# WPCLab/OpenSeg3D

Measured on AMD Instinct MI355X. Metric: points/sec fwd+bwd, Waymo 1-sweep ~180k pts @0.1m voxel; logit parity, higher is better.
Workload: dtype f32 storage/accumulate, bf16x3 products; 1 GPU; waymo_one_sweep (BASELINE configs[1]): synthetic scene, 174633 pts/step/GPU, voxel [0.1, 0.1, 0.1], grid [1440, 1440, 64], fwd (attention dropout p=0.1, DropPath) + criterion (ohem_ce+lovasz on 3 heads) + bwd + SGD step; mode=fwdbwd, segmentor=segformer, voxels=108690, parallelism=dp1

## Files before the change

include/seg3d_hip.h:

```cpp
#ifndef SEG3D_HIP_H
#define SEG3D_HIP_H

#include <stddef.h>
#include <stdint.h>

#ifdef __cplusplus
extern "C" {
#endif

#define SEG3D_OK 0
#define SEG3D_EINVAL (-1)
#define SEG3D_EWORKSPACE (-2)
#define SEG3D_ELAUNCH (-3)

#define SEG3D_REDUCE_SUM 0
#define SEG3D_REDUCE_MEAN 1
#define SEG3D_REDUCE_MAX 2

int seg3d_abi_version(void);

const char* seg3d_last_error(void);

int seg3d_grid_size(const float* voxel_size, const float* range, int32_t* grid_xyz);

size_t seg3d_voxelize_workspace_bytes(int64_t n_points);
int seg3d_voxelize_f32(const float* points, int64_t n_points, int32_t row_stride, int32_t xyz_col,
                       int32_t batch_col, const float* voxel_size, const float* range,
                       int32_t* voxel_coords, int32_t* point_voxel_ids, int32_t* n_voxels,
                       void* workspace, size_t workspace_bytes, void* stream);
int seg3d_voxelize_f64(const double* points, int64_t n_points, int32_t row_stride, int32_t xyz_col,
                       int32_t batch_col, const float* voxel_size, const float* range,
                       int32_t* voxel_coords, int32_t* point_voxel_ids, int32_t* n_voxels,
                       void* workspace, size_t workspace_bytes, void* stream);

size_t seg3d_voxelize_host_workspace_bytes(int64_t n_points);
int seg3d_voxelize_host_f32(const float* points, int64_t n_points, int32_t row_stride, int32_t xyz_col,
                            int32_t batch_col, const float* voxel_size, const float* range,
                            int32_t* voxel_coords, int32_t* point_voxel_ids, int32_t* n_voxels,
                            void* workspace, size_t workspace_bytes);
int seg3d_voxelize_host_f64(const double* points, int64_t n_points, int32_t row_stride, int32_t xyz_col,
                            int32_t batch_col, const float* voxel_size, const float* range,
                            int32_t* voxel_coords, int32_t* point_voxel_ids, int32_t* n_voxels,
                            void* workspace, size_t workspace_bytes);

int seg3d_cart2polar_f32(const float* points, int64_t n_points, int32_t row_stride, int32_t xyz_col,
                         float* out , void* stream);
int seg3d_cart2polar_f64(const double* points, int64_t n_points, int32_t row_stride, int32_t xyz_col,
                         double* out , void* stream);

size_t seg3d_group_index_workspace_bytes(int64_t n, int64_t n_groups);
int seg3d_group_index(const int32_t* group_ids, int64_t n, int64_t n_groups, int32_t* rank,
                      int32_t* order, int32_t* offsets, void* workspace, size_t workspace_bytes,
                      void* stream);

size_t seg3d_coord_hash_bytes(int64_t m);
int seg3d_coord_hash_build(const int32_t* coords, int64_t m, const int32_t* shape_zyx ,
                           void* table, size_t table_bytes, void* stream);
int seg3d_rulebook_subm(const int32_t* coords, int64_t m, const int32_t* shape_zyx ,
                        const void* table, size_t table_bytes, int32_t* nbr, void* stream);
size_t seg3d_downsample_workspace_bytes(int32_t batch_size, const int32_t* shape_in_zyx );
int seg3d_downsample_coords(const int32_t* coords_in, int64_t m_in,
                            const int32_t* m_in_dev ,
                            int32_t batch_size, const int32_t* shape_in_zyx , int32_t* coords_out,
                            int64_t cap_out, int32_t* m_out , void* workspace, size_t workspace_bytes,
                            void* stream);
int seg3d_rulebook_strided(const int32_t* coords_out, int64_t m_out, int64_t m_in,
                           const int32_t* shape_in_zyx , const void* table_in,
                           size_t table_bytes, int32_t* nbr_fwd, int32_t* nbr_inv, void* stream);

size_t seg3d_spconv_packed_bytes(int32_t cin, int32_t cout, int32_t flags);
int seg3d_spconv_pack_weight(const float* weight, int32_t cin, int32_t cout, int32_t flags,
                             void* w_packed, void* stream);
int seg3d_spconv_fwd(const float* x, const int32_t* nbr, int64_t m_out, int64_t m_in,
                     const void* w_packed, int32_t pack_flags, const float* bias ,
                     int32_t cin, int32_t cout, float* y,
                     const int32_t* row_order ,
                     void* stream);
int seg3d_spconv_fwd_act(const float* x, const int32_t* nbr, int64_t m_out, int64_t m_in, const void* w_packed,
                         int32_t pack_flags, const float* bias , const float* addend ,
                         int32_t relu, int32_t cin, int32_t cout, float* y, const int32_t* row_order ,
                         void* stream);
int seg3d_spconv_fwd_act_bf16(const void* x, int32_t x_bf16, const int32_t* nbr, int64_t m_out, int64_t m_in,
                              const void* w_packed, int32_t pack_flags, const float* bias,
                              const void* addend_bf16, int32_t relu, int32_t cin, int32_t cout, void* y_bf16,
                              const int32_t* row_order, void* stream);
size_t seg3d_spconv_presplit_bytes(int64_t m_in, int32_t cin);
int seg3d_spconv_presplit(const float* x, int64_t m_in, int32_t cin, void* xs, void* stream);
int seg3d_spconv_fwd_presplit(const void* xs, const int32_t* nbr, int64_t m_out, int64_t m_in, const void* w_packed,
                              int32_t pack_flags, const float* bias , const float* addend ,
                              int32_t relu, int32_t cin, int32_t cout, float* y,
                              const int32_t* row_order , void* stream);
size_t seg3d_conv_plan_bytes(int64_t m_out);
size_t seg3d_conv_plan_workspace_bytes(int64_t m_out);
int seg3d_conv_plan_build(const int32_t* coords, const int32_t* nbr, int64_t m_out, void* plan, void* workspace,
                          size_t workspace_bytes, void* stream);
int32_t seg3d_spconv_tiled_supported(int32_t cin, int32_t cout);
int seg3d_spconv_fwd_tiled(const float* x, const int32_t* nbr, const void* plan, int64_t m_out, int64_t m_in,
                           const void* w_packed, int32_t pack_flags, const float* bias ,
                           const float* addend , int32_t relu, int32_t cin, int32_t cout, float* y, void* stream);
int seg3d_spconv_fwd_tiled_bf16(const void* x, int32_t x_bf16, const int32_t* nbr, const void* plan, int64_t m_out,
                                int64_t m_in, const void* w_packed, int32_t pack_flags, const float* bias ,
                                const void* addend_bf16 , int32_t relu, int32_t cin, int32_t cout, void* y_bf16,
                                void* stream);
int seg3d_debug_set_conv_nbt(int32_t nbt);
int seg3d_debug_set_linear_stream(int32_t on);
size_t seg3d_spconv_wgrad_workspace_bytes(int64_t m_out, int32_t cin, int32_t cout);
int seg3d_spconv_wgrad(const float* x, const float* dy, const int32_t* nbr, int64_t m_out,
                       int64_t m_in, int32_t cin, int32_t cout, int32_t flags ,
                       float* dw, void* workspace, size_t workspace_bytes, void* stream);

int seg3d_spconv_wgrad_partials(const float* x, const float* dy, const int32_t* nbr, int64_t m_out, int64_t m_in,
                                int32_t cin, int32_t cout, void* workspace, size_t workspace_bytes, int32_t* chunks,
                                void* stream);
int seg3d_spconv_wgrad_partials_xbf16(const uint16_t* x_bf16, const float* dy, const int32_t* nbr, int64_t m_out,
                                      int64_t m_in, int32_t cin, int32_t cout, void* workspace, size_t workspace_bytes,
                                      int32_t* chunks, void* stream);

size_t seg3d_linear_wgrad_workspace_bytes(int64_t m, int32_t cin, int32_t cout);
int seg3d_linear_wgrad(const float* x, const float* dy, int64_t m, int32_t cin, int32_t cout, float* dw,
                       float* db , void* workspace, size_t workspace_bytes, void* stream);
int seg3d_linear_wgrad_partials(const float* x, const float* dy, int64_t m, int32_t cin, int32_t cout, int32_t with_bias,
                                void* workspace, size_t workspace_bytes, int32_t* chunks, void* stream);
int seg3d_linear_wgrad_partials_xbf16(const uint16_t* x_bf16, const float* dy, int64_t m, int32_t cin, int32_t cout,
                                      int32_t with_bias, void* workspace, size_t workspace_bytes, int32_t* chunks,
                                      void* stream);
int seg3d_debug_set_wgrad_lds(int32_t on);
int seg3d_reduce_partials(const float* part, int32_t chunks, int64_t n, int64_t nw, float* dw, float* db, void* stream);
int seg3d_reduce_partials_batched(const void* jobs, int32_t n_jobs, int64_t total_blocks, void* stream);
size_t seg3d_linear_packed_bytes_f32(int32_t cin, int32_t cout);
int seg3d_linear_pack_weight_f32(const float* weight, int32_t cin, int32_t cout, int32_t transpose,
                                 void* w_packed, void* stream);
int seg3d_linear_fwd_f32(const float* x, int64_t m, const void* w_packed, const float* bias ,
                         int32_t cin, int32_t cout, float* y, void* stream);
size_t seg3d_linear_packed_bytes_x6(int32_t cin, int32_t cout);
int seg3d_linear_pack_weight_x6(const float* weight, int32_t cin, int32_t cout, int32_t transpose, void* w_packed,
                                void* stream);
int seg3d_linear_fwd_x6(const float* x, int64_t m, const void* w_packed, const float* bias ,
                        const float* scale , const float* shift , int32_t relu, int32_t cin,
                        int32_t cout, float* y, void* stream);

typedef struct {
  const float* src;
  void* dst;
  int32_t cin, cout;
  int32_t kk, transpose, flip, reserved;
  int64_t first_block;
} seg3d_pack_job;
int seg3d_pack_weights_batched(const void* jobs, int32_t n_jobs, int64_t total_blocks, void* stream);

size_t seg3d_linear_packed_bytes(int32_t cin, int32_t cout, int32_t transpose);
int seg3d_linear_pack_weight(const float* weight, int32_t cin, int32_t cout, int32_t transpose,
                             void* w_packed, void* stream);
int seg3d_linear_fwd(const float* x, int64_t m, const void* w_packed, const float* bias ,
                     const float* addend , int32_t cin, int32_t cout,
                     float* y, void* stream);
int seg3d_linear_fwd_sum(const float* x, const float* x_add, int64_t m, const void* w_packed, const float* bias,
                         int32_t cin, int32_t cout, float* y, void* stream);
int seg3d_linear_layernorm_fwd(const float* x, int64_t m, const void* w_packed, const float* bias, const float* res,
                               const float* gamma, const float* beta, float eps, int32_t cin, int32_t cout, float* y,
                               void* stream);
int seg3d_linear_fwd_mul(const float* x, int64_t m, const void* w_packed, const float* factor, int32_t cin, int32_t cout,
                         float* y, void* stream);

size_t seg3d_window_partition_workspace_bytes(int64_t m, int32_t batch_size, const int32_t* nwin_xyz);
int seg3d_window_partition(const int32_t* coords, int64_t m, int32_t batch_size,
                           const int32_t* win_xyz, const int32_t* nwin_xyz, const int32_t* shift_xyz,
                           int32_t n_levels, const int32_t* level_lo, const int32_t* level_hi,
                           const int32_t* level_cap, int32_t* win_id, int32_t* in_win, int32_t* rank,
                           int32_t* level, int32_t* slot, int32_t* tok, int32_t* win_start,
                           int32_t* win_count, int32_t* win_tile0, int32_t* tile_item,
                           int32_t* qg_item, int32_t* counts, void* workspace,
                           size_t workspace_bytes, void* stream);

int seg3d_pos_embed(const int32_t* in_win, int64_t m, const int32_t* win_xyz ,
                    const float* inv_freq, int32_t c, float* pos, void* stream);

int seg3d_window_attn_supported(int32_t heads, int32_t dh);
size_t seg3d_window_attn_workspace_bytes(int64_t m, int32_t n_tiles, int32_t heads, int32_t dh);
int seg3d_window_attn_schedule(int32_t n_tiles, int32_t n_chunks, int32_t heads, int32_t dh, float dropout_p, int32_t* out);
int seg3d_window_attn_fwd(const float* q, const float* k, const float* v, int32_t ldq, int32_t ldk,
                          int32_t ldv, const int32_t* tok, const int32_t* win_start,
                          const int32_t* win_count, const int32_t* win_tile0,
                          const int32_t* tile_item, int32_t n_tiles, const int32_t* qg_item,
                          int32_t n_qgroups, int64_t m, int32_t n_windows, int32_t heads, int32_t dh,
                          const float* tau, float tau_min, float dropout_p, uint64_t dropout_seed, float* out,
                          float* lse, void* workspace, size_t workspace_bytes, void* stream);
int seg3d_window_attn_bwd(const float* q, const float* k, const float* v, int32_t ldq, int32_t ldk,
                          int32_t ldv, const float* out, const float* dout, const float* lse,
                          const int32_t* tok, const int32_t* win_start, const int32_t* win_count,
                          const int32_t* win_tile0, const int32_t* tile_item, int32_t n_tiles,
                          const int32_t* qg_item, int32_t n_qgroups, int64_t m, int32_t n_windows,
                          int32_t heads, int32_t dh, const float* tau,
                          float tau_min, float dropout_p, uint64_t dropout_seed, float* dq, float* dk,
                          float* dv, int32_t lddq, int32_t lddk,
                          int32_t lddv, float* dtau, void* workspace, size_t workspace_bytes,
                          void* stream);

int seg3d_layernorm_fwd(const float* x, const float* res, const float* gamma, const float* beta,
                        const float* rowscale, float eps, int64_t m, int32_t c, float* y, float* mean,
                        float* rstd, void* stream);
size_t seg3d_layernorm_bwd_workspace_bytes(int64_t m, int32_t c);
int seg3d_layernorm_bwd(const float* dy, const float* x, const float* mean, const float* rstd,
                        const float* gamma, const float* rowscale, int64_t m, int32_t c, float* dx,
                        float* dgamma, float* dbeta, void* workspace, size_t workspace_bytes, void* stream);
int seg3d_layernorm_bwd_partials(const float* dy, const float* x, const float* mean, const float* rstd,
                                 const float* gamma, const float* rowscale, int64_t m, int32_t c, float* dx,
                                 void* workspace, size_t workspace_bytes, int32_t* nblocks, void* stream);
size_t seg3d_batchnorm_workspace_bytes(int64_t m, int32_t c);
int seg3d_colstats(const float* x, int64_t m, int32_t c, float* sums, void* workspace, size_t workspace_bytes,
                   void* stream);
int seg3d_batchnorm_stats(const float* x, int64_t m, int32_t c, float eps, const float* gamma, const float* beta,
                          float momentum, float* running_mean, float* running_var, float* stats, void* workspace,
                          size_t workspace_bytes, void* stream);
int seg3d_gelu_fwd(const float* h, int64_t n, float* g, float* gp, void* stream);
int seg3d_affine_act(const float* x, const float* res, const float* scale, const float* shift, int32_t relu,
                     int64_t m, int32_t c, float* y, void* stream);
int seg3d_batchnorm_bwd(const float* dy, const float* y, const float* x, const float* mean, const float* rstd,
                        const float* gamma, int32_t relu, int64_t m, int32_t c, float* dx, float* dres,
                        float* sums, void* workspace, size_t workspace_bytes, void* stream);
int seg3d_batchnorm_bwd_reduce(const float* dy, const float* y, const float* x, const float* mean,
                               const float* rstd, int32_t relu, int64_t m, int32_t c, float* sums,
                               void* workspace, size_t workspace_bytes, void* stream);
int seg3d_batchnorm_bwd_apply(const float* dy, const float* y, const float* x, const float* mean,
                              const float* rstd, const float* gamma, const float* sums, const float* inv_count,
                              int32_t relu, int64_t m, int32_t c, float* dx, float* dres, void* stream);

int seg3d_segment_reduce_fwd(const float* x, int32_t c, const int32_t* order, const int32_t* offsets,
                             int64_t n_seg, int32_t mode, float* out, int32_t* argmax, void* stream);
int seg3d_segment_reduce_bwd(const float* dout, int32_t c, const int32_t* seg_of_row, int64_t n,
                             const int32_t* offsets, const int32_t* argmax, int64_t n_seg,
                             int32_t mode, float* dx, void* stream);

int seg3d_knn_attention_fwd(const float* q, const float* k, const float* v, const int32_t* idx,
                            const uint8_t* invalid, const float* keep, int64_t n, int64_t n_src,
                            int32_t n_neighbors, int32_t d, float scale, float* out, float* prob, void* stream);
int seg3d_knn_attention_bwd(const float* q, const float* k, const float* v, const int32_t* idx, const float* keep,
                            const float* prob, const float* dout, const int32_t* pair_order,
                            const int32_t* pair_offsets, int64_t n, int64_t n_src, int32_t n_neighbors, int32_t d,
                            float scale, float* dq, float* dk, float* dv, float* scratch, void* stream);

int seg3d_class_context_fwd(const float* feats, const float* probs, const int32_t* offsets, const int32_t* chunks,
                            const int32_t* chunk_offsets, int32_t n_chunks, int32_t batch, int64_t m,
                            int32_t classes, int32_t c, float scale, float* weights, float* partials, float* stats,
                            float* context, void* stream);
int seg3d_class_context_bwd(const float* feats, const float* weights, const float* dcontext,
                            const int32_t* offsets, const int32_t* chunks, const int32_t* chunk_offsets,
                            int32_t n_chunks, int32_t batch, int64_t m, int32_t classes, int32_t c, float scale,
                            float* dfeats, float* dprobs, float* scratch, void* stream);

int seg3d_gather_rows(const float* feats, const int32_t* ids, int64_t n, int32_t c, float* out,
                      void* stream);

int seg3d_knn_query(const float* xyz, int64_t n, const float* new_xyz, int64_t m, const int32_t* offset,
                    const int32_t* new_offset, int32_t batch_size, int32_t k, int32_t* idx, float* dist2,
                    void* stream);

size_t seg3d_knn_level_workspace_bytes(int64_t n);
int seg3d_knn_level_build(const float* xyz, int64_t n, const int32_t* offset, int32_t batch_size, float cell,
                          float* sorted_xyz, int32_t* src_index, int32_t* cell_end, void* table_keys, int32_t* table_vals,
                          int64_t capacity, void* workspace, size_t workspace_bytes, void* stream);
int seg3d_knn_query_order(const float* new_xyz, int64_t m, const int32_t* new_offset, int32_t batch_size, float cell,
                          int32_t* order, void* workspace, size_t workspace_bytes, void* stream);
int seg3d_parity_order(const int32_t* coords, int64_t m, int32_t* order, void* workspace, size_t workspace_bytes,
                       void* stream);
typedef struct {
  const float* sorted_xyz;
  const int32_t* src_index;
  const int32_t* cell_end;
  const void* table_keys;
  const int32_t* table_vals;
  int64_t capacity;
  float cell;
  int32_t max_ring;
} seg3d_knn_level;
int seg3d_knn_grid_query(const seg3d_knn_level* levels, int32_t n_levels, const float* new_xyz,
                         const int32_t* query_order , int64_t m,
                         const int32_t* offset, const int32_t* new_offset, int32_t batch_size, int32_t k,
                         int32_t* idx, float* dist2, void* stream);

size_t seg3d_furthest_sampling_workspace_bytes(int64_t n);
int seg3d_furthest_sampling(const float* xyz, int64_t n, const int32_t* order, const int32_t* offset,
                            const int32_t* new_offset, int32_t n_segments, int32_t* idx, void* workspace,
                            size_t workspace_bytes, void* stream);
int seg3d_furthest_sampling_host(const float* xyz, int64_t n, const int32_t* order, const int32_t* offset,
                                 const int32_t* new_offset, int32_t n_segments, int32_t* idx);
int seg3d_sector_angles(const float* xyz, int64_t n, const int32_t* offset, int32_t batch_size, float* angle,
                        float* minmax, void* stream);
int seg3d_sector_angles_host(const float* xyz, int64_t n, const int32_t* offset, int32_t batch_size, float* angle,
                             float* minmax);
int seg3d_sector_assign(const float* angle, int64_t n, const int32_t* offset, int32_t batch_size, const float* edges,
                        const int32_t* sector_offset, int32_t* sector_id, void* stream);
int seg3d_sector_assign_host(const float* angle, int64_t n, const int32_t* offset, int32_t batch_size,
                             const float* edges, const int32_t* sector_offset, int32_t* sector_id);

#define SEG3D_POINTOPS_CHUNK 512
size_t seg3d_pointops_scratch_bytes(int64_t m, int32_t k, int32_t width);
int seg3d_group_points_fwd(const float* xyz, const float* new_xyz, const float* feat, const int32_t* idx, int64_t n,
                           int64_t m, int32_t k, int32_t c, float* out, void* stream);
int seg3d_group_points_fwd_host(const float* xyz, const float* new_xyz, const float* feat, const int32_t* idx, int64_t n,
                                int64_t m, int32_t k, int32_t c, float* out);
int seg3d_group_points_bwd(const float* dout, const int32_t* idx, const int32_t* pair_order, const int32_t* pair_offsets,
                           int64_t n, int64_t m, int32_t k, int32_t c, int32_t with_xyz, float* dxyz, float* dnew_xyz,
                           float* dfeat, void* scratch, size_t scratch_bytes, void* stream);
int seg3d_group_points_bwd_host(const float* dout, const int32_t* idx, const int32_t* pair_order,
                                const int32_t* pair_offsets, int64_t n, int64_t m, int32_t k, int32_t c,
                                int32_t with_xyz, float* dxyz, float* dnew_xyz, float* dfeat);
int seg3d_knn_interpolate_fwd(const float* feat, const int32_t* idx, const float* dist, int64_t n, int64_t m, int32_t k,
                              int32_t c, float* out, float* weight, void* stream);
int seg3d_knn_interpolate_fwd_host(const float* feat, const int32_t* idx, const float* dist, int64_t n, int64_t m,
                                   int32_t k, int32_t c, float* out, float* weight);
int seg3d_knn_interpolate_bwd(const float* dout, const float* weight, const int32_t* idx, const int32_t* pair_order,
                              const int32_t* pair_offsets, int64_t n, int64_t m, int32_t k, int32_t c, float* dfeat,
                              void* scratch, size_t scratch_bytes, void* stream);
int seg3d_knn_interpolate_bwd_host(const float* dout, const float* weight, const int32_t* idx, const int32_t* pair_order,
                                   const int32_t* pair_offsets, int64_t n, int64_t m, int32_t k, int32_t c,
                                   float* dfeat);

#define SEG3D_SUBM_DOT_ROWS 128
size_t seg3d_subm_dot_scratch_bytes(int64_t M, int32_t C);
int seg3d_subm_dot_fwd(const float* x, const int32_t* nbr, const float* w, const float* bias, int64_t M, int32_t C,
                       float* s_out, float* y_out, void* stream);
int seg3d_subm_dot_fwd_host(const float* x, const int32_t* nbr, const float* w, const float* bias, int64_t M, int32_t C,
                            float* s_out, float* y_out);
int seg3d_subm_dot_bwd_ds(const float* dy, const float* x, const float* s, int64_t M, int32_t C, float* ds_out,
                          void* stream);
int seg3d_subm_dot_bwd_ds_host(const float* dy, const float* x, const float* s, int64_t M, int32_t C, float* ds_out);
int seg3d_subm_dot_bwd(const float* dy, const float* x, const float* s, const float* ds, const int32_t* nbr,
                       const float* w, int64_t M, int32_t C, float* dx, float* dw, float* dbias, void* scratch,
                       size_t scratch_bytes, void* stream);
int seg3d_subm_dot_bwd_host(const float* dy, const float* x, const float* s, const float* ds, const int32_t* nbr,
                            const float* w, int64_t M, int32_t C, float* dx, float* dw, float* dbias);

int seg3d_voxel_majority_labels(const uint8_t* point_labels, const int32_t* order, const int32_t* offsets,
                                int64_t n_voxels, int32_t ignore_index, uint8_t* voxel_labels, void* stream);

size_t seg3d_cross_entropy_workspace_bytes(int64_t n);
int seg3d_cross_entropy_fwd(const float* logits, const int64_t* labels, int64_t n, int32_t c, int64_t ignore_index,
                            float keep_thresh, float* lse, float* stats, void* workspace, size_t workspace_bytes,
                            void* stream);
int seg3d_cross_entropy_bwd(const float* logits, const int64_t* labels, const float* lse, const float* stats,
                            const float* grad_out, int64_t n, int32_t c, float* dlogits, void* stream);

size_t seg3d_lovasz_workspace_bytes(int64_t n, int32_t c);
int seg3d_lovasz_softmax_fwd(const float* logits, const int64_t* labels, int64_t n, int32_t c, int64_t ignore_index,
                             int32_t classes_mode, const int32_t* include, const float* class_weight, float* coef,
                             float* stats, void* workspace, size_t workspace_bytes, void* stream);
int seg3d_lovasz_softmax_bwd(const float* logits, const float* coef, const float* stats, const float* grad_out,
                             int64_t n, int32_t c, float* dlogits, void* stream);

#define SEG3D_CRITERION_MAX_HEADS 4
#define SEG3D_CRITERION_CE 1
#define SEG3D_CRITERION_LOVASZ 2
#define SEG3D_CRITERION_STATS_STRIDE 68
typedef struct {
    const float* logits;
    const int64_t* labels;
    int64_t n;
    float weight;
} seg3d_criterion_head;
typedef struct {
    int32_t n_heads;
    seg3d_criterion_head heads[SEG3D_CRITERION_MAX_HEADS];
} seg3d_criterion_table;
size_t seg3d_criterion_workspace_bytes(const seg3d_criterion_table* heads, int32_t c, int32_t terms);
int seg3d_criterion_fwd(const seg3d_criterion_table* heads, int32_t c, int32_t terms, int64_t ignore_index,
                        float keep_thresh, float w_ce, float w_lovasz, float* lse, float* coef, float* stats, float* loss,
                        void* workspace, size_t workspace_bytes, void* stream);
int seg3d_criterion_bwd(const seg3d_criterion_table* heads, int32_t c, int32_t terms, float w_ce, float w_lovasz,
                        const float* lse, const float* coef, const float* stats, const float* grad_out,
                        float* const* dlogits, void* stream);

size_t seg3d_pointwise_loss_workspace_bytes(int64_t n);
// ... 209 lines not shown
```

openseg3d_amd/_lib.py:

```python
import ctypes
import os
import re

_HERE = os.path.dirname(os.path.abspath(__file__))
LIB_PATH = os.path.join(_HERE, "csrc", "libseg3d_hip.so")
HEADER_PATH = os.path.join(os.path.dirname(_HERE), "include", "seg3d_hip.h")

OK, EINVAL, EWORKSPACE, ELAUNCH = 0, -1, -2, -3
REDUCE_SUM, REDUCE_MEAN, REDUCE_MAX = 0, 1, 2
ABI_VERSION = 53

_p, _i32, _i64, _sz, _f = ctypes.c_void_p, ctypes.c_int32, ctypes.c_int64, ctypes.c_size_t, ctypes.c_float
_u64 = ctypes.c_uint64
_d = ctypes.c_double

SIGNATURES = {
    "seg3d_abi_version": (ctypes.c_int, []),
    "seg3d_last_error": (ctypes.c_char_p, []),
    "seg3d_grid_size": (ctypes.c_int, [_p, _p, _p]),
    "seg3d_voxelize_workspace_bytes": (_sz, [_i64]),
    "seg3d_voxelize_f32": (ctypes.c_int, [_p, _i64, _i32, _i32, _i32, _p, _p, _p, _p, _p, _p, _sz, _p]),
    "seg3d_voxelize_f64": (ctypes.c_int, [_p, _i64, _i32, _i32, _i32, _p, _p, _p, _p, _p, _p, _sz, _p]),
    "seg3d_voxelize_host_workspace_bytes": (_sz, [_i64]),
    "seg3d_voxelize_host_f32": (ctypes.c_int, [_p, _i64, _i32, _i32, _i32, _p, _p, _p, _p, _p, _p, _sz]),
    "seg3d_voxelize_host_f64": (ctypes.c_int, [_p, _i64, _i32, _i32, _i32, _p, _p, _p, _p, _p, _p, _sz]),
    "seg3d_cart2polar_f32": (ctypes.c_int, [_p, _i64, _i32, _i32, _p, _p]),
    "seg3d_cart2polar_f64": (ctypes.c_int, [_p, _i64, _i32, _i32, _p, _p]),
    "seg3d_group_index_workspace_bytes": (_sz, [_i64, _i64]),
    "seg3d_group_index": (ctypes.c_int, [_p, _i64, _i64, _p, _p, _p, _p, _sz, _p]),
    "seg3d_coord_hash_bytes": (_sz, [_i64]),
    "seg3d_coord_hash_build": (ctypes.c_int, [_p, _i64, _p, _p, _sz, _p]),
    "seg3d_rulebook_subm": (ctypes.c_int, [_p, _i64, _p, _p, _sz, _p, _p]),
    "seg3d_downsample_workspace_bytes": (_sz, [_i32, _p]),
    "seg3d_downsample_coords": (ctypes.c_int, [_p, _i64, _p, _i32, _p, _p, _i64, _p, _p, _sz, _p]),
    "seg3d_rulebook_strided": (ctypes.c_int, [_p, _i64, _i64, _p, _p, _sz, _p, _p, _p]),
    "seg3d_spconv_packed_bytes": (_sz, [_i32, _i32, _i32]),
    "seg3d_spconv_pack_weight": (ctypes.c_int, [_p, _i32, _i32, _i32, _p, _p]),
    "seg3d_spconv_fwd": (ctypes.c_int, [_p, _p, _i64, _i64, _p, _i32, _p, _i32, _i32, _p, _p, _p]),
    "seg3d_spconv_fwd_act": (ctypes.c_int, [_p, _p, _i64, _i64, _p, _i32, _p, _p, _i32, _i32, _i32, _p, _p, _p]),
    "seg3d_spconv_fwd_act_bf16": (ctypes.c_int, [_p, _i32, _p, _i64, _i64, _p, _i32, _p, _p, _i32, _i32, _i32, _p, _p, _p]),
    "seg3d_spconv_presplit_bytes": (_sz, [_i64, _i32]),
    "seg3d_spconv_presplit": (ctypes.c_int, [_p, _i64, _i32, _p, _p]),
    "seg3d_spconv_fwd_presplit": (ctypes.c_int, [_p, _p, _i64, _i64, _p, _i32, _p, _p, _i32, _i32, _i32, _p, _p, _p]),
    "seg3d_conv_plan_bytes": (_sz, [_i64]),
    "seg3d_conv_plan_workspace_bytes": (_sz, [_i64]),
    "seg3d_conv_plan_build": (ctypes.c_int, [_p, _p, _i64, _p, _p, _sz, _p]),
    "seg3d_spconv_tiled_supported": (_i32, [_i32, _i32]),
    "seg3d_spconv_fwd_tiled": (ctypes.c_int, [_p, _p, _p, _i64, _i64, _p, _i32, _p, _p, _i32, _i32, _i32, _p, _p]),
    "seg3d_spconv_fwd_tiled_bf16": (ctypes.c_int, [_p, _i32, _p, _p, _i64, _i64, _p, _i32, _p, _p, _i32, _i32, _i32, _p, _p]),
    "seg3d_debug_set_conv_nbt": (ctypes.c_int, [_i32]),
    "seg3d_debug_set_linear_stream": (ctypes.c_int, [_i32]),
    "seg3d_spconv_wgrad_workspace_bytes": (_sz, [_i64, _i32, _i32]),
    "seg3d_spconv_wgrad": (ctypes.c_int, [_p, _p, _p, _i64, _i64, _i32, _i32, _i32, _p, _p, _sz, _p]),
    "seg3d_spconv_wgrad_partials": (ctypes.c_int, [_p, _p, _p, _i64, _i64, _i32, _i32, _p, _sz, _p, _p]),
    "seg3d_spconv_wgrad_partials_xbf16": (ctypes.c_int, [_p, _p, _p, _i64, _i64, _i32, _i32, _p, _sz, _p, _p]),
    "seg3d_linear_wgrad_partials_xbf16": (ctypes.c_int, [_p, _p, _i64, _i32, _i32, _i32, _p, ctypes.c_size_t, _p, _p]),
    "seg3d_linear_packed_bytes_f32": (ctypes.c_size_t, [_i32, _i32]),
    "seg3d_linear_pack_weight_f32": (ctypes.c_int, [_p, _i32, _i32, _i32, _p, _p]),
    "seg3d_linear_fwd_f32": (ctypes.c_int, [_p, _i64, _p, _p, _i32, _i32, _p, _p]),
    "seg3d_debug_set_wgrad_lds": (ctypes.c_int, [_i32]),
    "seg3d_linear_packed_bytes_x6": (ctypes.c_size_t, [_i32, _i32]),
    "seg3d_linear_pack_weight_x6": (ctypes.c_int, [_p, _i32, _i32, _i32, _p, _p]),
    "seg3d_linear_fwd_x6": (ctypes.c_int, [_p, _i64, _p, _p, _p, _p, _i32, _i32, _i32, _p, _p]),
    "seg3d_pack_weights_batched": (ctypes.c_int, [_p, _i32, _i64, _p]),
    "seg3d_linear_wgrad_workspace_bytes": (ctypes.c_size_t, [_i64, _i32, _i32]),
    "seg3d_linear_wgrad": (ctypes.c_int, [_p, _p, _i64, _i32, _i32, _p, _p, _p, ctypes.c_size_t, _p]),
    "seg3d_linear_wgrad_partials": (ctypes.c_int, [_p, _p, _i64, _i32, _i32, _i32, _p, ctypes.c_size_t, _p, _p]),
    "seg3d_reduce_partials": (ctypes.c_int, [_p, _i32, _i64, _i64, _p, _p, _p]),
    "seg3d_reduce_partials_batched": (ctypes.c_int, [_p, _i32, _i64, _p]),
    "seg3d_linear_packed_bytes": (_sz, [_i32, _i32, _i32]),
    "seg3d_linear_pack_weight": (ctypes.c_int, [_p, _i32, _i32, _i32, _p, _p]),
    "seg3d_linear_fwd": (ctypes.c_int, [_p, _i64, _p, _p, _p, _i32, _i32, _p, _p]),
    "seg3d_linear_fwd_sum": (ctypes.c_int, [_p, _p, _i64, _p, _p, _i32, _i32, _p, _p]),
    "seg3d_linear_fwd_mul": (ctypes.c_int, [_p, _i64, _p, _p, _i32, _i32, _p, _p]),
    "seg3d_linear_layernorm_fwd": (ctypes.c_int, [_p, _i64, _p, _p, _p, _p, _p, ctypes.c_float, _i32, _i32, _p, _p]),
    "seg3d_window_partition_workspace_bytes": (_sz, [_i64, _i32, _p]),
    "seg3d_window_partition": (ctypes.c_int, [_p, _i64, _i32, _p, _p, _p, _i32, _p, _p, _p,
                                              _p, _p, _p, _p, _p, _p, _p, _p, _p, _p, _p, _p, _p, _sz, _p]),
    "seg3d_pos_embed": (ctypes.c_int, [_p, _i64, _p, _p, _i32, _p, _p]),
    "seg3d_window_attn_supported": (ctypes.c_int, [_i32, _i32]),
    "seg3d_window_attn_workspace_bytes": (_sz, [_i64, _i32, _i32, _i32]),
    "seg3d_window_attn_schedule": (ctypes.c_int, [_i32, _i32, _i32, _i32, _f, _p]),
    "seg3d_window_attn_fwd": (ctypes.c_int, [_p, _p, _p, _i32, _i32, _i32, _p, _p, _p, _p, _p, _i32, _p, _i32,
                                             _i64, _i32, _i32, _i32, _p, _f, _f, _u64, _p, _p, _p, _sz, _p]),
    "seg3d_window_attn_bwd": (ctypes.c_int, [_p, _p, _p, _i32, _i32, _i32, _p, _p, _p, _p, _p, _p, _p, _p, _i32, _p,
                                             _i32, _i64, _i32, _i32, _i32, _p, _f, _f, _u64, _p, _p, _p, _i32, _i32, _i32,
                                             _p, _p, _sz, _p]),
    "seg3d_layernorm_fwd": (ctypes.c_int, [_p, _p, _p, _p, _p, _f, _i64, _i32, _p, _p, _p, _p]),
    "seg3d_layernorm_bwd_workspace_bytes": (ctypes.c_size_t, [_i64, _i32]),
    "seg3d_layernorm_bwd": (ctypes.c_int, [_p, _p, _p, _p, _p, _p, _i64, _i32, _p, _p, _p, _p, ctypes.c_size_t, _p]),
    "seg3d_layernorm_bwd_partials": (ctypes.c_int, [_p, _p, _p, _p, _p, _p, _i64, _i32, _p, _p, ctypes.c_size_t, _p, _p]),
    "seg3d_batchnorm_workspace_bytes": (ctypes.c_size_t, [_i64, _i32]),
    "seg3d_colstats": (ctypes.c_int, [_p, _i64, _i32, _p, _p, ctypes.c_size_t, _p]),
    "seg3d_batchnorm_stats": (ctypes.c_int, [_p, _i64, _i32, _f, _p, _p, _f, _p, _p, _p, _p, ctypes.c_size_t, _p]),
    "seg3d_affine_act": (ctypes.c_int, [_p, _p, _p, _p, _i32, _i64, _i32, _p, _p]),
    "seg3d_gelu_fwd": (ctypes.c_int, [_p, _i64, _p, _p, _p]),
    "seg3d_batchnorm_bwd": (ctypes.c_int, [_p, _p, _p, _p, _p, _p, _i32, _i64, _i32, _p, _p, _p, _p, ctypes.c_size_t, _p]),
    "seg3d_batchnorm_bwd_reduce": (ctypes.c_int, [_p, _p, _p, _p, _p, _i32, _i64, _i32, _p, _p, ctypes.c_size_t, _p]),
    "seg3d_batchnorm_bwd_apply": (ctypes.c_int, [_p, _p, _p, _p, _p, _p, _p, _p, _i32, _i64, _i32, _p, _p, _p]),
    "seg3d_segment_reduce_fwd": (ctypes.c_int, [_p, _i32, _p, _p, _i64, _i32, _p, _p, _p]),
    "seg3d_segment_reduce_bwd": (ctypes.c_int, [_p, _i32, _p, _i64, _p, _p, _i64, _i32, _p, _p]),
    "seg3d_voxel_majority_labels": (ctypes.c_int, [_p, _p, _p, _i64, _i32, _p, _p]),
    "seg3d_cross_entropy_workspace_bytes": (ctypes.c_size_t, [_i64]),
    "seg3d_cross_entropy_fwd": (ctypes.c_int, [_p, _p, _i64, _i32, _i64, _f, _p, _p, _p, ctypes.c_size_t, _p]),
    "seg3d_cross_entropy_bwd": (ctypes.c_int, [_p, _p, _p, _p, _p, _i64, _i32, _p, _p]),
    "seg3d_lovasz_workspace_bytes": (ctypes.c_size_t, [_i64, _i32]),
    "seg3d_lovasz_softmax_fwd": (ctypes.c_int, [_p, _p, _i64, _i32, _i64, _i32, _p, _p, _p, _p, _p, ctypes.c_size_t, _p]),
    "seg3d_lovasz_softmax_bwd": (ctypes.c_int, [_p, _p, _p, _p, _i64, _i32, _p, _p]),
    "seg3d_criterion_workspace_bytes": (ctypes.c_size_t, [_p, _i32, _i32]),
    "seg3d_criterion_fwd": (ctypes.c_int, [_p, _i32, _i32, _i64, _f, _f, _f, _p, _p, _p, _p, _p, ctypes.c_size_t, _p]),
    "seg3d_criterion_bwd": (ctypes.c_int, [_p, _i32, _i32, _f, _f, _p, _p, _p, _p, _p, _p]),
    "seg3d_pointwise_loss_workspace_bytes": (ctypes.c_size_t, [_i64]),
    "seg3d_focal_loss_fwd": (ctypes.c_int, [_p, _p, _i64, _i32, _i64, _f, _f, _p, _i32, _p, _p, ctypes.c_size_t, _p]),
    "seg3d_focal_loss_bwd": (ctypes.c_int, [_p, _p, _p, _p, _i64, _i32, _i64, _f, _f, _p, _i32, _p, _p]),
    "seg3d_dice_loss_fwd": (ctypes.c_int, [_p, _p, _i64, _i32, _i64, _f, _f, _p, _f, _f, _p, _p, ctypes.c_size_t, _p]),
    "seg3d_dice_loss_bwd": (ctypes.c_int, [_p, _p, _p, _i64, _i32, _i64, _f, _f, _p, _f, _f, _p, _p]),
    "seg3d_ce_select_workspace_bytes": (ctypes.c_size_t, [_i64]),
    "seg3d_ce_select_fwd": (ctypes.c_int, [_p, _p, _i64, _i32, _i64, _p, _i32, _f, ctypes.c_double, _p, _p, _p,
                                           ctypes.c_size_t, _p]),
    "seg3d_ce_select_bwd": (ctypes.c_int, [_p, _p, _p, _p, _p, _p, _i64, _i32, _i32, _p, _p]),
    "seg3d_knn_level_workspace_bytes": (ctypes.c_size_t, [_i64]),
    "seg3d_knn_level_build": (ctypes.c_int, [_p, _i64, _p, _i32, _f, _p, _p, _p, _p, _p, _i64, _p, ctypes.c_size_t, _p]),
    "seg3d_parity_order": (ctypes.c_int, [_p, _i64, _p, _p, ctypes.c_size_t, _p]),
    "seg3d_knn_query_order": (ctypes.c_int, [_p, _i64, _p, _i32, _f, _p, _p, ctypes.c_size_t, _p]),
    "seg3d_knn_grid_query": (ctypes.c_int, [_p, _i32, _p, _p, _i64, _p, _p, _i32, _i32, _p, _p, _p]),
    "seg3d_knn_query": (ctypes.c_int, [_p, _i64, _p, _i64, _p, _p, _i32, _i32, _p, _p, _p]),
    "seg3d_furthest_sampling_workspace_bytes": (_sz, [_i64]),
    "seg3d_furthest_sampling": (ctypes.c_int, [_p, _i64, _p, _p, _p, _i32, _p, _p, _sz, _p]),
    "seg3d_furthest_sampling_host": (ctypes.c_int, [_p, _i64, _p, _p, _p, _i32, _p]),
    "seg3d_sector_angles": (ctypes.c_int, [_p, _i64, _p, _i32, _p, _p, _p]),
    "seg3d_sector_angles_host": (ctypes.c_int, [_p, _i64, _p, _i32, _p, _p]),
    "seg3d_sector_assign": (ctypes.c_int, [_p, _i64, _p, _i32, _p, _p, _p, _p]),
    "seg3d_sector_assign_host": (ctypes.c_int, [_p, _i64, _p, _i32, _p, _p, _p]),
    "seg3d_pointops_scratch_bytes": (_sz, [_i64, _i32, _i32]),
    "seg3d_group_points_fwd": (ctypes.c_int, [_p, _p, _p, _p, _i64, _i64, _i32, _i32, _p, _p]),
    "seg3d_group_points_fwd_host": (ctypes.c_int, [_p, _p, _p, _p, _i64, _i64, _i32, _i32, _p]),
    "seg3d_group_points_bwd": (ctypes.c_int, [_p, _p, _p, _p, _i64, _i64, _i32, _i32, _i32, _p, _p, _p, _p, _sz, _p]),
    "seg3d_group_points_bwd_host": (ctypes.c_int, [_p, _p, _p, _p, _i64, _i64, _i32, _i32, _i32, _p, _p, _p]),
    "seg3d_knn_interpolate_fwd": (ctypes.c_int, [_p, _p, _p, _i64, _i64, _i32, _i32, _p, _p, _p]),
    "seg3d_knn_interpolate_fwd_host": (ctypes.c_int, [_p, _p, _p, _i64, _i64, _i32, _i32, _p, _p]),
    "seg3d_knn_interpolate_bwd": (ctypes.c_int, [_p, _p, _p, _p, _p, _i64, _i64, _i32, _i32, _p, _p, _sz, _p]),
    "seg3d_knn_interpolate_bwd_host": (ctypes.c_int, [_p, _p, _p, _p, _p, _i64, _i64, _i32, _i32, _p]),
    "seg3d_subm_dot_scratch_bytes": (_sz, [_i64, _i32]),
    "seg3d_subm_dot_fwd": (ctypes.c_int, [_p, _p, _p, _p, _i64, _i32, _p, _p, _p]),
    "seg3d_subm_dot_fwd_host": (ctypes.c_int, [_p, _p, _p, _p, _i64, _i32, _p, _p]),
    "seg3d_subm_dot_bwd_ds": (ctypes.c_int, [_p, _p, _p, _i64, _i32, _p, _p]),
    "seg3d_subm_dot_bwd_ds_host": (ctypes.c_int, [_p, _p, _p, _i64, _i32, _p]),
    "seg3d_subm_dot_bwd": (ctypes.c_int, [_p, _p, _p, _p, _p, _p, _i64, _i32, _p, _p, _p, _p, _sz, _p]),
    "seg3d_subm_dot_bwd_host": (ctypes.c_int, [_p, _p, _p, _p, _p, _p, _i64, _i32, _p, _p, _p]),
    "seg3d_gather_rows":(ctypes.c_int, [_p, _p, _i64, _i32, _p, _p]),
    "seg3d_class_context_fwd": (ctypes.c_int, [_p, _p, _p, _p, _p, _i32, _i32, _i64, _i32, _i32, _f, _p, _p, _p, _p, _p]),
    "seg3d_class_context_bwd": (ctypes.c_int, [_p, _p, _p, _p, _p, _p, _i32, _i32, _i64, _i32, _i32, _f, _p, _p, _p, _p]),
    "seg3d_knn_attention_fwd": (ctypes.c_int, [_p, _p, _p, _p, _p, _p, _i64, _i64, _i32, _i32, _f, _p, _p, _p]),
    "seg3d_knn_attention_bwd": (ctypes.c_int, [_p, _p, _p, _p, _p, _p, _p, _p, _p, _i64, _i64, _i32, _i32, _f, _p, _p, _p, _p, _p]),
    "seg3d_tta_views_f32": (ctypes.c_int, [_p, _i64, _i32, _p, _p, _p]),
    "seg3d_tta_views_host_f32": (ctypes.c_int, [_p, _i64, _i32, _p, _p]),
    "seg3d_softmax_accumulate_f32": (ctypes.c_int, [_p, _i64, _i32, _i32, _i32, _p, _p]),
    "seg3d_argmax_confusion": (ctypes.c_int, [_p, _p, _i64, _i32, _i32, _p, _i32, _p, _p, _p]),
    "seg3d_aug_polarmix_workspace_bytes": (_sz, [_i64, _i64]),
    "seg3d_aug_polarmix_map": (ctypes.c_int, [_p, _i64, _p, _i64, _i32, _i32, _p, _i32, _i32, _d, _d, _p, _i32, _i32, _i64,
                                              _p, _p, _p, _p, _sz, _p]),
    "seg3d_aug_polarmix_map_host": (ctypes.c_int, [_p, _i64, _p, _i64, _i32, _i32, _p, _i32, _i32, _d, _d, _p, _i32, _i32,
                                                   _i64, _p, _p, _p]),
    "seg3d_aug_far_near_workspace_bytes": (_sz, [_i64]),
    "seg3d_aug_far_near": (ctypes.c_int, [_p, _i64, _p, _i64, _i32, _i32, _p, _p, _i64, _p, _i64, _p, _f, _p, _p, _p, _p,
                                          _p, _sz, _p]),
    "seg3d_aug_far_near_host": (ctypes.c_int, [_p, _i64, _p, _i64, _i32, _i32, _p, _p, _i64, _p, _i64, _p, _f, _p, _p, _p,
                                               _p]),
    "seg3d_aug_sample_workspace_bytes": (_sz, [_i64]),
    "seg3d_aug_sample_device": (ctypes.c_int, [_p, _i64, _i64, _u64, _p, _p, _sz, _p]),
    "seg3d_aug_sample_host": (ctypes.c_int, [_p, _i64, _i64, _u64, _p]),
    "seg3d_aug_cur_map_workspace_bytes": (_sz, [_i64, _i64]),
    "seg3d_aug_cur_map": (ctypes.c_int, [_p, _i64, _p, _i64, _i64, _p, _p, _p, _p, _sz, _p]),
    "seg3d_aug_cur_map_host": (ctypes.c_int, [_p, _i64, _p, _i64, _i64, _p, _p, _p]),
    "seg3d_aug_apply_f32": (ctypes.c_int, [_p, _i64, _p, _i64, _i32, _p, _p, _i64, _p, _p, _p]),
    "seg3d_aug_apply_f64in": (ctypes.c_int, [_p, _i64, _p, _i64, _i32, _p, _p, _i64, _p, _p, _p]),
    "seg3d_aug_apply_host_f32": (ctypes.c_int, [_p, _i64, _p, _i64, _i32, _p, _p, _i64, _p, _p]),
    "seg3d_aug_apply_host_f64in": (ctypes.c_int, [_p, _i64, _p, _i64, _i32, _p, _p, _i64, _p, _p]),
    "seg3d_aug_gather": (ctypes.c_int, [_p, _i64, _p, _i64, _i64, _p, _i64, _p, _p]),
    "seg3d_aug_gather_host": (ctypes.c_int, [_p, _i64, _p, _i64, _i64, _p, _i64, _p]),
    "seg3d_aug_instance_workspace_bytes": (_sz, [_i64, _i64, _i32]),
    "seg3d_aug_instance_paste": (ctypes.c_int, [_p, _i64, _i32, _i32, _p, _i32, _p, _i32, _p, _i64, _p, _i32, _i64, _p, _p,
                                                _p, _p, _p, _sz, _p]),
    "seg3d_aug_instance_paste_host": (ctypes.c_int, [_p, _i64, _i32, _i32, _p, _i32, _p, _i32, _p, _i64, _p, _i32, _i64, _p,
                                                     _p, _p, _p]),
    "seg3d_instance_extract_workspace_bytes": (_sz, [_i64, _i32]),
    "seg3d_instance_extract": (ctypes.c_int, [_p, _i64, _i32, _i32, _p, _i32, _p, _p, _i32, _p, _i32, _d, _i32, _p, _p, _p, _p,
                                              _p, _sz, _p]),
    "seg3d_instance_extract_host": (ctypes.c_int, [_p, _i64, _i32, _i32, _p, _i32, _p, _p, _i32, _p, _i32, _d, _i32, _p, _p, _p,
                                                   _p]),
    "seg3d_frame_assemble": (ctypes.c_int, [_p, _i32, _i32, _p, _p, _p, _f, _p]),
    "seg3d_frame_assemble_host": (ctypes.c_int, [_p, _i32, _i32, _p, _p, _p, _f]),
    "seg3d_range_image_workspace_bytes": (_sz, [_i32, _i32]),
    "seg3d_range_image_labels": (ctypes.c_int, [_p, _i32, _p, _i64, _i32, _i32, _i32, _p, _p, _p, _p, _sz, _p]),
    "seg3d_range_image_labels_host": (ctypes.c_int, [_p, _i32, _p, _i64, _i32, _i32, _i32, _p, _p, _p]),
    "seg3d_point_image_features": (ctypes.c_int, [_p, _p, _i32, _i64, _i32, _i32, _p, _p, _p, _p]),
    "seg3d_point_image_features_host": (ctypes.c_int, [_p, _p, _i32, _i64, _i32, _i32, _p, _p, _p]),
}

_ERR = {EINVAL: "SEG3D_EINVAL (bad argument)", EWORKSPACE: "SEG3D_EWORKSPACE (workspace too small)",
        ELAUNCH: "SEG3D_ELAUNCH (HIP launch/runtime error)"}

_lib = None


class Seg3dError(RuntimeError):
    pass


def header_symbols():
    with open(HEADER_PATH) as f:
        text = f.read()
    text = re.sub(r"/\*.*?\*/", "", text, flags=re.S)
    return sorted(set(re.findall(r"\b(seg3d_[a-z0-9_]+)\s*\(", text)))


def load():
    global _lib
    if _lib is not None:
        return _lib
    if not os.path.exists(LIB_PATH):
        raise Seg3dError(
            f"{LIB_PATH} not found: the HIP library is required (no CPU fallback). "
            "Build it with `python __graft_entry__.py`.")
    import torch
    lib = ctypes.CDLL(LIB_PATH)
    for name, (res, args) in SIGNATURES.items():
        fn = getattr(lib, name)
        fn.restype = res
        fn.argtypes = args
    if lib.seg3d_abi_version() != ABI_VERSION:
        raise Seg3dError(f"libseg3d_hip.so ABI {lib.seg3d_abi_version()} != binding {ABI_VERSION}")
    _lib = lib
    return lib


def call(name, *args):
    lib = load()
    rc = getattr(lib, name)(*args)
    if rc != OK:
        detail = ""
        if rc == ELAUNCH:
            text = lib.seg3d_last_error()
            detail = f": {text.decode(errors='replace')}" if text else ""
        raise Seg3dError(f"{name} failed: {_ERR.get(rc, rc)}{detail}")


def query(name, *args):
    return int(getattr(load(), name)(*args))
```

openseg3d_amd/csrc/linear_x6.hip:

```cpp
#include <cstdlib>
#include <type_traits>

#include "split_bf16.hpp"

namespace {

using namespace sbf;

constexpr int kThreads = 256;
constexpr int kSlab = 4 * 3 * 64;

__global__ __launch_bounds__(256) void pack_x6_kernel(const float* __restrict__ w, int cin, int cout, int transpose,
                                                      uint4* __restrict__ wp) {
    const int ncg = cout >> 6;
    const int64_t total = (int64_t)(cin >> 5) * ncg * 4 * 64;
    const int64_t t = (int64_t)blockIdx.x * 256 + threadIdx.x;
    if (t >= total) return;
    const int lane = (int)(t & 63), j = (int)((t >> 6) & 3);
    const int64_t r = t >> 8;
    const int cg = (int)(r % ncg), kb = (int)(r / ncg);
    const int mi = lane & 15, g = lane >> 4;
    const int co = cg * 64 + 16 * j + mi;
    const int ci0 = kb * 32 + 4 * g;
    float v[8];
#pragma unroll
    for (int e = 0; e < 8; ++e) {
        const int ci = ci0 + (e < 4 ? e : 12 + e);
        v[e] = transpose ? w[(int64_t)ci * cout + co] : w[(int64_t)co * cin + ci];
    }
    bf16x8 h, m, l;
    split3(v, &h, &m, &l);
    uint4* dst = wp + ((((int64_t)kb * ncg + cg) * 4 + j) * 3) * 64 + lane;
    dst[0] = __builtin_bit_cast(uint4, h);
    dst[64] = __builtin_bit_cast(uint4, m);
    dst[128] = __builtin_bit_cast(uint4, l);
}

template <int RT, int WPS>
__global__ __launch_bounds__(kThreads, WPS) void linear_x6_kernel(const float* __restrict__ x, int64_t m_rows,
                                                                  const uint4* __restrict__ wp, const float* __restrict__ bias,
                                                                  const float* __restrict__ scale, const float* __restrict__ shift,
                                                                  int relu, int cin, int cout, float* __restrict__ y, int ncg,
                                                                  int64_t nrb) {
    constexpr int DEPTH = 2;
    __shared__ __attribute__((aligned(16))) uint4 wl[2][kSlab];
    const int tid = threadIdx.x, lane = tid & 63, wave = tid >> 6;
    const int g = lane >> 4, c16 = lane & 15;
    const int64_t id = blockIdx.x;
    const int64_t k = id >> 3;
    const int64_t rb = (k / ncg) * 8 + (id & 7);
    const int cg = (int)(k % ncg);
    if (rb >= nrb) return;
    const int64_t row0 = rb * (64 * RT) + wave * (16 * RT);
    const float* xp[RT];
#pragma unroll
    for (int i = 0; i < RT; ++i) {
        int64_t r = row0 + 16 * i + c16;
        r = r < m_rows ? r : m_rows - 1;
        xp[i] = x + r * cin + 4 * g;
    }
    const int nkb = cin >> 5;
    const uint4* wsrc = wp + (int64_t)cg * kSlab + tid;
    f32x4 raw[DEPTH][RT][2];
    auto issue_rows = [&](int kb, auto slot_tag) {
        constexpr int slot = decltype(slot_tag)::value;
        kb = kb < nkb ? kb : nkb - 1;
#pragma unroll
        for (int i = 0; i < RT; ++i) {
            const f32x4* p = reinterpret_cast<const f32x4*>(xp[i] + kb * 32);
            raw[slot][i][0] = p[0];
            raw[slot][i][1] = p[4];
        }
    };
    issue_rows(0, std::integral_constant<int, 0>{});
    issue_rows(1, std::integral_constant<int, 1>{});
    u32x4 wreg[2][3];
    auto issue_w = [&](int kb, auto slot_tag) {
        constexpr int slot = decltype(slot_tag)::value;
        kb = kb < nkb ? kb : nkb - 1;
        const u32x4* s = reinterpret_cast<const u32x4*>(wsrc + (int64_t)kb * ncg * kSlab);
        wreg[slot][0] = s[0];
        wreg[slot][1] = s[256];
        wreg[slot][2] = s[512];
    };
    {
        const uint4* s = wsrc;
        wl[0][tid] = s[0];
        wl[0][tid + 256] = s[256];
        wl[0][tid + 512] = s[512];
    }
    issue_w(1, std::integral_constant<int, 1>{});
    f32x4 acc[RT][4];
#pragma unroll
    for (int i = 0; i < RT; ++i)
#pragma unroll
        for (int j = 0; j < 4; ++j) acc[i][j] = (f32x4){0.f, 0.f, 0.f, 0.f};
    __syncthreads();

    auto step = [&](int kb, auto slot_tag) {
        constexpr int SLOT = decltype(slot_tag)::value;
        const int cur = kb & 1;
        const bool more = kb + 1 < nkb;
        bf16x8 xh[RT], xm[RT], xl[RT];
#pragma unroll
        for (int i = 0; i < RT; ++i) {
            const float v[8] = {raw[SLOT][i][0][0], raw[SLOT][i][0][1], raw[SLOT][i][0][2], raw[SLOT][i][0][3],
                                raw[SLOT][i][1][0], raw[SLOT][i][1][1], raw[SLOT][i][1][2], raw[SLOT][i][1][3]};
            split3(v, &xh[i], &xm[i], &xl[i]);
        }
        if (kb + 2 < nkb) {
            issue_rows(kb + DEPTH, slot_tag);
            issue_w(kb + 2, slot_tag);
        }
        __builtin_amdgcn_sched_barrier(0);
#pragma unroll
        for (int j = 0; j < 4; ++j) {
            const bf16x8 wh = __builtin_bit_cast(bf16x8, wl[cur][(j * 3 + 0) * 64 + lane]);
            const bf16x8 wm = __builtin_bit_cast(bf16x8, wl[cur][(j * 3 + 1) * 64 + lane]);
            const bf16x8 wlo = __builtin_bit_cast(bf16x8, wl[cur][(j * 3 + 2) * 64 + lane]);
#pragma unroll
            for (int i = 0; i < RT; ++i) {
                f32x4 a = acc[i][j];
                a = __builtin_amdgcn_mfma_f32_16x16x32_bf16(wlo, xh[i], a, 0, 0, 0);
                a = __builtin_amdgcn_mfma_f32_16x16x32_bf16(wh, xl[i], a, 0, 0, 0);
                a = __builtin_amdgcn_mfma_f32_16x16x32_bf16(wm, xm[i], a, 0, 0, 0);
                a = __builtin_amdgcn_mfma_f32_16x16x32_bf16(wm, xh[i], a, 0, 0, 0);
                a = __builtin_amdgcn_mfma_f32_16x16x32_bf16(wh, xm[i], a, 0, 0, 0);
                a = __builtin_amdgcn_mfma_f32_16x16x32_bf16(wh, xh[i], a, 0, 0, 0);
                acc[i][j] = a;
            }
        }
        if (more) {
            u32x4* dst = reinterpret_cast<u32x4*>(&wl[cur ^ 1][tid]);
            dst[0] = wreg[SLOT ^ 1][0];
            dst[256] = wreg[SLOT ^ 1][1];
            dst[512] = wreg[SLOT ^ 1][2];
        }
        __syncthreads();
    };
    if constexpr (DEPTH == 2) {
        int kb = 0;
        for (; kb + 1 < nkb; kb += 2) {
            step(kb, std::integral_constant<int, 0>{});
            step(kb + 1, std::integral_constant<int, 1>{});
        }
        if (kb < nkb) step(kb, std::integral_constant<int, 0>{});
    } else {
        for (int kb = 0; kb < nkb; ++kb) step(kb, std::integral_constant<int, 0>{});
    }

    const int col0 = cg * 64 + 4 * g;
    f32x4 b4[4], s4[4], t4[4];
#pragma unroll
    for (int j = 0; j < 4; ++j) {
        b4[j] = bias ? *reinterpret_cast<const f32x4*>(bias + col0 + 16 * j) : (f32x4){0.f, 0.f, 0.f, 0.f};
        if (scale) {
            s4[j] = *reinterpret_cast<const f32x4*>(scale + col0 + 16 * j);
            t4[j] = *reinterpret_cast<const f32x4*>(shift + col0 + 16 * j);
        }
    }
#pragma unroll
    for (int i = 0; i < RT; ++i) {
        const int64_t r = row0 + 16 * i + c16;
        if (r >= m_rows) continue;
        float* yr = y + r * cout + col0;
#pragma unroll
        for (int j = 0; j < 4; ++j) {
            f32x4 v = acc[i][j];
            if (bias) v = v + b4[j];
            if (scale) v = v * s4[j] + t4[j];
            if (relu) {
#pragma unroll
                for (int e = 0; e < 4; ++e) v[e] = fmaxf(v[e], 0.f);
            }
            *reinterpret_cast<f32x4*>(yr + 16 * j) = v;
        }
    }
}

static const int g_x6_rt = [] {
    const char* e = getenv("SEG3D_X6_RT");
    const int v = e ? atoi(e) : 2;
    return v == 4 ? 4 : 2;
}();
static const int g_x6_wps = [] {
    const char* e = getenv("SEG3D_X6_WPS");
    const int v = e ? atoi(e) : 3;
    return v == 4 ? 4 : 3;
}();

}

extern "C" {

size_t seg3d_linear_packed_bytes_x6(int32_t cin, int32_t cout) {
    if (cin <= 0 || cout <= 0 || (cin & 31) || (cout & 63)) return 0;
    return (size_t)(cin >> 5) * (size_t)(cout >> 6) * kSlab * sizeof(uint4);
}

int seg3d_linear_pack_weight_x6(const float* weight, int32_t cin, int32_t cout, int32_t transpose, void* w_packed, void* stream) {
    if (!weight || !w_packed || seg3d_linear_packed_bytes_x6(cin, cout) == 0) return SEG3D_EINVAL;
    const int64_t total = (int64_t)(cin >> 5) * (cout >> 6) * 256;
    hipLaunchKernelGGL(pack_x6_kernel, dim3((unsigned)((total + 255) / 256)), dim3(256), 0, as_stream(stream), weight, cin, cout,
                       transpose ? 1 : 0, static_cast<uint4*>(w_packed));
    SEG3D_CHECK_LAUNCH();
    return SEG3D_OK;
}

int seg3d_linear_fwd_x6(const float* x, int64_t m, const void* w_packed, const float* bias, const float* scale,
                        const float* shift, int32_t relu, int32_t cin, int32_t cout, float* y, void* stream) {
    if (m < 0 || seg3d_linear_packed_bytes_x6(cin, cout) == 0 || (scale == nullptr) != (shift == nullptr)) return SEG3D_EINVAL;
    if (m == 0) return SEG3D_OK;
    if (!x || !w_packed || !y) return SEG3D_EINVAL;
    const int ncg = cout >> 6;
    const int rows = 64 * g_x6_rt;
    const int64_t nrb = (m + rows - 1) / rows;
    const int64_t blocks = (nrb + 7) / 8 * 8 * ncg;
    if (blocks > 0x7FFFFFFFll) return SEG3D_EINVAL;
    if (g_x6_rt == 4)
        hipLaunchKernelGGL((linear_x6_kernel<4, 2>), dim3((unsigned)blocks), dim3(kThreads), 0, as_stream(stream), x, m,
                           static_cast<const uint4*>(w_packed), bias, scale, shift, relu ? 1 : 0, cin, cout, y, ncg, nrb);
    else if (g_x6_wps == 4)
        hipLaunchKernelGGL((linear_x6_kernel<2, 4>), dim3((unsigned)blocks), dim3(kThreads), 0, as_stream(stream), x, m,
                           static_cast<const uint4*>(w_packed), bias, scale, shift, relu ? 1 : 0, cin, cout, y, ncg, nrb);
    else
        hipLaunchKernelGGL((linear_x6_kernel<2, 3>), dim3((unsigned)blocks), dim3(kThreads), 0, as_stream(stream), x, m,
                           static_cast<const uint4*>(w_packed), bias, scale, shift, relu ? 1 : 0, cin, cout, y, ncg, nrb);
    SEG3D_CHECK_LAUNCH();
    return SEG3D_OK;
}

}
```

openseg3d_amd/csrc/rownorm.hip:

```cpp
#include "common.hpp"

namespace {

constexpr int kThreads = 256;
constexpr int kMaxBlocks = 2048;
constexpr int kLnBwdMaxBlocks = 1024;

struct RowMap {
    int quads;
    int p;
    int items;
};

inline RowMap row_map(int c) {
    RowMap m;
    m.quads = c / 4;
    m.items = (m.quads + 63) / 64;
    int need = (m.quads + m.items - 1) / m.items;
    m.p = 8;
    while (m.p < need) m.p <<= 1;
    return m;
}

__device__ __forceinline__ float group_sum(float v, int p) {
// ... 146 lines not shown
            s0 += part[(int64_t)b * 2 * c + i];
            s1 += part[(int64_t)(b + 32) * 2 * c + i];
            s2 += part[(int64_t)(b + 64) * 2 * c + i];
            s3 += part[(int64_t)(b + 96) * 2 * c + i];
        }
        for (; b < nblocks; b += 32) s0 += part[(int64_t)b * 2 * c + i];
        s = (s0 + s1) + (s2 + s3);
    }
    red[q][col] = s;
    __syncthreads();
    if (q == 0 && i < 2 * c) {
        float t = red[0][col];
#pragma unroll
        for (int k = 1; k < 32; ++k) t += red[k][col];
        if (i < c) dgamma[i] = t;
        else dbeta[i - c] = t;
    }
}

template <int MODE>
__global__ __launch_bounds__(kThreads) void col_reduce_kernel(const float* __restrict__ x, const float* __restrict__ dy,
                                                              const float* __restrict__ y, const float* __restrict__ mean,
                                                              const float* __restrict__ rstd, int relu, int64_t m, int c,
                                                              float* __restrict__ part ) {
    extern __shared__ float red[];
    const int quads = c / 4;
    const int lanes = kThreads / quads;
    const int q = threadIdx.x % quads, rl = threadIdx.x / quads;
    if (rl < lanes) {
        float4 a = make_float4(0.f, 0.f, 0.f, 0.f), b = a;
        float4 p0 = a, p1 = a;
        if (MODE == 0) p0 = *reinterpret_cast<const float4*>(x + 4 * q);
        if (MODE == 1) {
            p0 = *reinterpret_cast<const float4*>(mean + 4 * q);
            p1 = *reinterpret_cast<const float4*>(rstd + 4 * q);
        }
        for (int64_t row = (int64_t)blockIdx.x * lanes + rl; row < m; row += (int64_t)gridDim.x * lanes) {
            const float4 xv = *reinterpret_cast<const float4*>(x + row * c + 4 * q);
            if (MODE == 0) {
                const float dx_ = xv.x - p0.x, dy_ = xv.y - p0.y, dz_ = xv.z - p0.z, dw_ = xv.w - p0.w;
                a.x += dx_; a.y += dy_; a.z += dz_; a.w += dw_;
                b.x += dx_ * dx_; b.y += dy_ * dy_; b.z += dz_ * dz_; b.w += dw_ * dw_;
            } else {
                float4 g = *reinterpret_cast<const float4*>(dy + row * c + 4 * q);
                if (relu) {
                    const float4 yv = *reinterpret_cast<const float4*>(y + row * c + 4 * q);
                    g.x = yv.x > 0.f ? g.x : 0.f; g.y = yv.y > 0.f ? g.y : 0.f;
                    g.z = yv.z > 0.f ? g.z : 0.f; g.w = yv.w > 0.f ? g.w : 0.f;
                }
                a.x += g.x; a.y += g.y; a.z += g.z; a.w += g.w;
                b.x += g.x * (xv.x - p0.x) * p1.x; b.y += g.y * (xv.y - p0.y) * p1.y;
                b.z += g.z * (xv.z - p0.z) * p1.z; b.w += g.w * (xv.w - p0.w) * p1.w;
            }
        }
        *reinterpret_cast<float4*>(red + (size_t)rl * 2 * c + 4 * q) = a;
        *reinterpret_cast<float4*>(red + (size_t)rl * 2 * c + c + 4 * q) = b;
    }
    __syncthreads();
    for (int i = threadIdx.x; i < 2 * c; i += kThreads) {
        float t = red[i];
        for (int l = 1; l < lanes; ++l) t += red[(size_t)l * 2 * c + i];
        part[(size_t)blockIdx.x * 2 * c + i] = t;
    }
}

__device__ __forceinline__ float col_partial_sum(const float* __restrict__ part, int nblocks, int c2, int i, float (*red)[33]) {
    const int col = threadIdx.x & 31, q = threadIdx.x >> 5;
    float s = 0.f;
    if (i < c2) {
        float s0 = 0.f, s1 = 0.f, s2 = 0.f, s3 = 0.f;
        int b = q;
        for (; b + 96 < nblocks; b += 128) {
            s0 += part[(int64_t)b * c2 + i];
            s1 += part[(int64_t)(b + 32) * c2 + i];
            s2 += part[(int64_t)(b + 64) * c2 + i];
            s3 += part[(int64_t)(b + 96) * c2 + i];
        }
        for (; b < nblocks; b += 32) s0 += part[(int64_t)b * c2 + i];
        s = (s0 + s1) + (s2 + s3);
    }
    red[q][col] = s;
    __syncthreads();
    float t = red[0][col];
#pragma unroll
    for (int k = 1; k < 32; ++k) t += red[k][col];
    __syncthreads();
    return t;
}

__global__ __launch_bounds__(1024) void col_sums_finish(const float* __restrict__ part, int nblocks, int c,
                                                        float* __restrict__ sums ) {
    __shared__ float red[32][33];
    const int i = blockIdx.x * 32 + (threadIdx.x & 31);
    const float t = col_partial_sum(part, nblocks, 2 * c, i, red);
    if ((threadIdx.x >> 5) == 0 && i < 2 * c) sums[i] = t;
}

__global__ __launch_bounds__(kThreads) void gelu_fwd_kernel(const float* __restrict__ h, int64_t quads, float* __restrict__ g,
                                                            float* __restrict__ gp) {
    for (int64_t t = (int64_t)blockIdx.x * kThreads + threadIdx.x; t < quads; t += (int64_t)gridDim.x * kThreads) {
        const float4 v = reinterpret_cast<const float4*>(h)[t];
        const float in[4] = {v.x, v.y, v.z, v.w};
        float o[4], d[4];
#pragma unroll
        for (int i = 0; i < 4; ++i) {
            const float cdf = 0.5f * (1.0f + erff(in[i] * 0.70710678118654752440f));
            o[i] = in[i] * cdf;
            d[i] = cdf + in[i] * (0.39894228040143267794f * __expf(-0.5f * in[i] * in[i]));
        }
        reinterpret_cast<float4*>(g)[t] = make_float4(o[0], o[1], o[2], o[3]);
        if (gp) reinterpret_cast<float4*>(gp)[t] = make_float4(d[0], d[1], d[2], d[3]);
    }
}

__global__ __launch_bounds__(kThreads) void affine_act_kernel(const float* __restrict__ x, const float* __restrict__ res,
                                                              const float* __restrict__ scale, const float* __restrict__ shift,
                                                              int relu, int64_t total_quads, int quads, float* __restrict__ y) {
    for (int64_t t = (int64_t)blockIdx.x * kThreads + threadIdx.x; t < total_quads; t += (int64_t)gridDim.x * kThreads) {
        const int q = (int)(t % quads);
        const float4 xv = reinterpret_cast<const float4*>(x)[t];
        const float4 s = *reinterpret_cast<const float4*>(scale + 4 * q);
        const float4 b = *reinterpret_cast<const float4*>(shift + 4 * q);
        float4 o = make_float4(xv.x * s.x + b.x, xv.y * s.y + b.y, xv.z * s.z + b.z, xv.w * s.w + b.w);
        if (res) {
            const float4 r = reinterpret_cast<const float4*>(res)[t];
            o.x += r.x; o.y += r.y; o.z += r.z; o.w += r.w;
        }
        if (relu) {
            o.x = fmaxf(o.x, 0.f); o.y = fmaxf(o.y, 0.f); o.z = fmaxf(o.z, 0.f); o.w = fmaxf(o.w, 0.f);
        }
        reinterpret_cast<float4*>(y)[t] = o;
    }
}

__global__ __launch_bounds__(kThreads) void bn_bwd_apply_kernel(const float* __restrict__ dy, const float* __restrict__ y,
                                                                const float* __restrict__ x, const float* __restrict__ mean,
                                                                const float* __restrict__ rstd, const float* __restrict__ gamma,
                                                                const float* __restrict__ sums , int relu,
                                                                float inv_m, const float* __restrict__ inv_m_dev,
                                                                int64_t total_quads, int quads,
                                                                float* __restrict__ dx, float* __restrict__ dres) {
    const int c = quads * 4;
    if (inv_m_dev) inv_m = inv_m_dev[0];
    for (int64_t t = (int64_t)blockIdx.x * kThreads + threadIdx.x; t < total_quads; t += (int64_t)gridDim.x * kThreads) {
        const int q = (int)(t % quads);
        float4 g = reinterpret_cast<const float4*>(dy)[t];
        if (relu) {
            const float4 yv = reinterpret_cast<const float4*>(y)[t];
            g.x = yv.x > 0.f ? g.x : 0.f; g.y = yv.y > 0.f ? g.y : 0.f;
            g.z = yv.z > 0.f ? g.z : 0.f; g.w = yv.w > 0.f ? g.w : 0.f;
        }
        if (dres) reinterpret_cast<float4*>(dres)[t] = g;
        const float4 xv = reinterpret_cast<const float4*>(x)[t];
        const float4 mu = *reinterpret_cast<const float4*>(mean + 4 * q);
        const float4 rs = *reinterpret_cast<const float4*>(rstd + 4 * q);
        const float4 ga = *reinterpret_cast<const float4*>(gamma + 4 * q);
        const float4 s1 = *reinterpret_cast<const float4*>(sums + 4 * q);
        const float4 s2 = *reinterpret_cast<const float4*>(sums + c + 4 * q);
        float4 o;
        o.x = ga.x * rs.x * (g.x - s1.x * inv_m - (xv.x - mu.x) * rs.x * s2.x * inv_m);
        o.y = ga.y * rs.y * (g.y - s1.y * inv_m - (xv.y - mu.y) * rs.y * s2.y * inv_m);
        o.z = ga.z * rs.z * (g.z - s1.z * inv_m - (xv.z - mu.z) * rs.z * s2.z * inv_m);
        o.w = ga.w * rs.w * (g.w - s1.w * inv_m - (xv.w - mu.w) * rs.w * s2.w * inv_m);
        reinterpret_cast<float4*>(dx)[t] = o;
    }
}

__global__ __launch_bounds__(1024) void bn_finalize_kernel(const float* __restrict__ x, const float* __restrict__ part,
                                                           int nblocks, int64_t m, int c, float eps,
                                                           const float* __restrict__ gamma, const float* __restrict__ beta,
                                                           float momentum, float* __restrict__ running_mean,
                                                           float* __restrict__ running_var, float* __restrict__ stats) {
    __shared__ float red[32][33];
    const int i = blockIdx.x * 32 + (threadIdx.x & 31);
    const float s1 = col_partial_sum(part, nblocks, 2 * c, i < c ? i : 2 * c, red);
    const float s2 = col_partial_sum(part, nblocks, 2 * c, i < c ? c + i : 2 * c, red);
    if ((threadIdx.x >> 5) != 0 || i >= c) return;
    stats[i] = s1;
    stats[c + i] = s2;
    const float inv_m = 1.0f / (float)m;
    const float d = s1 * inv_m;
    const float mean = x[i] + d;
    const float var = fmaxf(s2 * inv_m - d * d, 0.0f);
    const float rstd = 1.0f / sqrtf(var + eps);
    const float scale = gamma[i] * rstd;
    stats[2 * c + i] = mean;
    stats[3 * c + i] = rstd;
    stats[4 * c + i] = scale;
    stats[5 * c + i] = beta[i] - mean * scale;
    if (running_mean) {
        running_mean[i] = running_mean[i] * (1.0f - momentum) + mean * momentum;
        const float unbiased = m > 1 ? var * ((float)m / (float)(m - 1)) : var;
        running_var[i] = running_var[i] * (1.0f - momentum) + unbiased * momentum;
    }
}

constexpr int kColMaxBlocks = 1024;
constexpr size_t kColSmem = 8192;

inline unsigned blocks_for(int64_t work_items, int per_block) {
    int64_t b = ceil_div64(work_items, per_block);
    if (b > kMaxBlocks) b = kMaxBlocks;
    if (b < 1) b = 1;
    return (unsigned)b;
}

inline bool bad_c(int c) { return c <= 0 || (c & 3) || c > 1024; }

}

extern "C" {

int seg3d_layernorm_fwd(const float* x, const float* res, const float* gamma, const float* beta, const float* rowscale,
                        float eps, int64_t m, int32_t c, float* y, float* mean, float* rstd, void* stream) {
    if (m < 0 || bad_c(c) || c > 512) return SEG3D_EINVAL;
    if (m == 0) return SEG3D_OK;
    if (!x || !gamma || !beta || !y) return SEG3D_EINVAL;
    const RowMap rm = row_map(c);
    const unsigned nb = blocks_for(m, 4 * (64 / rm.p));
    if (rm.items == 1)
        hipLaunchKernelGGL(ln_fwd_kernel<1>, dim3(nb), dim3(kThreads), 0, as_stream(stream), x, res, gamma, beta, rowscale,
                           eps, m, c, rm, y, mean, rstd);
    else
        hipLaunchKernelGGL(ln_fwd_kernel<2>, dim3(nb), dim3(kThreads), 0, as_stream(stream), x, res, gamma, beta, rowscale,
                           eps, m, c, rm, y, mean, rstd);
    SEG3D_CHECK_LAUNCH();
    return SEG3D_OK;
}

size_t seg3d_layernorm_bwd_workspace_bytes(int64_t m, int32_t c) {
    if (m < 0 || bad_c(c)) return 0;
    return (size_t)kLnBwdMaxBlocks * 2 * c * sizeof(float);
}

int seg3d_layernorm_bwd_partials(const float* dy, const float* x, const float* mean, const float* rstd, const float* gamma,
                                 const float* rowscale, int64_t m, int32_t c, float* dx, void* workspace,
                                 size_t workspace_bytes, int32_t* nblocks, void* stream) {
    if (m < 0 || bad_c(c) || c > 512 || !nblocks) return SEG3D_EINVAL;
    if (workspace_bytes < seg3d_layernorm_bwd_workspace_bytes(m, c) || !workspace) return SEG3D_EWORKSPACE;
    *nblocks = 0;
    if (m == 0) return SEG3D_OK;
    if (!dy || !x || !mean || !rstd || !gamma || !dx) return SEG3D_EINVAL;
    hipStream_t st = as_stream(stream);
    float* part = static_cast<float*>(workspace);
    const RowMap rm = row_map(c);
    unsigned nb = blocks_for(m, 4 * (64 / rm.p) * 4);
    if (nb > (unsigned)kLnBwdMaxBlocks) nb = kLnBwdMaxBlocks;
    const size_t smem = (size_t)4 * (64 / rm.p) * 2 * c * sizeof(float);
    if (rm.items == 1)
        hipLaunchKernelGGL(ln_bwd_kernel<1>, dim3(nb), dim3(kThreads), smem, st, dy, x, mean, rstd, gamma, rowscale, m, c, rm,
                           dx, part);
    else
        hipLaunchKernelGGL(ln_bwd_kernel<2>, dim3(nb), dim3(kThreads), smem, st, dy, x, mean, rstd, gamma, rowscale, m, c, rm,
                           dx, part);
    SEG3D_CHECK_LAUNCH();
    *nblocks = (int32_t)nb;
    return SEG3D_OK;
}

int seg3d_layernorm_bwd(const float* dy, const float* x, const float* mean, const float* rstd, const float* gamma,
                        const float* rowscale, int64_t m, int32_t c, float* dx, float* dgamma, float* dbeta,
                        void* workspace, size_t workspace_bytes, void* stream) {
    if (m < 0 || bad_c(c) || c > 512 || !dgamma || !dbeta) return SEG3D_EINVAL;
    if (workspace_bytes < seg3d_layernorm_bwd_workspace_bytes(m, c) || !workspace) return SEG3D_EWORKSPACE;
    hipStream_t st = as_stream(stream);
    float* part = static_cast<float*>(workspace);
    unsigned nb = 0;
    if (m > 0) {
        if (!dy || !x || !mean || !rstd || !gamma || !dx) return SEG3D_EINVAL;
        const RowMap rm = row_map(c);
        nb = blocks_for(m, 4 * (64 / rm.p) * 4);
        if (nb > (unsigned)kLnBwdMaxBlocks) nb = kLnBwdMaxBlocks;
        const size_t smem = (size_t)4 * (64 / rm.p) * 2 * c * sizeof(float);
        if (rm.items == 1)
            hipLaunchKernelGGL(ln_bwd_kernel<1>, dim3(nb), dim3(kThreads), smem, st, dy, x, mean, rstd, gamma, rowscale, m, c,
                               rm, dx, part);
        else
            hipLaunchKernelGGL(ln_bwd_kernel<2>, dim3(nb), dim3(kThreads), smem, st, dy, x, mean, rstd, gamma, rowscale, m, c,
                               rm, dx, part);
        SEG3D_CHECK_LAUNCH();
    }
    hipLaunchKernelGGL(ln_bwd_reduce, dim3((unsigned)((2 * c + 31) / 32)), dim3(1024), 0, st, part, (int)nb, c, dgamma,
                       dbeta);
    SEG3D_CHECK_LAUNCH();
    return SEG3D_OK;
}

size_t seg3d_batchnorm_workspace_bytes(int64_t m, int32_t c) {
    if (m < 0 || bad_c(c)) return 0;
    return (size_t)kColMaxBlocks * 2 * c * sizeof(float);
}

static unsigned col_blocks(int64_t m, int c) {
    const int lanes = kThreads / (c / 4);
    unsigned nb = blocks_for(m, lanes * 16);
    return nb > (unsigned)kColMaxBlocks ? (unsigned)kColMaxBlocks : nb;
}

int seg3d_colstats(const float* x, int64_t m, int32_t c, float* sums ,
                   void* workspace, size_t workspace_bytes, void* stream) {
    if (m <= 0 || bad_c(c) || !sums || !x) return SEG3D_EINVAL;
    if (!workspace || workspace_bytes < seg3d_batchnorm_workspace_bytes(m, c)) return SEG3D_EWORKSPACE;
    hipStream_t st = as_stream(stream);
    float* part = static_cast<float*>(workspace);
    const unsigned nb = col_blocks(m, c);
    hipLaunchKernelGGL(col_reduce_kernel<0>, dim3(nb), dim3(kThreads), kColSmem, st, x, nullptr, nullptr, nullptr, nullptr, 0, m,
                       c, part);
    SEG3D_CHECK_LAUNCH();
    hipLaunchKernelGGL(col_sums_finish, dim3((unsigned)((2 * c + 31) / 32)), dim3(1024), 0, st, part, (int)nb, c, sums);
    SEG3D_CHECK_LAUNCH();
    return SEG3D_OK;
}

int seg3d_batchnorm_stats(const float* x, int64_t m, int32_t c, float eps, const float* gamma, const float* beta,
                          float momentum, float* running_mean, float* running_var, float* stats ,
                          void* workspace, size_t workspace_bytes, void* stream) {
    if (m <= 0 || bad_c(c) || !x || !gamma || !beta || !stats || (running_mean && !running_var)) return SEG3D_EINVAL;
    if (!workspace || workspace_bytes < seg3d_batchnorm_workspace_bytes(m, c)) return SEG3D_EWORKSPACE;
    hipStream_t st = as_stream(stream);
    float* part = static_cast<float*>(workspace);
    const unsigned nb = col_blocks(m, c);
    hipLaunchKernelGGL(col_reduce_kernel<0>, dim3(nb), dim3(kThreads), kColSmem, st, x, nullptr, nullptr, nullptr, nullptr, 0, m,
                       c, part);
    SEG3D_CHECK_LAUNCH();
    hipLaunchKernelGGL(bn_finalize_kernel, dim3((unsigned)((c + 31) / 32)), dim3(1024), 0, st, x, part, (int)nb, m, c, eps, gamma,
                       beta, momentum, running_mean, running_var, stats);
    SEG3D_CHECK_LAUNCH();
    return SEG3D_OK;
}

int seg3d_gelu_fwd(const float* h, int64_t n, float* g, float* gp, void* stream) {
    if (n < 0 || (n & 3)) return SEG3D_EINVAL;
    if (n == 0) return SEG3D_OK;
    if (!h || !g) return SEG3D_EINVAL;
    hipLaunchKernelGGL(gelu_fwd_kernel, dim3(blocks_for(n / 4, kThreads * 4)), dim3(kThreads), 0, as_stream(stream), h, n / 4, g,
                       gp);
    SEG3D_CHECK_LAUNCH();
    return SEG3D_OK;
}

int seg3d_affine_act(const float* x, const float* res, const float* scale, const float* shift, int32_t relu, int64_t m,
                     int32_t c, float* y, void* stream) {
    if (m < 0 || bad_c(c)) return SEG3D_EINVAL;
    if (m == 0) return SEG3D_OK;
    if (!x || !scale || !shift || !y) return SEG3D_EINVAL;
    const int64_t tq = m * (c / 4);
    hipLaunchKernelGGL(affine_act_kernel, dim3(blocks_for(tq, kThreads * 4)), dim3(kThreads), 0, as_stream(stream), x, res,
                       scale, shift, relu, tq, c / 4, y);
    SEG3D_CHECK_LAUNCH();
    return SEG3D_OK;
}

int seg3d_batchnorm_bwd(const float* dy, const float* y, const float* x, const float* mean, const float* rstd,
                        const float* gamma, int32_t relu, int64_t m, int32_t c, float* dx, float* dres,
                        float* sums , void* workspace, size_t workspace_bytes, void* stream) {
    if (m <= 0 || bad_c(c) || !sums) return SEG3D_EINVAL;
    if (!workspace || workspace_bytes < seg3d_batchnorm_workspace_bytes(m, c)) return SEG3D_EWORKSPACE;
    if (!dy || !x || !mean || !rstd || !gamma || !dx || (relu && !y)) return SEG3D_EINVAL;
    hipStream_t st = as_stream(stream);
    float* part = static_cast<float*>(workspace);
    const unsigned nb = col_blocks(m, c);
    hipLaunchKernelGGL(col_reduce_kernel<1>, dim3(nb), dim3(kThreads), kColSmem, st, x, dy, y, mean, rstd, relu, m, c, part);
    SEG3D_CHECK_LAUNCH();
    hipLaunchKernelGGL(col_sums_finish, dim3((unsigned)((2 * c + 31) / 32)), dim3(1024), 0, st, part, (int)nb, c, sums);
    SEG3D_CHECK_LAUNCH();
    const int64_t tq = m * (c / 4);
    hipLaunchKernelGGL(bn_bwd_apply_kernel, dim3(blocks_for(tq, kThreads * 4)), dim3(kThreads), 0, st, dy, y, x, mean, rstd,
                       gamma, sums, relu, 1.0f / (float)m, nullptr, tq, c / 4, dx, dres);
    SEG3D_CHECK_LAUNCH();
    return SEG3D_OK;
}

int seg3d_batchnorm_bwd_reduce(const float* dy, const float* y, const float* x, const float* mean, const float* rstd,
                               int32_t relu, int64_t m, int32_t c, float* sums, void* workspace, size_t workspace_bytes,
                               void* stream) {
    if (m <= 0 || bad_c(c) || !sums) return SEG3D_EINVAL;
    if (!workspace || workspace_bytes < seg3d_batchnorm_workspace_bytes(m, c)) return SEG3D_EWORKSPACE;
    if (!dy || !x || !mean || !rstd || (relu && !y)) return SEG3D_EINVAL;
    hipStream_t st = as_stream(stream);
    float* part = static_cast<float*>(workspace);
    const unsigned nb = col_blocks(m, c);
    hipLaunchKernelGGL(col_reduce_kernel<1>, dim3(nb), dim3(kThreads), kColSmem, st, x, dy, y, mean, rstd, relu, m, c, part);
    SEG3D_CHECK_LAUNCH();
    hipLaunchKernelGGL(col_sums_finish, dim3((unsigned)((2 * c + 31) / 32)), dim3(1024), 0, st, part, (int)nb, c, sums);
    SEG3D_CHECK_LAUNCH();
    return SEG3D_OK;
}

int seg3d_batchnorm_bwd_apply(const float* dy, const float* y, const float* x, const float* mean, const float* rstd,
                              const float* gamma, const float* sums, const float* inv_count, int32_t relu, int64_t m,
                              int32_t c, float* dx, float* dres, void* stream) {
    if (m <= 0 || bad_c(c) || !sums || !inv_count) return SEG3D_EINVAL;
    if (!dy || !x || !mean || !rstd || !gamma || !dx || (relu && !y)) return SEG3D_EINVAL;
    const int64_t tq = m * (c / 4);
    hipLaunchKernelGGL(bn_bwd_apply_kernel, dim3(blocks_for(tq, kThreads * 4)), dim3(kThreads), 0, as_stream(stream), dy, y, x,
                       mean, rstd, gamma, sums, relu, 0.0f, inv_count, tq, c / 4, dx, dres);
    SEG3D_CHECK_LAUNCH();
    return SEG3D_OK;
}

}
```

openseg3d_amd/csrc/voxelize.hip:

```cpp
#include <cstdio>

#include "common.hpp"

namespace {

constexpr int kThreads = 256;

struct VoxParams {
    int32_t grid[3];
    int32_t row_stride, xyz_col, batch_col;
};

template <typename T>
struct VoxConst {
    T lo[3];
    T vs[3];
};

__device__ __forceinline__ float floor_t(float v) { return floorf(v); }
__device__ __forceinline__ double floor_t(double v) { return floor(v); }

template <typename T>
__global__ __launch_bounds__(kThreads) void vox_insert(const T* __restrict__ pts, int64_t n, VoxParams p,
                                                       VoxConst<T> c, HashView h, uint32_t* __restrict__ slot_of) {
// ... 97 lines not shown
                  int32_t* n_voxels, void* workspace, size_t workspace_bytes, void* stream) {
    if (n < 0 || n >= (int64_t)0x7F000000 || !voxel_size || !range || !voxel_coords || !n_voxels || !workspace ||
        row_stride < 3 || xyz_col < 0 || xyz_col + 3 > row_stride || batch_col >= row_stride)
        return SEG3D_EINVAL;
    if (n > 0 && (!points || !point_voxel_ids)) return SEG3D_EINVAL;
    if (workspace_bytes < ws_bytes(n)) return SEG3D_EWORKSPACE;
    hipStream_t st = as_stream(stream);
    VoxParams p;
    if (seg3d_grid_size(voxel_size, range, p.grid) != SEG3D_OK) return SEG3D_EINVAL;
    p.row_stride = row_stride;
    p.xyz_col = xyz_col;
    p.batch_col = batch_col;
    VoxConst<T> c;
    for (int j = 0; j < 3; ++j) {
        c.lo[j] = (T)range[j];
        c.vs[j] = (T)voxel_size[j];
    }
    VoxWs w = carve(workspace, n);
    HashView h = hash_view(w.table, w.cap);
    SEG3D_CHECK_HIP(hipMemsetAsync(h.keys, 0xFF, w.cap * 8, st));
    SEG3D_CHECK_HIP(hipMemsetAsync(h.vals, 0x7F, w.cap * 4, st));
    if (n == 0) {
        SEG3D_CHECK_HIP(hipMemsetAsync(n_voxels, 0, 4, st));
        return SEG3D_OK;
    }
    const unsigned nb = (unsigned)ceil_div64(n, kThreads);
    hipLaunchKernelGGL(vox_insert<T>, dim3(nb), dim3(kThreads), 0, st, points, n, p, c, h, w.slot_of);
    SEG3D_CHECK_LAUNCH();
    hipLaunchKernelGGL(vox_flag, dim3(nb), dim3(kThreads), 0, st, w.slot_of, n, h, w.flag);
    SEG3D_CHECK_LAUNCH();
    int rc = scan_exclusive_u32(w.flag, w.rank, n, reinterpret_cast<uint32_t*>(n_voxels), w.tmp, st);
    if (rc != SEG3D_OK) return rc;
    hipLaunchKernelGGL(vox_emit, dim3(nb), dim3(kThreads), 0, st, w.slot_of, w.rank, n, h, p, voxel_coords,
                       point_voxel_ids);
    SEG3D_CHECK_LAUNCH();
    return SEG3D_OK;
}

__device__ __forceinline__ float atan2_t(float y, float x) { return (float)atan2((double)y, (double)x); }
__device__ __forceinline__ double atan2_t(double y, double x) { return atan2(y, x); }
__device__ __forceinline__ float sqrt_t(float v) { return sqrtf(v); }
__device__ __forceinline__ double sqrt_t(double v) { return sqrt(v); }

template <typename T>
__global__ __launch_bounds__(kThreads) void cart2polar_rows(const T* __restrict__ pts, int64_t n, int row_stride, int xyz_col,
                                                            T* __restrict__ out) {
    const int64_t i = (int64_t)blockIdx.x * kThreads + threadIdx.x;
    if (i >= n) return;
    const T* row = pts + i * row_stride;
    T* o = out + i * (row_stride + 2);
    for (int j = 0; j < xyz_col; ++j) o[j] = row[j];
    const T x = row[xyz_col], y = row[xyz_col + 1], z = row[xyz_col + 2];
    o[xyz_col] = sqrt_t(x * x + y * y);
    o[xyz_col + 1] = atan2_t(y, x);
    o[xyz_col + 2] = z;
    o[xyz_col + 3] = x;
    o[xyz_col + 4] = y;
    for (int j = xyz_col + 3; j < row_stride; ++j) o[j + 2] = row[j];
}

template <typename T>
int cart2polar_impl(const T* points, int64_t n, int32_t row_stride, int32_t xyz_col, T* out, void* stream) {
    if (n < 0 || row_stride < 3 || xyz_col < 0 || xyz_col + 3 > row_stride) return SEG3D_EINVAL;
    if (n == 0) return SEG3D_OK;
    if (!points || !out) return SEG3D_EINVAL;
    hipLaunchKernelGGL(cart2polar_rows<T>, dim3((unsigned)ceil_div64(n, kThreads)), dim3(kThreads), 0, as_stream(stream), points, n,
                       row_stride, xyz_col, out);
    SEG3D_CHECK_LAUNCH();
    return SEG3D_OK;
}


inline float floor_h(float v) { return __builtin_floorf(v); }
inline double floor_h(double v) { return __builtin_floor(v); }

inline uint64_t host_capacity(int64_t n) {
    uint64_t cap = 64;
    while (cap < (uint64_t)(2 * n + 2)) cap <<= 1;
    return cap;
}

template <typename T>
int voxelize_host_impl(const T* points, int64_t n, int32_t row_stride, int32_t xyz_col, int32_t batch_col,
                       const float* voxel_size, const float* range, int32_t* voxel_coords, int32_t* point_voxel_ids,
                       int32_t* n_voxels, void* workspace, size_t workspace_bytes) {
    if (n < 0 || n >= (int64_t)0x7F000000 || !voxel_size || !range || !n_voxels || row_stride < 3 || xyz_col < 0 ||
        xyz_col + 3 > row_stride || batch_col >= row_stride)
        return SEG3D_EINVAL;
    if (n > 0 && (!points || !point_voxel_ids || !voxel_coords || !workspace)) return SEG3D_EINVAL;
    const uint64_t cap = host_capacity(n);
    if (n > 0 && workspace_bytes < cap * 12) return SEG3D_EWORKSPACE;
    int32_t grid[3];
    if (seg3d_grid_size(voxel_size, range, grid) != SEG3D_OK) return SEG3D_EINVAL;
    *n_voxels = 0;
    if (n == 0) return SEG3D_OK;
    uint64_t* keys = static_cast<uint64_t*>(workspace);
    int32_t* vals = reinterpret_cast<int32_t*>(keys + cap);
    for (uint64_t s = 0; s < cap; ++s) keys[s] = ~0ull;
    T lo[3], vs[3];
    for (int j = 0; j < 3; ++j) {
        lo[j] = (T)range[j];
        vs[j] = (T)voxel_size[j];
    }
    int32_t count = 0;
    for (int64_t i = 0; i < n; ++i) {
        const T* row = points + i * row_stride;
        int32_t cc[3];
        bool ok = true;
        for (int j = 0; j < 3 && ok; ++j) {
            volatile T d = row[xyz_col + j] - lo[j];
            volatile T q = d / vs[j];
            const T v = floor_h((T)q);
            if (!(v >= (T)0) || v >= (T)grid[j]) ok = false;
            else cc[j] = (int32_t)v;
        }
        if (!ok) {
            point_voxel_ids[i] = -1;
            continue;
        }
        const int64_t b = batch_col >= 0 ? (int64_t)row[batch_col] : 0;
        const uint64_t key = (uint64_t)(((b * grid[2] + cc[2]) * grid[1] + cc[1]) * (int64_t)grid[0] + cc[0]);
        uint64_t h = key * 0x9E3779B97F4A7C15ull;
        uint64_t s = (h ^ (h >> 29)) & (cap - 1);
        while (keys[s] != key && keys[s] != ~0ull) s = (s + 1) & (cap - 1);
        if (keys[s] == ~0ull) {
            keys[s] = key;
            vals[s] = count;
            int32_t* o = voxel_coords + 4 * (int64_t)count;
            o[0] = (int32_t)b;
            o[1] = cc[2];
            o[2] = cc[1];
            o[3] = cc[0];
            ++count;
        }
        point_voxel_ids[i] = vals[s];
    }
    *n_voxels = count;
    return SEG3D_OK;
}

}

extern "C" {

int seg3d_cart2polar_f32(const float* points, int64_t n_points, int32_t row_stride, int32_t xyz_col, float* out, void* stream) {
    return cart2polar_impl<float>(points, n_points, row_stride, xyz_col, out, stream);
}

int seg3d_cart2polar_f64(const double* points, int64_t n_points, int32_t row_stride, int32_t xyz_col, double* out,
                         void* stream) {
    return cart2polar_impl<double>(points, n_points, row_stride, xyz_col, out, stream);
}

int seg3d_abi_version(void) { return 53; }

namespace {
thread_local char g_last_error[320] = "";
}

const char* seg3d_last_error(void) { return g_last_error; }

int seg3d_grid_size(const float* voxel_size, const float* range, int32_t* grid_xyz) {
    if (!voxel_size || !range || !grid_xyz) return SEG3D_EINVAL;
    for (int j = 0; j < 3; ++j) {
        volatile float span = range[3 + j] - range[j];
        volatile float g = span / voxel_size[j];
        grid_xyz[j] = (int32_t)__builtin_rintf(g);
        if (grid_xyz[j] <= 0) return SEG3D_EINVAL;
    }
    return SEG3D_OK;
}

size_t seg3d_voxelize_workspace_bytes(int64_t n_points) { return ws_bytes(n_points < 0 ? 0 : n_points); }

int seg3d_voxelize_f32(const float* points, int64_t n_points, int32_t row_stride, int32_t xyz_col, int32_t batch_col,
                       const float* voxel_size, const float* range, int32_t* voxel_coords, int32_t* point_voxel_ids,
                       int32_t* n_voxels, void* workspace, size_t workspace_bytes, void* stream) {
    return voxelize_impl<float>(points, n_points, row_stride, xyz_col, batch_col, voxel_size, range, voxel_coords,
                                point_voxel_ids, n_voxels, workspace, workspace_bytes, stream);
}

int seg3d_voxelize_f64(const double* points, int64_t n_points, int32_t row_stride, int32_t xyz_col, int32_t batch_col,
                       const float* voxel_size, const float* range, int32_t* voxel_coords, int32_t* point_voxel_ids,
                       int32_t* n_voxels, void* workspace, size_t workspace_bytes, void* stream) {
    return voxelize_impl<double>(points, n_points, row_stride, xyz_col, batch_col, voxel_size, range, voxel_coords,
                                 point_voxel_ids, n_voxels, workspace, workspace_bytes, stream);
}

size_t seg3d_voxelize_host_workspace_bytes(int64_t n_points) { return (size_t)host_capacity(n_points < 0 ? 0 : n_points) * 12; }

int seg3d_voxelize_host_f32(const float* points, int64_t n_points, int32_t row_stride, int32_t xyz_col, int32_t batch_col,
                            const float* voxel_size, const float* range, int32_t* voxel_coords, int32_t* point_voxel_ids,
                            int32_t* n_voxels, void* workspace, size_t workspace_bytes) {
    return voxelize_host_impl<float>(points, n_points, row_stride, xyz_col, batch_col, voxel_size, range, voxel_coords,
                                     point_voxel_ids, n_voxels, workspace, workspace_bytes);
}

int seg3d_voxelize_host_f64(const double* points, int64_t n_points, int32_t row_stride, int32_t xyz_col, int32_t batch_col,
                            const float* voxel_size, const float* range, int32_t* voxel_coords, int32_t* point_voxel_ids,
                            int32_t* n_voxels, void* workspace, size_t workspace_bytes) {
    return voxelize_host_impl<double>(points, n_points, row_stride, xyz_col, batch_col, voxel_size, range, voxel_coords,
                                      point_voxel_ids, n_voxels, workspace, workspace_bytes);
}

}

void seg3d_note_hip_error(int code, const char* file, int line) {
    const char* base = file;
    for (const char* p = file; *p; ++p)
        if (*p == '/') base = p + 1;
    snprintf(g_last_error, sizeof(g_last_error), "%s (%s) at %s:%d", hipGetErrorString((hipError_t)code),
             hipGetErrorName((hipError_t)code), base, line);
}
```

openseg3d_amd/csrc/wgrad_dense.hip:

```cpp
#include <cstdlib>
#include <type_traits>

#include "split_bf16.hpp"

int wgrad_dense_lds_plan(int64_t m, int cin, int cout, int* chunks, int64_t* rows);
int wgrad_dense_lds_launch(const float* x, const float* dy, int64_t m, int cin, int cout, int chunks, int64_t rows, float* part,
                           int want_bias, hipStream_t st);

namespace {

using namespace sbf;

constexpr int kWaves = 4;
constexpr int kThreads = 64 * kWaves;

struct Plan {
    int nbo, nbi;
    int chunks;
    int64_t rows;
    int group;
    int lds;
};

static const bool g_wgrad_group = [] {
    const char* e = getenv("SEG3D_WGRAD_GROUP");
    return e && atoi(e) == 1;
}();

Plan plan(int64_t m, int cin, int cout, bool allow_lds = false) {
    Plan p{(cout + 63) / 64, (cin + 63) / 64, 0, 32, 0, 0};
    if (m <= 0) return p;
    if (allow_lds) {
        int c = 0;
        int64_t r = 0;
        if (wgrad_dense_lds_plan(m, cin, cout, &c, &r)) {
            p.chunks = c;
            p.rows = r;
            p.lds = 1;
            return p;
        }
    }
    if (g_wgrad_group && p.nbo * p.nbi >= 4 && m >= 8192) {
        int best_b = 0, best_c = 0;
        float best = 1e9f;
        for (int qb = 1; qb <= 4; ++qb)
            for (int qc = 1; qb * qc <= 4; ++qc) {
                if (p.nbo % qb || p.nbi % qc || qb * qc < 3) continue;
                const float slabs = (float)(qb + qc) / (float)(qb * qc) - 0.01f * (float)(qb * qc);
                if (slabs < best) best = slabs, best_b = qb, best_c = qc;
            }
        if (best_b) {
            p.group = best_b << 4 | best_c;
            const int groups = (p.nbo / best_b) * (p.nbi / best_c);
            int64_t chunks = 512 / groups / 8 * 8;
            if (chunks < 8) chunks = 8;
            int64_t rows = (m + chunks - 1) / chunks;
            if (rows < 32 * 8) rows = 32 * 8;
            rows = (rows + 31) / 32 * 32;
            p.rows = rows;
            p.chunks = (int)((m + rows - 1) / rows);
            return p;
        }
    }
    const int tiles = p.nbo * p.nbi;
    int target = tiles >= 16 ? 1024 : 512;
    if (const char* e = getenv("SEG3D_WGRAD_TARGET")) target = atoi(e);
    int64_t chunks = target / tiles / 8 * 8;
    if (chunks < 8) chunks = 8;
    int64_t rows = (m + chunks - 1) / chunks;
    if (rows < 32 * kWaves * 4) rows = 32 * kWaves * 4;
    rows = (rows + 31) / 32 * 32;
    p.rows = rows;
    p.chunks = (int)((m + rows - 1) / rows);
    return p;
}

template <bool XB, bool GROUP, int DEPTH = 1>
__global__ __launch_bounds__(kThreads, (DEPTH > 1 ? 1 : 2)) void wgrad_dense_kernel(const void* __restrict__ x_v, const float* __restrict__ dy,
                                                               int64_t m_rows, int cin, int cout, int rows_per_chunk,
                                                               int nbi, int tiles, float* __restrict__ part,
                                                               int want_bias, int group) {
    const float* x = static_cast<const float*>(x_v);
    __shared__ __attribute__((aligned(16))) float red[GROUP ? 4 : 64 * 64];
    __shared__ float red_b[GROUP ? 1 : kWaves][64];
    const int lane = threadIdx.x & 63, wave = threadIdx.x >> 6;
    const int cq = lane & 15, rg = lane >> 4;
    const int xcd = blockIdx.x & 7, k = blockIdx.x >> 3;
    const int chunk = (k / tiles) * 8 + xcd, tile = k % tiles;
    int bi = tile % nbi, bo = tile / nbi;
    if constexpr (GROUP) {
        const int qb = group >> 4, qc = group & 15;
        if (wave >= qb * qc) return;
        bo = bo * qb + wave / qc;
        bi = bi * qc + wave % qc;
    }
    const int ci0 = bi * 64, co0 = bo * 64;
    const int64_t r_begin = (int64_t)chunk * rows_per_chunk;
    if (r_begin >= m_rows) return;
    const int64_t r_end = r_begin + rows_per_chunk < m_rows ? r_begin + rows_per_chunk : m_rows;
    const bool a_ok = co0 + 4 * cq < cout, b_ok = ci0 + 4 * cq < cin;
    const uint32_t yoff = (uint32_t)((8 * rg * cout + (a_ok ? co0 + 4 * cq : 0)) * 4);
    const uint32_t xoff = (uint32_t)((8 * rg * cin + (b_ok ? ci0 + 4 * cq : 0)) * (XB ? 2 : 4));
    const bool want_db = want_bias && bi == 0;

    f32x4 acc[4][4];
#pragma unroll
    for (int a = 0; a < 4; ++a)
#pragma unroll
        for (int b = 0; b < 4; ++b) acc[a][b] = (f32x4){0.f, 0.f, 0.f, 0.f};
    f32x4 db_acc = {0.f, 0.f, 0.f, 0.f};

    f32x4 xr[XB ? 1 : 8], yr[8];
    f32x4 xd[DEPTH > 1 ? DEPTH : 1][8], yd[DEPTH > 1 ? DEPTH : 1][8];
    uint2 xq[XB ? 8 : 1];
    bf16x8 b_hi[4], b_lo[XB ? 1 : 4];
    auto load_rows = [&](const float* src, int ld, uint32_t off, int step, f32x4(&dst)[8]) {
        const char* base = reinterpret_cast<const char*>(src + (r_begin + 32 * (int64_t)step) * ld);
#pragma unroll
        for (int i = 0; i < 8; ++i) dst[i] = *reinterpret_cast<const f32x4*>(base + (size_t)i * ld * 4 + off);
    };
    auto load_x = [&](int step, auto& xs) {
        if constexpr (XB) {
            const char* base = static_cast<const char*>(x_v) + (r_begin + 32 * (int64_t)step) * cin * 2;
#pragma unroll
            for (int i = 0; i < 8; ++i) xq[i] = *reinterpret_cast<const uint2*>(base + (size_t)i * cin * 2 + xoff);
        } else {
            const char* base = reinterpret_cast<const char*>(x + (r_begin + 32 * (int64_t)step) * cin);
#pragma unroll
            for (int i = 0; i < 8; ++i) xs[i] = *reinterpret_cast<const f32x4*>(base + (size_t)i * cin * 4 + xoff);
        }
    };
    auto make_b = [&](auto& xs) {
#pragma unroll
        for (int b = 0; b < 4; ++b) {
            if constexpr (XB) {
                b_hi[b] = frag_from_bf16_rows(xq, b);
            } else {
                float v[8];
#pragma unroll
                for (int i = 0; i < 8; ++i) v[i] = xs[i][b];
                split_frag(v, &b_hi[b], &b_lo[b]);
            }
        }
    };
    auto multiply = [&](auto& ys) {
        if (want_db) {
#pragma unroll
            for (int i = 0; i < 8; ++i) db_acc += ys[i];
        }
#pragma unroll
        for (int a = 0; a < 4; ++a) {
            float v[8];
#pragma unroll
            for (int i = 0; i < 8; ++i) v[i] = ys[i][a];
            bf16x8 a_hi, a_lo;
            split_frag(v, &a_hi, &a_lo);
#pragma unroll
            for (int b = 0; b < 4; ++b) {
                if constexpr (XB) acc[a][b] = mfma2(a_hi, a_lo, b_hi[b], acc[a][b]);
                else acc[a][b] = mfma3(a_hi, a_lo, b_hi[b], b_lo[b], acc[a][b]);
            }
        }
    };
    const int n_full = (int)((r_end - r_begin) / 32);
    constexpr int kStride = GROUP ? 1 : kWaves;
    int s = GROUP ? 0 : wave;
    if constexpr (DEPTH > 1) {
        static_assert(!XB && !GROUP, "the deep form is the fp32 split-K form's");
#pragma unroll
        for (int d = 0; d < DEPTH; ++d)
            if (s + d * kStride < n_full) {
                load_x(s + d * kStride, xd[d]);
                load_rows(dy, cout, yoff, s + d * kStride, yd[d]);
            }
        for (; s < n_full; s += DEPTH * kStride) {
#pragma unroll
            for (int d = 0; d < DEPTH; ++d) {
                const int cur = s + d * kStride;
                if (cur < n_full) {
                    const bool more = cur + DEPTH * kStride < n_full;
                    make_b(xd[d]);
                    if (more) load_x(cur + DEPTH * kStride, xd[d]);
                    multiply(yd[d]);
                    if (more) load_rows(dy, cout, yoff, cur + DEPTH * kStride, yd[d]);
                }
            }
        }
    } else {
        if (s < n_full) {
            load_x(s, xr);
            load_rows(dy, cout, yoff, s, yr);
        }
        for (; s < n_full; s += kStride) {
            const bool more = s + kStride < n_full;
            make_b(xr);
            if (more) load_x(s + kStride, xr);
            multiply(yr);
            if (more) load_rows(dy, cout, yoff, s + kStride, yr);
        }
    }
    if ((r_end - r_begin) % 32 != 0 && (GROUP || n_full % kWaves == wave)) {
        const int64_t r0 = r_begin + 32 * (int64_t)n_full + 8 * rg;
        const f32x4 z = {0.f, 0.f, 0.f, 0.f};
#pragma unroll
        for (int i = 0; i < 8; ++i) {
            const bool ok = r0 + i < r_end;
            const int64_t r = ok ? r0 + i : r_end - 1;
            const f32x4 vy = *reinterpret_cast<const f32x4*>(dy + r * cout + (a_ok ? co0 + 4 * cq : 0));
            if constexpr (XB) {
                const uint2 vx = *reinterpret_cast<const uint2*>(static_cast<const char*>(x_v) + (r * cin + (b_ok ? ci0 + 4 * cq : 0)) * 2);
                xq[i] = ok ? vx : make_uint2(0u, 0u);
            } else {
                const f32x4 vx = *reinterpret_cast<const f32x4*>(x + r * cin + (b_ok ? ci0 + 4 * cq : 0));
                xr[i] = ok ? vx : z;
            }
            yr[i] = ok ? vy : z;
        }
        make_b(xr);
        multiply(yr);
    }

    float* pw = part + (int64_t)chunk * ((int64_t)cout * cin + cout);
    if constexpr (GROUP) {
#pragma unroll
        for (int a = 0; a < 4; ++a)
#pragma unroll
            for (int r = 0; r < 4; ++r) {
                const int co = co0 + 4 * (4 * rg + r) + a, ci = ci0 + 4 * cq;
                if (co < cout && ci < cin)
                    *reinterpret_cast<f32x4*>(pw + (int64_t)co * cin + ci) = (f32x4){acc[a][0][r], acc[a][1][r], acc[a][2][r], acc[a][3][r]};
            }
        if (want_db) {
#pragma unroll
            for (int j = 0; j < 4; ++j) {
                float v = db_acc[j];
                v += __shfl_xor(v, 16, SEG3D_WAVE);
                v += __shfl_xor(v, 32, SEG3D_WAVE);
                if (rg == 0 && co0 + 4 * cq + j < cout) pw[(int64_t)cout * cin + co0 + 4 * cq + j] = v;
            }
        }
        return;
    }
    for (int w = 0; w < kWaves; ++w) {
        if (wave == w) {
#pragma unroll
            for (int a = 0; a < 4; ++a)
#pragma unroll
                for (int r = 0; r < 4; ++r) {
                    f32x4* slot = reinterpret_cast<f32x4*>(&red[(4 * (4 * rg + r) + a) * 64 + 4 * cq]);
                    f32x4 v = {acc[a][0][r], acc[a][1][r], acc[a][2][r], acc[a][3][r]};
                    if (w > 0) v += *slot;
                    *slot = v;
                }
        }
        __syncthreads();
    }
    for (int e = threadIdx.x; e < 64 * 16; e += kThreads) {
        const int row = e >> 4, q = e & 15;
        const int co = co0 + row, ci = ci0 + 4 * q;
        if (co < cout && ci < cin)
            *reinterpret_cast<f32x4*>(pw + (int64_t)co * cin + ci) = *reinterpret_cast<const f32x4*>(&red[row * 64 + 4 * q]);
    }
    if (want_db) {
#pragma unroll
        for (int j = 0; j < 4; ++j) {
            float v = db_acc[j];
            v += __shfl_xor(v, 16, SEG3D_WAVE);
            v += __shfl_xor(v, 32, SEG3D_WAVE);
            if (rg == 0) red_b[wave][4 * cq + j] = v;
        }
        __syncthreads();
        if (threadIdx.x < 64 && co0 + threadIdx.x < cout) {
            float t = red_b[0][threadIdx.x];
#pragma unroll
            for (int w = 1; w < kWaves; ++w) t += red_b[w][threadIdx.x];
            pw[(int64_t)cout * cin + co0 + threadIdx.x] = t;
        }
    }
}

__device__ __forceinline__ void reduce_block(const float* __restrict__ part, int chunks, int64_t n, int64_t nw,
                                             float* __restrict__ dw, float* __restrict__ db, int64_t block) {
    __shared__ float4 red[4][64];
    const int cq = threadIdx.x & 63, q = threadIdx.x >> 6;
    const int64_t i = (block * 64 + cq) * 4;
    float4 acc[4];
#pragma unroll
    for (int u = 0; u < 4; ++u) acc[u] = make_float4(0.f, 0.f, 0.f, 0.f);
    if (i < n) {
        int c = q;
        for (; c + 12 < chunks; c += 16) {
#pragma unroll
            for (int u = 0; u < 4; ++u) {
                const float4 v = *reinterpret_cast<const float4*>(part + (int64_t)(c + 4 * u) * n + i);
                acc[u].x += v.x; acc[u].y += v.y; acc[u].z += v.z; acc[u].w += v.w;
            }
        }
        for (; c < chunks; c += 4) {
            const float4 v = *reinterpret_cast<const float4*>(part + (int64_t)c * n + i);
            acc[0].x += v.x; acc[0].y += v.y; acc[0].z += v.z; acc[0].w += v.w;
        }
    }
    float4 s;
    s.x = (acc[0].x + acc[1].x) + (acc[2].x + acc[3].x);
    s.y = (acc[0].y + acc[1].y) + (acc[2].y + acc[3].y);
    s.z = (acc[0].z + acc[1].z) + (acc[2].z + acc[3].z);
    s.w = (acc[0].w + acc[1].w) + (acc[2].w + acc[3].w);
    red[q][cq] = s;
    __syncthreads();
    if (q == 0 && i < n) {
        float4 t = red[0][cq];
#pragma unroll
        for (int k = 1; k < 4; ++k) {
            const float4 v = red[k][cq];
            t.x += v.x; t.y += v.y; t.z += v.z; t.w += v.w;
        }
        if (i < nw) *reinterpret_cast<float4*>(dw + i) = t;
        else if (db) *reinterpret_cast<float4*>(db + (i - nw)) = t;
    }
}

__global__ __launch_bounds__(256) void wgrad_dense_reduce(const float* __restrict__ part, int chunks, int64_t n,
                                                          int64_t nw, float* __restrict__ dw,
                                                          float* __restrict__ db) {
    reduce_block(part, chunks, n, nw, dw, db, (int64_t)blockIdx.x);
}

struct ReduceJob {
    const float* part;
    float* dw;
    float* db;
    int64_t n, nw;
    int32_t chunks, reserved;
    int64_t first_block;
};
static_assert(sizeof(ReduceJob) == 56, "ReduceJob layout is part of the C ABI (seg3d_reduce_partials_batched)");

__global__ __launch_bounds__(256) void reduce_partials_batched(const ReduceJob* __restrict__ jobs, int n_jobs) {
    int lo = 0, hi = n_jobs - 1;
    while (lo < hi) {
        const int mid = (lo + hi + 1) >> 1;
        if (jobs[mid].first_block <= (int64_t)blockIdx.x) lo = mid;
        else hi = mid - 1;
    }
    const ReduceJob jb = jobs[lo];
    reduce_block(jb.part, jb.chunks, jb.n, jb.nw, jb.dw, jb.db, (int64_t)blockIdx.x - jb.first_block);
}

}

int wgrad_chunk_reduce(const float* part, int chunks, int64_t n, int64_t nw, float* dw, float* db, hipStream_t st) {
    hipLaunchKernelGGL(wgrad_dense_reduce, dim3((unsigned)ceil_div64(n, 256)), dim3(256), 0, st, part, chunks, n, nw, dw, db);
    SEG3D_CHECK_LAUNCH();
    return SEG3D_OK;
}

extern "C" size_t seg3d_linear_wgrad_workspace_bytes(int64_t m, int32_t cin, int32_t cout) {
    if (m < 0 || cin <= 0 || cout <= 0) return 0;
    const Plan p = plan(m, cin, cout), q = plan(m, cin, cout, true);
    return ((size_t)(p.chunks > q.chunks ? p.chunks : q.chunks) * ((size_t)cin * cout + cout) + 64) * sizeof(float);
}

static void launch_dense(const Plan& p, const void* x, bool x_bf16, const float* dy, int64_t m, int cin, int cout, float* part,
                         int want_bias, hipStream_t st) {
    if (p.lds) {
        wgrad_dense_lds_launch(static_cast<const float*>(x), dy, m, cin, cout, p.chunks, p.rows, part, want_bias, st);
        return;
    }
    if (p.group) {
        const int qb = p.group >> 4, qc = p.group & 15;
        const int nbi_g = p.nbi / qc, groups = (p.nbo / qb) * nbi_g;
        const unsigned blocks = (unsigned)((p.chunks + 7) / 8 * 8) * (unsigned)groups;
        if (x_bf16)
            hipLaunchKernelGGL((wgrad_dense_kernel<true, true>), dim3(blocks), dim3(kThreads), 0, st, x, dy, m, cin, cout, (int)p.rows,
                               nbi_g, groups, part, want_bias, p.group);
        else
            hipLaunchKernelGGL((wgrad_dense_kernel<false, true>), dim3(blocks), dim3(kThreads), 0, st, x, dy, m, cin, cout, (int)p.rows,
                               nbi_g, groups, part, want_bias, p.group);
        return;
    }
    const int tiles = p.nbo * p.nbi;
    const unsigned blocks = (unsigned)((p.chunks + 7) / 8 * 8) * (unsigned)tiles;
    static const int depth = [] {
        const char* e = getenv("SEG3D_WGRAD_DENSE_DEPTH");
        return (e && atoi(e) == 3) ? 3 : 1;
    }();
    if (!x_bf16 && depth == 3) {
        hipLaunchKernelGGL((wgrad_dense_kernel<false, false, 3>), dim3(blocks), dim3(kThreads), 0, st, x, dy, m, cin, cout, (int)p.rows,
                           p.nbi, tiles, part, want_bias, 0);
        return;
    }
    if (x_bf16)
        hipLaunchKernelGGL((wgrad_dense_kernel<true, false>), dim3(blocks), dim3(kThreads), 0, st, x, dy, m, cin, cout, (int)p.rows,
                           p.nbi, tiles, part, want_bias, 0);
    else
        hipLaunchKernelGGL((wgrad_dense_kernel<false, false>), dim3(blocks), dim3(kThreads), 0, st, x, dy, m, cin, cout, (int)p.rows,
                           p.nbi, tiles, part, want_bias, 0);
}

static int linear_wgrad_partials(const void* x, bool x_bf16, const float* dy, int64_t m, int32_t cin, int32_t cout,
                                 int32_t with_bias, void* workspace, size_t workspace_bytes, int32_t* chunks, void* stream) {
    if (m < 0 || cin <= 0 || cout <= 0 || (cin & 3) || (cout & 3) || !chunks) return SEG3D_EINVAL;
    if (m > 0 && (!x || !dy)) return SEG3D_EINVAL;
    if (workspace_bytes < seg3d_linear_wgrad_workspace_bytes(m, cin, cout) || (m > 0 && !workspace)) return SEG3D_EINVAL;
    *chunks = 0;
    if (m == 0) return SEG3D_OK;
    const Plan p = plan(m, cin, cout, !x_bf16);
    launch_dense(p, x, x_bf16, dy, m, cin, cout, static_cast<float*>(workspace), with_bias ? 1 : 0, as_stream(stream));
    SEG3D_CHECK_LAUNCH();
    *chunks = p.chunks;
    return SEG3D_OK;
}

extern "C" int seg3d_linear_wgrad_partials(const float* x, const float* dy, int64_t m, int32_t cin, int32_t cout,
                                           int32_t with_bias, void* workspace, size_t workspace_bytes, int32_t* chunks,
                                           void* stream) {
    return linear_wgrad_partials(x, false, dy, m, cin, cout, with_bias, workspace, workspace_bytes, chunks, stream);
}

extern "C" int seg3d_linear_wgrad_partials_xbf16(const uint16_t* x_bf16, const float* dy, int64_t m, int32_t cin, int32_t cout,
                                                 int32_t with_bias, void* workspace, size_t workspace_bytes, int32_t* chunks,
                                                 void* stream) {
    return linear_wgrad_partials(x_bf16, true, dy, m, cin, cout, with_bias, workspace, workspace_bytes, chunks, stream);
}

extern "C" int seg3d_reduce_partials(const float* part, int32_t chunks, int64_t n, int64_t nw, float* dw, float* db,
                                     void* stream) {
    if (chunks < 0 || n <= 0 || nw < 0 || nw > n || (n & 3) || (nw & 3) || !dw || (chunks > 0 && !part)) return SEG3D_EINVAL;
    return wgrad_chunk_reduce(part, chunks, n, nw, dw, db, as_stream(stream));
}

extern "C" int seg3d_reduce_partials_batched(const void* jobs, int32_t n_jobs, int64_t total_blocks, void* stream) {
    if (n_jobs < 0 || total_blocks < 0 || total_blocks > 0x7FFFFFFF || (n_jobs > 0 && !jobs)) return SEG3D_EINVAL;
    if (n_jobs == 0 || total_blocks == 0) return SEG3D_OK;
    hipLaunchKernelGGL(reduce_partials_batched, dim3((unsigned)total_blocks), dim3(256), 0, as_stream(stream),
                       static_cast<const ReduceJob*>(jobs), (int)n_jobs);
    SEG3D_CHECK_LAUNCH();
    return SEG3D_OK;
}

extern "C" int seg3d_linear_wgrad(const float* x, const float* dy, int64_t m, int32_t cin, int32_t cout, float* dw,
                                  float* db, void* workspace, size_t workspace_bytes, void* stream) {
    if (m < 0 || cin <= 0 || cout <= 0 || (cin & 3) || (cout & 3) || !dw) return SEG3D_EINVAL;
    if (m > 0 && (!x || !dy)) return SEG3D_EINVAL;
    if (workspace_bytes < seg3d_linear_wgrad_workspace_bytes(m, cin, cout) || (m > 0 && !workspace)) return SEG3D_EINVAL;
    hipStream_t st = as_stream(stream);
    const Plan p = plan(m, cin, cout, true);
    float* part = static_cast<float*>(workspace);
    if (m > 0) {
        launch_dense(p, x, false, dy, m, cin, cout, part, db ? 1 : 0, st);
        SEG3D_CHECK_LAUNCH();
    }
    const int64_t nw = (int64_t)cin * cout;
    return wgrad_chunk_reduce(part, p.chunks, nw + cout, nw, dw, db, st);
}
```

openseg3d_amd/ops.py:

```python
import ctypes
import weakref
import os

import numpy as np
import torch

from . import _lib
from ._lib import REDUCE_MAX, REDUCE_MEAN, REDUCE_SUM

_F3 = ctypes.c_float * 3
_F6 = ctypes.c_float * 6
_I3 = ctypes.c_int32 * 3


def _need_gpu(*tensors):
    for t in tensors:
        if t is not None and not t.is_cuda:
            raise _lib.Seg3dError("openseg3d_amd ops run on the GPU only (no CPU fallback); got a CPU tensor")


def _ptr(t):
    return None if t is None else ctypes.c_void_p(t.data_ptr())


# ... 857 lines not shown

    @staticmethod
    def forward(ctx, x, weight, bias, exact):
        x = _f32c(x)
        cout, cin = weight.shape
        ctx.save_for_backward(_saved_rows(x) if ctx.needs_input_grad[1] else x, weight)
        ctx.has_bias, ctx.exact = bias is not None, exact
        ctx.bias_param = bias
        if exact:
            if _x6_fits(cin, cout):
                return _linear_apply_x6(x, _linear_pack_x6(weight), None if bias is None else _f32c(bias), cin, cout)
            if cin % 16 == 0 and cout % 16 == 0:
                return _linear_apply_f32(x, _linear_pack_f32(weight, 0), None if bias is None else _f32c(bias), cin, cout)
            return torch.nn.functional.linear(x, weight, bias)
        return _linear_apply(x, _linear_pack(weight, 0), None if bias is None else _f32c(bias), cin, cout)

    @staticmethod
    def backward(ctx, dy):
        x, weight = ctx.saved_tensors
        dy = _f32c(dy)
        cout, cin = weight.shape
        dx = dw = db = None
        fk = _WgradFork(dy.device)
        want_db = ctx.has_bias and ctx.needs_input_grad[2]
        if ctx.needs_input_grad[1]:
            dw = torch.empty_like(weight, memory_format=torch.contiguous_format)
            if want_db:
                db = torch.empty((cout,), dtype=torch.float32, device=dy.device)
            _linear_wgrad_into(fk, x, dy, cin, cout, dw.data_ptr(), db.data_ptr() if want_db else 0)
        elif want_db:
            db = dy.sum(0)
        if ctx.needs_input_grad[0]:
            if cout % 8 == 0 and cin % 16 == 0:
                dx = _linear_apply(dy, _linear_pack(weight, 1), None, cout, cin)
            elif ctx.exact and cout % 16 == 0 and cin % 16 == 0:
                dx = _linear_apply_f32(dy, _linear_pack_f32(weight, 1), None, cout, cin)
            else:
                dx = dy @ weight
        fk.join((weight, dw), (ctx.bias_param, db))
        return dx, dw, db, None


class _LinearOddShapeFn(torch.autograd.Function):

    @staticmethod
    def forward(ctx, x, weight, bias):
        x = _f32c(x)
        ctx.save_for_backward(x, weight)
        ctx.has_bias = bias is not None
        ctx.bias_param = bias
        return torch.nn.functional.linear(x, weight, bias)

    @staticmethod
    def backward(ctx, dy):
        x, weight = ctx.saved_tensors
        dy = _f32c(dy)
        cout, cin = weight.shape
        dx = dw = db = None
        fk = _WgradFork(dy.device)
        want_db = ctx.has_bias and ctx.needs_input_grad[2]
        if ctx.needs_input_grad[1]:
            pi, po = (-cin) % 4, (-cout) % 4
            xp = torch.nn.functional.pad(x, (0, pi)) if pi else x
            dyp = torch.nn.functional.pad(dy, (0, po)) if po else dy
            dwp = torch.empty((cout + po, cin + pi), dtype=torch.float32, device=dy.device)
            dbp = torch.empty((cout + po,), dtype=torch.float32, device=dy.device) if want_db else None
            _linear_wgrad_into(fk, xp, dyp, cin + pi, cout + po, dwp.data_ptr(), dbp.data_ptr() if want_db else 0)
            dw = dwp[:cout, :cin]
            if want_db:
                db = dbp[:cout]
        elif want_db:
            db = dy.sum(0)
        if ctx.needs_input_grad[0]:
            dx = dy @ weight
        if (cin % 4) or (cout % 4):
            fk.join()
        else:
            fk.join((weight, dw), (ctx.bias_param, db))
        return dx, dw, db


def linear(x, weight, bias=None, exact=False):
    fits = (x.is_cuda and x.dim() == 2 and x.dtype == torch.float32 and weight.shape[0] % 16 == 0
            and weight.shape[1] % 8 == 0 and CONV_PRECISION == "bf16x3")
    if exact and fits and weight.shape[1] % 16 == 0:
        return _LinearFn.apply(x, weight, bias, True)
    if not fits and x.is_cuda and x.dim() == 2 and x.dtype == torch.float32 and CONV_PRECISION == "bf16x3" \
            and torch.is_grad_enabled() and weight.requires_grad and x.shape[0] >= 4096:
        return _LinearOddShapeFn.apply(x, weight, bias)
    if not fits or (exact and not (torch.is_grad_enabled() and weight.requires_grad)):
        return torch.nn.functional.linear(x, weight, bias)
    return _LinearFn.apply(x, weight, bias, exact)


class _LayerNormResidualFn(torch.autograd.Function):

    @staticmethod
    def forward(ctx, x, res, gamma, beta, eps, rowscale):
        x = _f32c(x)
        m, c = x.shape
        y = torch.empty_like(x)
        mean = torch.empty((m,), dtype=torch.float32, device=x.device)
        rstd = torch.empty((m,), dtype=torch.float32, device=x.device)
        r = None if res is None else _f32c(res)
        rs = None if rowscale is None else _f32c(rowscale.reshape(-1))
        _lib.call("seg3d_layernorm_fwd", _ptr(x), _ptr(r), _ptr(gamma), _ptr(beta), _ptr(rs), float(eps), m, c, _ptr(y),
                  _ptr(mean), _ptr(rstd), _stream())
        ctx.save_for_backward(x, mean, rstd, gamma, rs)
        ctx.has_res = res is not None
        return y

    @staticmethod
    def backward(ctx, dy):
        x, mean, rstd, gamma, rs = ctx.saved_tensors
        dy = _f32c(dy)
        m, c = x.shape
        dx = torch.empty_like(x)
        dg = torch.empty((c,), dtype=torch.float32, device=x.device)
        db = torch.empty((c,), dtype=torch.float32, device=x.device)
        ws_bytes = _lib.query("seg3d_layernorm_bwd_workspace_bytes", m, c)
        ws = torch.empty((ws_bytes,), dtype=torch.uint8, device=x.device)
        fork = getattr(ctx, "fork", None)
        if fork is not None:
            nb = ctypes.c_int32(0)
            _lib.call("seg3d_layernorm_bwd_partials", _ptr(dy), _ptr(x), _ptr(mean), _ptr(rstd), _ptr(gamma), _ptr(rs), m, c,
                      _ptr(dx), _ptr(ws), ws_bytes, ctypes.byref(nb), _stream())
            fork.add_reduce(ws, nb.value, 2 * c, c, dg.data_ptr(), db.data_ptr())
            return dx, (dy if ctx.has_res else None), dg, db, None, None
        _lib.call("seg3d_layernorm_bwd", _ptr(dy), _ptr(x), _ptr(mean), _ptr(rstd), _ptr(gamma), _ptr(rs), m, c, _ptr(dx),
                  _ptr(dg), _ptr(db), _ptr(ws), ws_bytes, _stream())
        return dx, (dy if ctx.has_res else None), dg, db, None, None


def layer_norm_residual(x, res, ln, rowscale=None):
    c = x.shape[1]
    if not (x.is_cuda and x.dim() == 2 and x.dtype == torch.float32 and c % 4 == 0 and c <= 512
            and ln.elementwise_affine and ln.bias is not None):
        y = ln(x)
        if rowscale is not None:
            y = y * rowscale.reshape(-1, 1)
        return y if res is None else res + y
    return _LayerNormResidualFn.apply(x, res, ln.weight, ln.bias, ln.eps, rowscale)


class _BatchNormActFn(torch.autograd.Function):

    @staticmethod
    def forward(ctx, x, res, gamma, beta, mean, rstd, scale, shift, relu):
        x = _f32c(x)
        m, c = x.shape
        y = torch.empty_like(x)
        r = None if res is None else _f32c(res)
        _lib.call("seg3d_affine_act", _ptr(x), _ptr(r), _ptr(scale), _ptr(shift), int(relu), m, c, _ptr(y), _stream())
        ctx.save_for_backward(x, y, mean, rstd, gamma)
        ctx.relu, ctx.has_res = relu, res is not None
        return y

    @staticmethod
    def backward(ctx, dy):
        x, y, mean, rstd, gamma = ctx.saved_tensors
        dy = _f32c(dy)
        m, c = x.shape
        dx = torch.empty_like(x)
        dres = torch.empty_like(x) if ctx.has_res else None
        sums = torch.empty((2, c), dtype=torch.float32, device=x.device)
        ws_bytes = _lib.query("seg3d_batchnorm_workspace_bytes", m, c)
        ws = _workspace(ws_bytes, x.device)
        _lib.call("seg3d_batchnorm_bwd", _ptr(dy), _ptr(y), _ptr(x), _ptr(mean), _ptr(rstd), _ptr(gamma), int(ctx.relu),
                  m, c, _ptr(dx), _ptr(dres), _ptr(sums), _ptr(ws), ws_bytes, _stream())
        return dx, dres, sums[1], sums[0], None, None, None, None, None


def _sync_bn_group(bn):
    if not isinstance(bn, torch.nn.SyncBatchNorm) or not bn.training:
        return None
    import torch.distributed as dist
    if not (dist.is_available() and dist.is_initialized()):
        return None
    group = bn.process_group if bn.process_group is not None else dist.group.WORLD
    return group if dist.get_world_size(group) > 1 else None


def combine_moments(mean, m2, count):
    total = count.sum(dim=0)
    g_mean = (mean * count).sum(dim=0) / total
    g_m2 = (m2 + count * (mean - g_mean) ** 2).sum(dim=0)
    return g_mean, g_m2, total


def _all_gather_rows(t, group):
    import torch.distributed as dist
    world = dist.get_world_size(group)
    if dist.get_backend(group) == "gloo":
        parts = [torch.empty_like(t) for _ in range(world)]
        dist.all_gather(parts, t, group=group)
        return torch.stack(parts)
    out = torch.empty((world,) + tuple(t.shape), dtype=t.dtype, device=t.device)
    dist.all_gather_into_tensor(out, t, group=group)
    return out


class _SyncBatchNormActFn(torch.autograd.Function):

    @staticmethod
    def forward(ctx, x, res, gamma, beta, mean, rstd, scale, shift, inv_count, relu, group):
        m, c = x.shape
        y = torch.empty_like(x)
        r = None if res is None else _f32c(res)
        _lib.call("seg3d_affine_act", _ptr(x), _ptr(r), _ptr(scale), _ptr(shift), int(relu), m, c, _ptr(y), _stream())
        ctx.save_for_backward(x, y, mean, rstd, gamma, inv_count)
        ctx.relu, ctx.has_res, ctx.group = relu, res is not None, group
        return y

    @staticmethod
    def backward(ctx, dy):
        import torch.distributed as dist
        x, y, mean, rstd, gamma, inv_count = ctx.saved_tensors
        dy = _f32c(dy)
        m, c = x.shape
        sums = torch.empty((2, c), dtype=torch.float32, device=x.device)
        ws_bytes = _lib.query("seg3d_batchnorm_workspace_bytes", m, c)
        ws = _workspace(ws_bytes, x.device)
        if m > 0:
            _lib.call("seg3d_batchnorm_bwd_reduce", _ptr(dy), _ptr(y), _ptr(x), _ptr(mean), _ptr(rstd), int(ctx.relu), m, c,
                      _ptr(sums), _ptr(ws), ws_bytes, _stream())
        else:
            sums.zero_()
        total = sums.clone()
        dist.all_reduce(total, op=dist.ReduceOp.SUM, group=ctx.group)
        dx = torch.empty_like(x)
        dres = torch.empty_like(x) if ctx.has_res else None
        if m > 0:
            _lib.call("seg3d_batchnorm_bwd_apply", _ptr(dy), _ptr(y), _ptr(x), _ptr(mean), _ptr(rstd), _ptr(gamma),
                      _ptr(total), _ptr(inv_count), int(ctx.relu), m, c, _ptr(dx), _ptr(dres), _stream())
        return dx, dres, sums[1], sums[0], None, None, None, None, None, None, None


def _sync_batch_norm_act(x, bn, relu, res, group):
    xc = _f32c(x)
    m, c = xc.shape
    with torch.no_grad():
        sums = torch.empty((2, c), dtype=torch.float32, device=x.device)
        ws_bytes = _lib.query("seg3d_batchnorm_workspace_bytes", m, c)
        ws = _workspace(ws_bytes, x.device)
        if m > 0:
            _lib.call("seg3d_colstats", _ptr(xc), m, c, _ptr(sums), _ptr(ws), ws_bytes, _stream())
            d = sums[0] / m
            local = torch.cat([xc[0] + d, sums[1] - sums[0] * d, torch.full((1,), float(m), device=x.device)])
        else:
            local = torch.zeros((2 * c + 1,), dtype=torch.float32, device=x.device)
        g = _all_gather_rows(local, group)
        mean, m2, total = combine_moments(g[:, :c], g[:, c:2 * c], g[:, 2 * c:])
        var = (m2 / total).clamp_(min=0.0)
        rstd = torch.rsqrt(var + bn.eps)
        scale = (bn.weight * rstd).contiguous()
        shift = (bn.bias - mean * scale).contiguous()
        if bn.track_running_stats:
            bn._seg3d_stats_epoch = getattr(bn, "_seg3d_stats_epoch", 0) + 1
            _bump_batches_tracked(bn)
            mom = bn.momentum if bn.momentum is not None else 1.0 / float(bn.num_batches_tracked)
            bn.running_mean.mul_(1 - mom).add_(mean, alpha=mom)
            bn.running_var.mul_(1 - mom).add_(m2 / (total - 1).clamp_(min=1.0), alpha=mom)
        inv_count = (1.0 / total).to(torch.float32).contiguous()
    return _SyncBatchNormActFn.apply(xc, res, bn.weight, bn.bias, mean.contiguous(), rstd.contiguous(), scale, shift, inv_count,
                                     bool(relu), group)


class _SpanMeanFn(torch.autograd.Function):

    @staticmethod
    def forward(ctx, x, offsets):
        x = _f32c(x)
        c = x.shape[1]
        out = torch.zeros((len(offsets), c), dtype=torch.float32, device=x.device)
        lo = 0
        for b, hi in enumerate(offsets):
            rows = hi - lo
            if rows > 0:
                sums = torch.empty((2, c), dtype=torch.float32, device=x.device)
                ws_bytes = _lib.query("seg3d_batchnorm_workspace_bytes", rows, c)
                ws = _workspace(ws_bytes, x.device)
                _lib.call("seg3d_colstats", ctypes.c_void_p(x.data_ptr() + 4 * lo * c), rows, c, _ptr(sums), _ptr(ws), ws_bytes,
                          _stream())
                out[b] = x[lo] + sums[0] / rows
            lo = hi
        ctx.offsets, ctx.rows = tuple(offsets), x.shape[0]
        return out

    @staticmethod
    def backward(ctx, g):
        pieces, lo = [], 0
        for b, hi in enumerate(ctx.offsets):
            if hi > lo:
                pieces.append((g[b] / (hi - lo)).expand(hi - lo, g.shape[1]))
            lo = hi
        if lo < ctx.rows:
            pieces.append(g.new_zeros((ctx.rows - lo, g.shape[1])))
        if not pieces:
            return g.new_zeros((ctx.rows, g.shape[1])), None
        return (torch.cat(pieces) if len(pieces) != 1 else pieces[0].contiguous()), None


def span_mean(x, row_offsets):
    if not (x.is_cuda and x.dim() == 2 and x.dtype == torch.float32 and x.shape[1] % 4 == 0 and x.shape[1] <= 1024):
        lo, out = 0, []
        for hi in row_offsets:
            out.append(x[lo:hi].mean(dim=0) if hi > lo else x.new_zeros(x.shape[1]))
            lo = hi
        return torch.stack(out)
    return _SpanMeanFn.apply(x, [int(o) for o in row_offsets])


def narrow_batch_norm(x, bn):
    m, c = x.shape
    pad = (-c) % 4
    xp = torch.nn.functional.pad(_f32c(x), (0, pad))
    w = torch.nn.functional.pad(bn.weight, (0, pad), value=1.0)
    b = torch.nn.functional.pad(bn.bias, (0, pad))
    cp = c + pad
    with torch.no_grad():
        stats = torch.empty((6, cp), dtype=torch.float32, device=x.device)
        ws_bytes = _lib.query("seg3d_batchnorm_workspace_bytes", m, cp)
        ws = _workspace(ws_bytes, x.device)
        _lib.call("seg3d_batchnorm_stats", _ptr(xp), m, cp, float(bn.eps), _ptr(w), _ptr(b), 0.0, None, None, _ptr(stats),
                  _ptr(ws), ws_bytes, _stream())
        _bump_batches_tracked(bn)
        mom = bn.momentum if bn.momentum is not None else 1.0 / float(bn.num_batches_tracked)
        d = stats[0, :c] / m
        var = (stats[1, :c] / m - d * d).clamp_(min=0.0)
        bn.running_mean.mul_(1 - mom).add_(stats[2, :c], alpha=mom)
        bn.running_var.mul_(1 - mom).add_(var, alpha=mom * (m / max(m - 1, 1)))
    y = _BatchNormActFn.apply(xp, None, w, b, stats[2], stats[3], stats[4], stats[5], False)
    return y[:, :c]


_BN_COUNTERS = None


class deferred_bn_counters:
    def __enter__(self):
        global _BN_COUNTERS
        self.outer = _BN_COUNTERS
        if _BN_COUNTERS is None:
            _BN_COUNTERS = []
        return self

    def __exit__(self, *exc):
        global _BN_COUNTERS
        if self.outer is None:
            pending, _BN_COUNTERS = _BN_COUNTERS, None
            if pending:
                torch._foreach_add_(pending, 1)
        return False


def _bump_batches_tracked(bn):
    if _BN_COUNTERS is not None and bn.momentum is not None:
        _BN_COUNTERS.append(bn.num_batches_tracked)
    else:
        bn.num_batches_tracked += 1


def bn_eval_affine(bn):
    key = (_stamp(bn.weight), bn.bias._version, bn.running_mean._version, bn.running_var._version,
           bn.weight.data_ptr(), bn.running_var.data_ptr(), bn.eps, getattr(bn, "_seg3d_stats_epoch", 0))
    cached = getattr(bn, "_seg3d_eval_affine", None)
    if cached is None or cached[0] != key:
        with torch.no_grad():
            scale = bn.weight * torch.rsqrt(bn.running_var + bn.eps)
            shift = bn.bias - bn.running_mean * scale
        bn._seg3d_eval_affine = cached = (key, scale.contiguous(), shift.contiguous())
    return cached[1], cached[2], key


def batch_norm_act(x, bn, relu=True, res=None):
    c = x.shape[1]
    fits = x.is_cuda and x.dim() == 2 and x.dtype == torch.float32 and c % 4 == 0 and c <= 1024 and bn.affine
    use_batch = bn.training or not bn.track_running_stats
    if fits and use_batch:
        group = _sync_bn_group(bn)
        if group is not None:
            return _sync_batch_norm_act(x, bn, relu, res, group)
    if not fits or (not use_batch and torch.is_grad_enabled() and x.requires_grad) or x.shape[0] < 2:
        y = bn(x)
        if res is not None:
            y = y + res
        return torch.relu(y) if relu else y
    if use_batch:
        xc = _f32c(x)
        m = xc.shape[0]
        with torch.no_grad():
            stats = torch.empty((6, c), dtype=torch.float32, device=x.device)
            track = bn.training and bn.track_running_stats
            mom = 0.0
            if track:
                bn._seg3d_stats_epoch = getattr(bn, "_seg3d_stats_epoch", 0) + 1
                _bump_batches_tracked(bn)
                mom = bn.momentum if bn.momentum is not None else 1.0 / float(bn.num_batches_tracked)
            ws_bytes = _lib.query("seg3d_batchnorm_workspace_bytes", m, c)
            ws = _workspace(ws_bytes, x.device)
            _lib.call("seg3d_batchnorm_stats", _ptr(xc), m, c, float(bn.eps), _ptr(bn.weight), _ptr(bn.bias), float(mom),
                      _ptr(bn.running_mean) if track else None, _ptr(bn.running_var) if track else None, _ptr(stats),
                      _ptr(ws), ws_bytes, _stream())
        return _BatchNormActFn.apply(xc, res, bn.weight, bn.bias, stats[2], stats[3], stats[4], stats[5], bool(relu))
    with torch.no_grad():
        scale, shift, _ = bn_eval_affine(bn)
        xc = _f32c(x)
        y = torch.empty_like(xc)
        r = None if res is None else _f32c(res)
        _lib.call("seg3d_affine_act", _ptr(xc), _ptr(r), _ptr(scale), _ptr(shift), int(relu), xc.shape[0], c, _ptr(y),
                  _stream())
    return y


def linear_bn_act_eval(x, lin, bn, relu):
    if not (x.is_cuda and x.dim() == 2 and x.dtype == torch.float32):
        return None
    cout, cin = lin.weight.shape
    if not _x6_fits(cin, cout) or bn.training or not bn.track_running_stats or not bn.affine or bn.num_features != cout:
        return None
    if torch.is_grad_enabled() and (x.requires_grad or lin.weight.requires_grad):
        return None
    with torch.no_grad():
        scale, shift, _ = bn_eval_affine(bn)
        return _linear_apply_x6(_f32c(x), _linear_pack_x6(lin.weight), None if lin.bias is None else _f32c(lin.bias), cin, cout,
                                scale=scale, shift=shift, relu=relu)


class WindowIndex:
    __slots__ = ("win_id", "in_win", "rank", "level", "slot", "tok", "win_start", "win_count", "win_tile0",
                 "tile_item", "qg_item", "counts", "n_windows", "n_dropped", "n_tiles", "n_qgroups", "m")


def window_partition(coords, batch_size, window_shape, nwin_xyz, shift_xyz, levels, want_debug=False):
    _need_gpu(coords)
    coords = _i32c(coords)
    m, dev = coords.shape[0], coords.device
    canvas = int(batch_size) * int(nwin_xyz[0]) * int(nwin_xyz[1]) * int(nwin_xyz[2])
    cap = max(min(m, canvas), 1)
    wi = WindowIndex()
    wi.m = m
    i32 = dict(dtype=torch.int32, device=dev)
    wi.in_win = torch.empty((m, 3), **i32)
    wi.win_id = torch.empty((m,), **i32) if want_debug else None
    wi.rank = torch.empty((m,), **i32) if want_debug else None
    wi.level = torch.empty((m,), **i32) if want_debug else None
    wi.slot = torch.empty((m,), **i32) if want_debug else None
    wi.tok = torch.empty((max(m, 1),), **i32)
    wi.win_start = torch.empty((cap,), **i32)
    wi.win_count = torch.empty((cap,), **i32)
    wi.win_tile0 = torch.empty((cap,), **i32)
    wi.tile_item = torch.empty((m // 32 + cap + 1, 4), **i32)
    wi.qg_item = torch.empty((m // 16 + cap + 1, 4), **i32)
    wi.counts = torch.zeros((4,), **i32)
    nl = len(levels)
    arr = ctypes.c_int32 * nl
    lo, hi, capt = arr(*[int(l[0]) for l in levels]), arr(*[int(l[1]) for l in levels]), arr(*[int(l[2]) for l in levels])
    ws = _workspace(_lib.query("seg3d_window_partition_workspace_bytes", m, int(batch_size), _i3(nwin_xyz)), dev)
    _lib.call("seg3d_window_partition", _ptr(coords), m, int(batch_size), _i3(window_shape), _i3(nwin_xyz),
              _i3(shift_xyz), nl, lo, hi, capt, _ptr(wi.win_id), _ptr(wi.in_win), _ptr(wi.rank), _ptr(wi.level),
              _ptr(wi.slot), _ptr(wi.tok), _ptr(wi.win_start), _ptr(wi.win_count), _ptr(wi.win_tile0),
              _ptr(wi.tile_item), _ptr(wi.qg_item), _ptr(wi.counts), _ptr(ws), ws.numel(), _stream())
    wi.n_windows = wi.n_dropped = wi.n_tiles = wi.n_qgroups = None
    return wi


def pos_embed(in_win, window_shape, inv_freq, c):
    m = in_win.shape[0]
    pos = torch.empty((m, c), dtype=torch.float32, device=in_win.device)
    _lib.call("seg3d_pos_embed", _ptr(in_win), m, _i3(window_shape), _ptr(inv_freq), int(c), _ptr(pos), _stream())
    return pos


class _WindowAttnFn(torch.autograd.Function):
    @staticmethod
    def forward(ctx, q, k, v, tau, tau_min, heads, wi):
        m, c = v.shape
        dh = c // heads
        dev = v.device
        out = torch.empty((m, c), dtype=torch.float32, device=dev)
        lse = torch.empty((m, heads), dtype=torch.float32, device=dev)
        tau_f = tau.reshape(-1)
        _lib.call("seg3d_window_attn_fwd", _ptr(q), _ptr(k), _ptr(v), q.stride(0), k.stride(0), v.stride(0),
                  _ptr(wi.tok), _ptr(wi.win_start), _ptr(wi.win_count), _ptr(wi.win_tile0), _ptr(wi.tile_item),
                  int(wi.n_tiles), _ptr(wi.qg_item), int(wi.n_qgroups), m, int(wi.n_windows), heads, dh,
                  _ptr(tau_f), float(tau_min), 0.0, 0, _ptr(out), _ptr(lse), None, 0, _stream())
        ctx.save_for_backward(q, k, v, tau, out, lse)
        ctx.wi, ctx.heads, ctx.tau_min = wi, heads, tau_min
        return out

    @staticmethod
    def backward(ctx, dout):
        q, k, v, tau, out, lse = ctx.saved_tensors
        wi, heads = ctx.wi, ctx.heads
        m, c = v.shape
        dev = v.device
        dout = _f32c(dout)
        dq, dk, dv = (torch.empty((m, c), dtype=torch.float32, device=dev) for _ in range(3))
        dtau = torch.empty((1,), dtype=torch.float32, device=dev)
        ws = _workspace(_lib.query("seg3d_window_attn_workspace_bytes", m, int(wi.n_tiles), heads, c // heads), dev)
        _lib.call("seg3d_window_attn_bwd", _ptr(q), _ptr(k), _ptr(v), q.stride(0), k.stride(0), v.stride(0),
                  _ptr(out), _ptr(dout), _ptr(lse), _ptr(wi.tok), _ptr(wi.win_start), _ptr(wi.win_count),
                  _ptr(wi.win_tile0), _ptr(wi.tile_item), int(wi.n_tiles), _ptr(wi.qg_item), int(wi.n_qgroups), m,
                  int(wi.n_windows), heads, c // heads, _ptr(tau.reshape(-1)), float(ctx.tau_min), 0.0, 0, _ptr(dq), _ptr(dk),
                  _ptr(dv), c, c, c, _ptr(dtau), _ptr(ws), ws.numel(), _stream())
        return dq, dk, dv, dtau.reshape(tau.shape), None, None, None


class _WindowAttnPackedFn(torch.autograd.Function):

    @staticmethod
    def forward(ctx, qk, v, tau, tau_min, heads, wi, drop_p=0.0, drop_seed=0):
        m, c = v.shape
        dh = c // heads
        dev = v.device
        out = torch.empty((m, c), dtype=torch.float32, device=dev)
        lse = torch.empty((m, heads), dtype=torch.float32, device=dev)
        ctx.drop_p, ctx.drop_seed = drop_p, drop_seed
        kp = ctypes.c_void_p(qk.data_ptr() + 4 * c)
        _lib.call("seg3d_window_attn_fwd", _ptr(qk), kp, _ptr(v), 2 * c, 2 * c, c,
                  _ptr(wi.tok), _ptr(wi.win_start), _ptr(wi.win_count), _ptr(wi.win_tile0), _ptr(wi.tile_item),
                  int(wi.n_tiles), _ptr(wi.qg_item), int(wi.n_qgroups), m, int(wi.n_windows), heads, dh,
                  _ptr(tau.reshape(-1)), float(tau_min), float(drop_p), int(drop_seed), _ptr(out), _ptr(lse), None, 0,
                  _stream())
        ctx.save_for_backward(qk, v, tau, out, lse)
        ctx.wi, ctx.heads, ctx.tau_min = wi, heads, tau_min
        return out

    @staticmethod
    def backward(ctx, dout):
        qk, v, tau, out, lse = ctx.saved_tensors
        wi, heads = ctx.wi, ctx.heads
        m, c = v.shape
        dev = v.device
        dout = _f32c(dout)
        dqk = torch.empty((m, 2 * c), dtype=torch.float32, device=dev)
        dv = torch.empty((m, c), dtype=torch.float32, device=dev)
        dtau = torch.empty((1,), dtype=torch.float32, device=dev)
        ws = _workspace(_lib.query("seg3d_window_attn_workspace_bytes", m, int(wi.n_tiles), heads, c // heads), dev)
        kp = ctypes.c_void_p(qk.data_ptr() + 4 * c)
        dkp = ctypes.c_void_p(dqk.data_ptr() + 4 * c)
        _lib.call("seg3d_window_attn_bwd", _ptr(qk), kp, _ptr(v), 2 * c, 2 * c, c,
                  _ptr(out), _ptr(dout), _ptr(lse), _ptr(wi.tok), _ptr(wi.win_start), _ptr(wi.win_count),
                  _ptr(wi.win_tile0), _ptr(wi.tile_item), int(wi.n_tiles), _ptr(wi.qg_item), int(wi.n_qgroups), m,
                  int(wi.n_windows), heads, c // heads, _ptr(tau.reshape(-1)), float(ctx.tau_min), float(ctx.drop_p),
                  int(ctx.drop_seed), _ptr(dqk), dkp, _ptr(dv), 2 * c, 2 * c, c, _ptr(dtau), _ptr(ws), ws.numel(), _stream())
        return dqk, dv, dtau.reshape(tau.shape), None, None, None, None, None


def window_attention_packed(qk, v, tau, tau_min, heads, wi, drop_p=0.0, drop_seed=0):
    _need_gpu(qk, v, tau)
    if qk.dtype != torch.float32 or v.dtype != torch.float32 or not qk.is_contiguous() or not v.is_contiguous() \
            or qk.shape[1] != 2 * v.shape[1]:
        raise _lib.Seg3dError("qk must be contiguous float32 [m, 2C] and v contiguous float32 [m, C]")
    if v.shape[1] % heads or not _lib.load().seg3d_window_attn_supported(int(heads), v.shape[1] // int(heads)):
        raise _lib.Seg3dError(
# ... 1917 lines not shown
```

openseg3d_amd/segformer.py:

```python
import os
from collections import OrderedDict
from functools import partial

import torch
import torch.nn as nn

from . import ops
from . import spconv
from .swformer import SparseWindowPartitionLayer, SWFormerBlock


PLAN_FIRST = os.environ.get("SEG3D_PLAN_FIRST", "1") != "0"


def replace_feature(out, new_features):
    return out.replace_feature(new_features)


def conv_module(cin, cout, norm_fn, act_fn, conv_type="subm", indice_key=None):
    if conv_type == "subm":
        conv = spconv.SubMConv3d(cin, cout, 3, padding=1, bias=False, indice_key=indice_key)
    elif conv_type == "spconv":
        conv = spconv.SparseConv3d(cin, cout, 3, stride=2, padding=1, bias=False, indice_key=indice_key)
    elif conv_type == "inverseconv":
        conv = spconv.SparseInverseConv3d(cin, cout, 3, bias=False, indice_key=indice_key)
    else:
        raise NotImplementedError(conv_type)
    return ConvBnAct(conv, norm_fn(cout), act_fn)


class ConvBnAct(spconv.SparseSequential):

    def forward(self, x):
        conv, bn = self._modules["0"], self._modules["1"]
        if conv.fusable_with(bn, x):
            return conv.forward_bn_act(x, bn, relu=True)
        y = conv(x)
        return y.replace_feature(ops.batch_norm_act(y.features, bn, relu=True))


class FusedMLP(nn.Sequential):

    def forward(self, x):
        mods = list(self._modules.values())
        i = 0
        while i < len(mods):
            m = mods[i]
            if isinstance(m, RowLinear) and i + 1 < len(mods) and not self.training \
                    and isinstance(mods[i + 1], nn.BatchNorm1d) and not isinstance(mods[i + 1], NarrowBatchNorm1d):
                relu = i + 2 < len(mods) and isinstance(mods[i + 2], nn.ReLU)
                y = ops.linear_bn_act_eval(x, m, mods[i + 1], relu)
                if y is not None:
                    x = y
                    i += 3 if relu else 2
                    continue
            if isinstance(m, (nn.BatchNorm1d, nn.SyncBatchNorm)) and not isinstance(m, NarrowBatchNorm1d) \
                    and m.num_features % 4 == 0:
                relu = i + 1 < len(mods) and isinstance(mods[i + 1], nn.ReLU)
                x = ops.batch_norm_act(x, m, relu=relu)
                i += 2 if relu else 1
            else:
                x = m(x)
                i += 1
        return x


class VFE(nn.Module):

    def __init__(self, voxel_feature_channel, reduce="mean"):
        super().__init__()
        self.voxel_feature_channel = voxel_feature_channel
        self.reduce = reduce

    def forward(self, features, seg):
        return ops.segment_reduce(features, seg, {"mean": ops.REDUCE_MEAN, "max": ops.REDUCE_MAX}[self.reduce])


class FlattenSELayer(nn.Module):

    def __init__(self, channel, reduction=4):
        super().__init__()
        self.fc = nn.Sequential(nn.Linear(channel, channel // reduction, bias=False), nn.ReLU(inplace=True),
                                nn.Linear(channel // reduction, channel, bias=False), nn.Sigmoid())

    def forward(self, x, indices, row_offsets=None):
        if row_offsets is not None:
            starts = [0] + list(row_offsets[:-1])
            spans = [(s, e) for s, e in zip(starts, row_offsets)]
            pooled = ops.span_mean(x, row_offsets)
            gate = self.fc(pooled)
            return torch.cat([x[s:e] * gate[b] for b, (s, e) in enumerate(spans)], dim=0)
        indices = indices.long()
        pooled = ops.scatter(x, indices, reduce="mean")
        return x * self.fc(pooled)[indices]


class SALayer(spconv.SparseModule):

    def __init__(self, planes, indice_key=None):
        super().__init__()
        self.conv = spconv.SubMConv3d(planes, 1, 3, padding=1, bias=False, indice_key=indice_key)

    def forward(self, x):
        return x.replace_feature(ops.sa_gate(x.features, self.conv.weight, x.level.subm()))


def _block_tail(block, y, x):
    if block.se is not None:
        y = y.replace_feature(block.se(y.features, y.indices[:, 0], y.level.sample_offsets()))
    if block.sa is not None:
        y = block.sa(y)
    return y.replace_feature(torch.relu(y.features + x.features))


class SparseBasicBlock(spconv.SparseModule):
    def __init__(self, inplanes, planes, norm_fn, act_fn, indice_key=None, with_se=False, with_sa=False):
        super().__init__()
        self.conv1 = spconv.SubMConv3d(inplanes, planes, 3, padding=1, bias=True, indice_key=indice_key)
        self.bn1 = norm_fn(planes)
        self.act = act_fn
        self.conv2 = spconv.SubMConv3d(planes, planes, 3, padding=1, bias=True, indice_key=indice_key)
        self.bn2 = norm_fn(planes)
        self.se = FlattenSELayer(planes) if with_se else None
        self.sa = SALayer(planes, indice_key=indice_key) if with_sa else None

    def forward(self, x):
        plain = self.se is None and self.sa is None
        if self.conv1.fusable_with(self.bn1, x) and self.conv2.fusable_with(self.bn2, x):
            y = self.conv1.forward_bn_act(x, self.bn1, relu=True)
            if plain:
                return self.conv2.forward_bn_act(y, self.bn2, relu=True, res=x.features)
            return _block_tail(self, self.conv2.forward_bn_act(y, self.bn2, relu=False, res=None), x)
        y = self.conv1(x)
        y = y.replace_feature(ops.batch_norm_act(y.features, self.bn1, relu=True))
        y = self.conv2(y)
        if plain:
            return y.replace_feature(ops.batch_norm_act(y.features, self.bn2, relu=True, res=x.features))
        return _block_tail(self, y.replace_feature(ops.batch_norm_act(y.features, self.bn2, relu=False)), x)


class UpBlock(spconv.SparseModule):
    def __init__(self, inplanes, planes, norm_fn, act_fn, conv_type, layer_id):
        super().__init__()
        self.transform = SparseBasicBlock(inplanes, inplanes, norm_fn, act_fn, indice_key=f"subm{layer_id}")
        self.bottleneck = conv_module(2 * inplanes, inplanes, norm_fn, act_fn, "subm", f"subm{layer_id}")
        key = f"spconv{layer_id}" if conv_type == "inverseconv" else f"subm{layer_id}"
        self.out = conv_module(inplanes, planes, norm_fn, act_fn, conv_type, key)

    def forward(self, x_bottom, x_lateral):
        t = self.transform(x_lateral)
        cat = torch.cat([x_bottom.features, t.features], dim=1)
        m = self.bottleneck(t.replace_feature(cat)).features
        if cat.shape[1] == 2 * m.shape[1]:
            skip = cat[:, 0::2] + cat[:, 1::2]
        else:
            skip = cat.view(cat.shape[0], m.shape[1], -1).sum(dim=2)
        return self.out(t.replace_feature(m + skip))


class PointTransformer(nn.Module):
    def __init__(self, input_channels, output_channels, grid_size, voxel_size, point_cloud_range, batching_info,
                 window_shape, drop_path_rate, depths, num_classes):
        super().__init__()
        self.sparse_shape = [int(g) for g in grid_size][::-1]
        self.voxel_size, self.point_cloud_range = voxel_size, point_cloud_range
        self.depths = list(depths)
        grid_xyz = [float(g) for g in grid_size]
        self.norm_fn = partial(nn.BatchNorm1d, eps=1e-3, momentum=0.01)
        self.act_fn = nn.ReLU(inplace=True)
        norm_fn, act_fn = self.norm_fn, self.act_fn

        self.conv_input = ConvBnAct(
            spconv.SubMConv3d(input_channels, 48, 3, padding=1, bias=False, indice_key="subm1"), norm_fn(48), act_fn)
        dpr = [x.item() for x in torch.linspace(0, drop_path_rate, sum(self.depths))]
        widths = (48, 96, 192, 384)
        for k, c in enumerate(widths):
            lo, hi = sum(self.depths[:k]), sum(self.depths[:k + 1])
            stage = nn.Sequential(
                SparseWindowPartitionLayer(batching_info[k], window_shape, [g / (2 ** k) for g in grid_xyz]),
                SWFormerBlock(c, 8, depth=self.depths[k], drop_path=dpr[lo:hi]))
            setattr(self, f"swformer_block{k + 1}", stage)
        for k in (1, 2, 3):
            setattr(self, f"conv_down{k}", conv_module(widths[k - 1], widths[k], norm_fn, act_fn, "spconv",
                                                       f"spconv{k + 1}"))
        self.up4 = UpBlock(384, 192, norm_fn, act_fn, "inverseconv", 4)
        self.up3 = UpBlock(192, 96, norm_fn, act_fn, "inverseconv", 3)
        self.up2 = UpBlock(96, 48, norm_fn, act_fn, "inverseconv", 2)
        self.up1 = UpBlock(48, output_channels, norm_fn, act_fn, "subm", 1)
        self.aux_voxel_classifier = nn.Sequential(RowLinear(384, num_classes, bias=False))
        self.voxel_classifier = nn.Sequential(RowLinear(output_channels, num_classes, bias=False))

    def prepare(self, batch_dict):
        level = spconv.SiteLevel(batch_dict["voxel_coords"].int(), self.sparse_shape, batch_dict["batch_size"])
        batch_dict["site_level"] = level
        widths = (48, 96, 192, 384)
        level.seed_chain(3)
        launched = []
        for k in range(4):
            level.subm()
            level.mask_order()
            level.subm_plan()
            part = getattr(self, f"swformer_block{k + 1}")[0]
            if part not in level.window_plans:
                level.window_plans[part] = part.launch_plan(level.coords, level.batch_size, widths[k])
                launched.append(level.window_plans[part])
            if k < 3:
                level.parity_order()
                level = level.down()[0]
        if launched:
            SparseWindowPartitionLayer.finish_plans(launched)
        return batch_dict
# ... 240 lines not shown
```

Baseline: 4.203 million points/s.

## Fuse training BN+ReLU into following linear's input load and backward

In training FusedMLP, a BatchNorm+ReLU followed by a RowLinear is now computed by applying the per-channel affine and ReLU on load inside the bf16x3 linear forward kernel, so the activated tensor is never materialized. Backward recomputes the ReLU mask from the pre-activation input in a new wgrad-partials kernel and in new BN backward kernels, which avoids storing and re-reading the BN output. This saves a full activation write and read per fused layer at the cost of extra per-element FMA work and LDS staging of scale and shift. The new path is gated by an environment flag that defaults to on.

```diff
diff --git a/include/seg3d_hip.h b/include/seg3d_hip.h
--- a/include/seg3d_hip.h
+++ b/include/seg3d_hip.h
@@ -124,6 +124,10 @@
 int seg3d_linear_wgrad_partials_xbf16(const uint16_t* x_bf16, const float* dy, int64_t m, int32_t cin, int32_t cout,
                                       int32_t with_bias, void* workspace, size_t workspace_bytes, int32_t* chunks,
                                       void* stream);
+int seg3d_linear_wgrad_bnrelu_fits(int64_t m, int32_t cin, int32_t cout);
+int seg3d_linear_wgrad_partials_bnrelu(const float* x_pre, const float* scale_in, const float* shift_in, const float* dy,
+                                       int64_t m, int32_t cin, int32_t cout, int32_t with_bias, void* workspace,
+                                       size_t workspace_bytes, int32_t* chunks, void* stream);
 int seg3d_debug_set_wgrad_lds(int32_t on);
 int seg3d_reduce_partials(const float* part, int32_t chunks, int64_t n, int64_t nw, float* dw, float* db, void* stream);
 int seg3d_reduce_partials_batched(const void* jobs, int32_t n_jobs, int64_t total_blocks, void* stream);
@@ -138,6 +142,9 @@
 int seg3d_linear_fwd_x6(const float* x, int64_t m, const void* w_packed, const float* bias ,
                         const float* scale , const float* shift , int32_t relu, int32_t cin,
                         int32_t cout, float* y, void* stream);
+int seg3d_linear_fwd_x6_bnrelu(const float* x_pre, const float* scale_in, const float* shift_in, int64_t m,
+                               const void* w_packed, const float* bias , int32_t cin, int32_t cout, float* y,
+                               void* stream);
 
 typedef struct {
   const float* src;
@@ -218,6 +225,9 @@
 int seg3d_batchnorm_bwd(const float* dy, const float* y, const float* x, const float* mean, const float* rstd,
                         const float* gamma, int32_t relu, int64_t m, int32_t c, float* dx, float* dres,
                         float* sums, void* workspace, size_t workspace_bytes, void* stream);
+int seg3d_batchnorm_bwd_pre(const float* dy, const float* x, const float* scale, const float* shift, const float* mean,
+                            const float* rstd, const float* gamma, int64_t m, int32_t c, float* dx, float* sums,
+                            void* workspace, size_t workspace_bytes, void* stream);
 int seg3d_batchnorm_bwd_reduce(const float* dy, const float* y, const float* x, const float* mean,
                                const float* rstd, int32_t relu, int64_t m, int32_t c, float* sums,
                                void* workspace, size_t workspace_bytes, void* stream);
diff --git a/openseg3d_amd/_lib.py b/openseg3d_amd/_lib.py
--- a/openseg3d_amd/_lib.py
+++ b/openseg3d_amd/_lib.py
@@ -8,7 +8,7 @@
 
 OK, EINVAL, EWORKSPACE, ELAUNCH = 0, -1, -2, -3
 REDUCE_SUM, REDUCE_MEAN, REDUCE_MAX = 0, 1, 2
-ABI_VERSION = 53
+ABI_VERSION = 54
 
 _p, _i32, _i64, _sz, _f = ctypes.c_void_p, ctypes.c_int32, ctypes.c_int64, ctypes.c_size_t, ctypes.c_float
 _u64 = ctypes.c_uint64
@@ -62,10 +62,13 @@
     "seg3d_linear_packed_bytes_x6": (ctypes.c_size_t, [_i32, _i32]),
     "seg3d_linear_pack_weight_x6": (ctypes.c_int, [_p, _i32, _i32, _i32, _p, _p]),
     "seg3d_linear_fwd_x6": (ctypes.c_int, [_p, _i64, _p, _p, _p, _p, _i32, _i32, _i32, _p, _p]),
+    "seg3d_linear_fwd_x6_bnrelu": (ctypes.c_int, [_p, _p, _p, _i64, _p, _p, _i32, _i32, _p, _p]),
     "seg3d_pack_weights_batched": (ctypes.c_int, [_p, _i32, _i64, _p]),
     "seg3d_linear_wgrad_workspace_bytes": (ctypes.c_size_t, [_i64, _i32, _i32]),
     "seg3d_linear_wgrad": (ctypes.c_int, [_p, _p, _i64, _i32, _i32, _p, _p, _p, ctypes.c_size_t, _p]),
     "seg3d_linear_wgrad_partials": (ctypes.c_int, [_p, _p, _i64, _i32, _i32, _i32, _p, ctypes.c_size_t, _p, _p]),
+    "seg3d_linear_wgrad_bnrelu_fits": (ctypes.c_int, [_i64, _i32, _i32]),
+    "seg3d_linear_wgrad_partials_bnrelu": (ctypes.c_int, [_p, _p, _p, _p, _i64, _i32, _i32, _i32, _p, ctypes.c_size_t, _p, _p]),
     "seg3d_reduce_partials": (ctypes.c_int, [_p, _i32, _i64, _i64, _p, _p, _p]),
     "seg3d_reduce_partials_batched": (ctypes.c_int, [_p, _i32, _i64, _p]),
     "seg3d_linear_packed_bytes": (_sz, [_i32, _i32, _i32]),
@@ -96,6 +99,7 @@
     "seg3d_affine_act": (ctypes.c_int, [_p, _p, _p, _p, _i32, _i64, _i32, _p, _p]),
     "seg3d_gelu_fwd": (ctypes.c_int, [_p, _i64, _p, _p, _p]),
     "seg3d_batchnorm_bwd": (ctypes.c_int, [_p, _p, _p, _p, _p, _p, _i32, _i64, _i32, _p, _p, _p, _p, ctypes.c_size_t, _p]),
+    "seg3d_batchnorm_bwd_pre": (ctypes.c_int, [_p, _p, _p, _p, _p, _p, _p, _i64, _i32, _p, _p, _p, ctypes.c_size_t, _p]),
     "seg3d_batchnorm_bwd_reduce": (ctypes.c_int, [_p, _p, _p, _p, _p, _i32, _i64, _i32, _p, _p, ctypes.c_size_t, _p]),
     "seg3d_batchnorm_bwd_apply": (ctypes.c_int, [_p, _p, _p, _p, _p, _p, _p, _p, _i32, _i64, _i32, _p, _p, _p]),
     "seg3d_segment_reduce_fwd": (ctypes.c_int, [_p, _i32, _p, _p, _i64, _i32, _p, _p, _p]),
diff --git a/openseg3d_amd/csrc/linear_x6.hip b/openseg3d_amd/csrc/linear_x6.hip
--- a/openseg3d_amd/csrc/linear_x6.hip
+++ b/openseg3d_amd/csrc/linear_x6.hip
@@ -36,14 +36,16 @@
     dst[128] = __builtin_bit_cast(uint4, l);
 }
 
-template <int RT, int WPS>
+template <int RT, int WPS, bool BN = false>
 __global__ __launch_bounds__(kThreads, WPS) void linear_x6_kernel(const float* __restrict__ x, int64_t m_rows,
                                                                   const uint4* __restrict__ wp, const float* __restrict__ bias,
                                                                   const float* __restrict__ scale, const float* __restrict__ shift,
                                                                   int relu, int cin, int cout, float* __restrict__ y, int ncg,
-                                                                  int64_t nrb) {
+                                                                  int64_t nrb, const float* __restrict__ scale_in,
+                                                                  const float* __restrict__ shift_in) {
     constexpr int DEPTH = 2;
     __shared__ __attribute__((aligned(16))) uint4 wl[2][kSlab];
+    extern __shared__ __attribute__((aligned(16))) float affine_in[];
     const int tid = threadIdx.x, lane = tid & 63, wave = tid >> 6;
     const int g = lane >> 4, c16 = lane & 15;
     const int64_t id = blockIdx.x;
@@ -60,6 +62,12 @@
         xp[i] = x + r * cin + 4 * g;
     }
     const int nkb = cin >> 5;
+    if constexpr (BN) {
+        for (int i = tid; i < cin; i += kThreads) {
+            affine_in[i] = scale_in[i];
+            affine_in[cin + i] = shift_in[i];
+        }
+    }
     const uint4* wsrc = wp + (int64_t)cg * kSlab + tid;
     f32x4 raw[DEPTH][RT][2];
     auto issue_rows = [&](int kb, auto slot_tag) {
@@ -102,10 +110,22 @@
         const int cur = kb & 1;
         const bool more = kb + 1 < nkb;
         bf16x8 xh[RT], xm[RT], xl[RT];
+        f32x4 si[2], ti[2];
+        if constexpr (BN) {
+#pragma unroll
+            for (int h = 0; h < 2; ++h) {
+                si[h] = *reinterpret_cast<const f32x4*>(affine_in + kb * 32 + 16 * h + 4 * g);
+                ti[h] = *reinterpret_cast<const f32x4*>(affine_in + cin + kb * 32 + 16 * h + 4 * g);
+            }
+        }
 #pragma unroll
         for (int i = 0; i < RT; ++i) {
-            const float v[8] = {raw[SLOT][i][0][0], raw[SLOT][i][0][1], raw[SLOT][i][0][2], raw[SLOT][i][0][3],
-                                raw[SLOT][i][1][0], raw[SLOT][i][1][1], raw[SLOT][i][1][2], raw[SLOT][i][1][3]};
+            float v[8] = {raw[SLOT][i][0][0], raw[SLOT][i][0][1], raw[SLOT][i][0][2], raw[SLOT][i][0][3],
+                          raw[SLOT][i][1][0], raw[SLOT][i][1][1], raw[SLOT][i][1][2], raw[SLOT][i][1][3]};
+            if constexpr (BN) {
+#pragma unroll
+                for (int e = 0; e < 8; ++e) v[e] = fmaxf(v[e] * si[e >> 2][e & 3] + ti[e >> 2][e & 3], 0.f);
+            }
             split3(v, &xh[i], &xm[i], &xl[i]);
         }
         if (kb + 2 < nkb) {
@@ -219,15 +239,34 @@
     if (blocks > 0x7FFFFFFFll) return SEG3D_EINVAL;
     if (g_x6_rt == 4)
         hipLaunchKernelGGL((linear_x6_kernel<4, 2>), dim3((unsigned)blocks), dim3(kThreads), 0, as_stream(stream), x, m,
-                           static_cast<const uint4*>(w_packed), bias, scale, shift, relu ? 1 : 0, cin, cout, y, ncg, nrb);
+                           static_cast<const uint4*>(w_packed), bias, scale, shift, relu ? 1 : 0, cin, cout, y, ncg, nrb, nullptr,
+                           nullptr);
     else if (g_x6_wps == 4)
         hipLaunchKernelGGL((linear_x6_kernel<2, 4>), dim3((unsigned)blocks), dim3(kThreads), 0, as_stream(stream), x, m,
-                           static_cast<const uint4*>(w_packed), bias, scale, shift, relu ? 1 : 0, cin, cout, y, ncg, nrb);
+                           static_cast<const uint4*>(w_packed), bias, scale, shift, relu ? 1 : 0, cin, cout, y, ncg, nrb, nullptr,
+                           nullptr);
     else
         hipLaunchKernelGGL((linear_x6_kernel<2, 3>), dim3((unsigned)blocks), dim3(kThreads), 0, as_stream(stream), x, m,
-                           static_cast<const uint4*>(w_packed), bias, scale, shift, relu ? 1 : 0, cin, cout, y, ncg, nrb);
+                           static_cast<const uint4*>(w_packed), bias, scale, shift, relu ? 1 : 0, cin, cout, y, ncg, nrb, nullptr,
+                           nullptr);
     SEG3D_CHECK_LAUNCH();
     return SEG3D_OK;
 }
 
-}
+int seg3d_linear_fwd_x6_bnrelu(const float* x_pre, const float* scale_in, const float* shift_in, int64_t m,
+                               const void* w_packed, const float* bias, int32_t cin, int32_t cout, float* y, void* stream) {
+    if (m < 0 || seg3d_linear_packed_bytes_x6(cin, cout) == 0 || cin > 2048) return SEG3D_EINVAL;
+    if (m == 0) return SEG3D_OK;
+    if (!x_pre || !scale_in || !shift_in || !w_packed || !y) return SEG3D_EINVAL;
+    const int ncg = cout >> 6;
+    const int64_t nrb = (m + 127) / 128;
+    const int64_t blocks = (nrb + 7) / 8 * 8 * ncg;
+    if (blocks > 0x7FFFFFFFll) return SEG3D_EINVAL;
+    hipLaunchKernelGGL((linear_x6_kernel<2, 3, true>), dim3((unsigned)blocks), dim3(kThreads), (size_t)cin * 2 * sizeof(float),
+                       as_stream(stream), x_pre, m, static_cast<const uint4*>(w_packed), bias, nullptr, nullptr, 0, cin, cout, y,
+                       ncg, nrb, scale_in, shift_in);
+    SEG3D_CHECK_LAUNCH();
+    return SEG3D_OK;
+}
+
+}
diff --git a/openseg3d_amd/csrc/rownorm.hip b/openseg3d_amd/csrc/rownorm.hip
--- a/openseg3d_amd/csrc/rownorm.hip
+++ b/openseg3d_amd/csrc/rownorm.hip
@@ -322,6 +322,76 @@
         }
         if (dres) reinterpret_cast<float4*>(dres)[t] = g;
         const float4 xv = reinterpret_cast<const float4*>(x)[t];
+        const float4 mu = *reinterpret_cast<const float4*>(mean + 4 * q);
+        const float4 rs = *reinterpret_cast<const float4*>(rstd + 4 * q);
+        const float4 ga = *reinterpret_cast<const float4*>(gamma + 4 * q);
+        const float4 s1 = *reinterpret_cast<const float4*>(sums + 4 * q);
+        const float4 s2 = *reinterpret_cast<const float4*>(sums + c + 4 * q);
+        float4 o;
+        o.x = ga.x * rs.x * (g.x - s1.x * inv_m - (xv.x - mu.x) * rs.x * s2.x * inv_m);
+        o.y = ga.y * rs.y * (g.y - s1.y * inv_m - (xv.y - mu.y) * rs.y * s2.y * inv_m);
+        o.z = ga.z * rs.z * (g.z - s1.z * inv_m - (xv.z - mu.z) * rs.z * s2.z * inv_m);
+        o.w = ga.w * rs.w * (g.w - s1.w * inv_m - (xv.w - mu.w) * rs.w * s2.w * inv_m);
+        reinterpret_cast<float4*>(dx)[t] = o;
+    }
+}
+
+__device__ __forceinline__ float4 relu_mask_pre(float4 g, const float4 xv, const float4 s, const float4 b) {
+    const float4 v = make_float4(xv.x * s.x + b.x, xv.y * s.y + b.y, xv.z * s.z + b.z, xv.w * s.w + b.w);
+    g.x = v.x > 0.f ? g.x : 0.f; g.y = v.y > 0.f ? g.y : 0.f;
+    g.z = v.z > 0.f ? g.z : 0.f; g.w = v.w > 0.f ? g.w : 0.f;
+    return g;
+}
+
+__global__ __launch_bounds__(kThreads) void col_reduce_pre_kernel(const float* __restrict__ x, const float* __restrict__ dy,
+                                                                  const float* __restrict__ scale,
+                                                                  const float* __restrict__ shift,
+                                                                  const float* __restrict__ mean,
+                                                                  const float* __restrict__ rstd, int64_t m, int c,
+                                                                  float* __restrict__ part ) {
+    extern __shared__ float red[];
+    const int quads = c / 4;
+    const int lanes = kThreads / quads;
+    const int q = threadIdx.x % quads, rl = threadIdx.x / quads;
+    if (rl < lanes) {
+        float4 a = make_float4(0.f, 0.f, 0.f, 0.f), b = a;
+        const float4 p0 = *reinterpret_cast<const float4*>(mean + 4 * q);
+        const float4 p1 = *reinterpret_cast<const float4*>(rstd + 4 * q);
+        const float4 sc = *reinterpret_cast<const float4*>(scale + 4 * q);
+        const float4 sh = *reinterpret_cast<const float4*>(shift + 4 * q);
+        for (int64_t row = (int64_t)blockIdx.x * lanes + rl; row < m; row += (int64_t)gridDim.x * lanes) {
+            const float4 xv = *reinterpret_cast<const float4*>(x + row * c + 4 * q);
+            const float4 g = relu_mask_pre(*reinterpret_cast<const float4*>(dy + row * c + 4 * q), xv, sc, sh);
+            a.x += g.x; a.y += g.y; a.z += g.z; a.w += g.w;
+            b.x += g.x * (xv.x - p0.x) * p1.x; b.y += g.y * (xv.y - p0.y) * p1.y;
+            b.z += g.z * (xv.z - p0.z) * p1.z; b.w += g.w * (xv.w - p0.w) * p1.w;
+        }
+        *reinterpret_cast<float4*>(red + (size_t)rl * 2 * c + 4 * q) = a;
+        *reinterpret_cast<float4*>(red + (size_t)rl * 2 * c + c + 4 * q) = b;
+    }
+    __syncthreads();
+    for (int i = threadIdx.x; i < 2 * c; i += kThreads) {
+        float t = red[i];
+        for (int l = 1; l < lanes; ++l) t += red[(size_t)l * 2 * c + i];
+        part[(size_t)blockIdx.x * 2 * c + i] = t;
+    }
+}
+
+__global__ __launch_bounds__(kThreads) void bn_bwd_apply_pre_kernel(const float* __restrict__ dy, const float* __restrict__ x,
+                                                                    const float* __restrict__ scale,
+                                                                    const float* __restrict__ shift,
+                                                                    const float* __restrict__ mean,
+                                                                    const float* __restrict__ rstd,
+                                                                    const float* __restrict__ gamma,
+                                                                    const float* __restrict__ sums , float inv_m,
+                                                                    int64_t total_quads, int quads, float* __restrict__ dx) {
+    const int c = quads * 4;
+    for (int64_t t = (int64_t)blockIdx.x * kThreads + threadIdx.x; t < total_quads; t += (int64_t)gridDim.x * kThreads) {
+        const int q = (int)(t % quads);
+        const float4 xv = reinterpret_cast<const float4*>(x)[t];
+        const float4 sc = *reinterpret_cast<const float4*>(scale + 4 * q);
+        const float4 sh = *reinterpret_cast<const float4*>(shift + 4 * q);
+        const float4 g = relu_mask_pre(reinterpret_cast<const float4*>(dy)[t], xv, sc, sh);
         const float4 mu = *reinterpret_cast<const float4*>(mean + 4 * q);
         const float4 rs = *reinterpret_cast<const float4*>(rstd + 4 * q);
         const float4 ga = *reinterpret_cast<const float4*>(gamma + 4 * q);
@@ -541,6 +611,26 @@
     return SEG3D_OK;
 }
 
+int seg3d_batchnorm_bwd_pre(const float* dy, const float* x, const float* scale, const float* shift, const float* mean,
+                            const float* rstd, const float* gamma, int64_t m, int32_t c, float* dx,
+                            float* sums , void* workspace, size_t workspace_bytes, void* stream) {
+    if (m <= 0 || bad_c(c) || !sums) return SEG3D_EINVAL;
+    if (!workspace || workspace_bytes < seg3d_batchnorm_workspace_bytes(m, c)) return SEG3D_EWORKSPACE;
+    if (!dy || !x || !scale || !shift || !mean || !rstd || !gamma || !dx) return SEG3D_EINVAL;
+    hipStream_t st = as_stream(stream);
+    float* part = static_cast<float*>(workspace);
+    const unsigned nb = col_blocks(m, c);
+    hipLaunchKernelGGL(col_reduce_pre_kernel, dim3(nb), dim3(kThreads), kColSmem, st, x, dy, scale, shift, mean, rstd, m, c, part);
+    SEG3D_CHECK_LAUNCH();
+    hipLaunchKernelGGL(col_sums_finish, dim3((unsigned)((2 * c + 31) / 32)), dim3(1024), 0, st, part, (int)nb, c, sums);
+    SEG3D_CHECK_LAUNCH();
+    const int64_t tq = m * (c / 4);
+    hipLaunchKernelGGL(bn_bwd_apply_pre_kernel, dim3(blocks_for(tq, kThreads * 4)), dim3(kThreads), 0, st, dy, x, scale, shift,
+                       mean, rstd, gamma, sums, 1.0f / (float)m, tq, c / 4, dx);
+    SEG3D_CHECK_LAUNCH();
+    return SEG3D_OK;
+}
+
 int seg3d_batchnorm_bwd_reduce(const float* dy, const float* y, const float* x, const float* mean, const float* rstd,
                                int32_t relu, int64_t m, int32_t c, float* sums, void* workspace, size_t workspace_bytes,
                                void* stream) {
diff --git a/openseg3d_amd/csrc/voxelize.hip b/openseg3d_amd/csrc/voxelize.hip
--- a/openseg3d_amd/csrc/voxelize.hip
+++ b/openseg3d_amd/csrc/voxelize.hip
@@ -273,7 +273,7 @@
     return cart2polar_impl<double>(points, n_points, row_stride, xyz_col, out, stream);
 }
 
-int seg3d_abi_version(void) { return 53; }
+int seg3d_abi_version(void) { return 54; }
 
 namespace {
 thread_local char g_last_error[320] = "";
diff --git a/openseg3d_amd/csrc/wgrad_dense.hip b/openseg3d_amd/csrc/wgrad_dense.hip
--- a/openseg3d_amd/csrc/wgrad_dense.hip
+++ b/openseg3d_amd/csrc/wgrad_dense.hip
@@ -75,11 +75,14 @@
     return p;
 }
 
-template <bool XB, bool GROUP, int DEPTH = 1>
+template <bool XB, bool GROUP, int DEPTH = 1, bool BN = false>
 __global__ __launch_bounds__(kThreads, (DEPTH > 1 ? 1 : 2)) void wgrad_dense_kernel(const void* __restrict__ x_v, const float* __restrict__ dy,
                                                                int64_t m_rows, int cin, int cout, int rows_per_chunk,
                                                                int nbi, int tiles, float* __restrict__ part,
-                                                               int want_bias, int group) {
+                                                               int want_bias, int group,
+                                                               const float* __restrict__ scale_in,
+                                                               const float* __restrict__ shift_in) {
+    static_assert(!BN || (!XB && !GROUP && DEPTH == 1), "the BatchNorm + ReLU prologue is the fp32 split-K form's");
     const float* x = static_cast<const float*>(x_v);
     __shared__ __attribute__((aligned(16))) float red[GROUP ? 4 : 64 * 64];
     __shared__ float red_b[GROUP ? 1 : kWaves][64];
@@ -102,6 +105,17 @@
     const uint32_t yoff = (uint32_t)((8 * rg * cout + (a_ok ? co0 + 4 * cq : 0)) * 4);
     const uint32_t xoff = (uint32_t)((8 * rg * cin + (b_ok ? ci0 + 4 * cq : 0)) * (XB ? 2 : 4));
     const bool want_db = want_bias && bi == 0;
+    f32x4 s_in = {0.f, 0.f, 0.f, 0.f}, t_in = s_in;
+    if constexpr (BN) {
+        s_in = *reinterpret_cast<const f32x4*>(scale_in + (b_ok ? ci0 + 4 * cq : 0));
+        t_in = *reinterpret_cast<const f32x4*>(shift_in + (b_ok ? ci0 + 4 * cq : 0));
+    }
+    auto bn_relu = [&](f32x4 v) {
+        v = v * s_in + t_in;
+#pragma unroll
+        for (int e = 0; e < 4; ++e) v[e] = fmaxf(v[e], 0.f);
+        return v;
+    };
 
     f32x4 acc[4][4];
 #pragma unroll
@@ -130,7 +144,7 @@
             for (int i = 0; i < 8; ++i) xs[i] = *reinterpret_cast<const f32x4*>(base + (size_t)i * cin * 4 + xoff);
         }
     };
-    auto make_b = [&](auto& xs) {
+    auto make_b = [&](auto& xs, auto activated) {
 #pragma unroll
         for (int b = 0; b < 4; ++b) {
             if constexpr (XB) {
@@ -138,11 +152,15 @@
             } else {
                 float v[8];
 #pragma unroll
-                for (int i = 0; i < 8; ++i) v[i] = xs[i][b];
+                for (int i = 0; i < 8; ++i) {
+                    v[i] = xs[i][b];
+                    if constexpr (BN && !decltype(activated)::value) v[i] = fmaxf(v[i] * s_in[b] + t_in[b], 0.f);
+                }
                 split_frag(v, &b_hi[b], &b_lo[b]);
             }
         }
     };
+    constexpr std::false_type kRaw{};
     auto multiply = [&](auto& ys) {
         if (want_db) {
 #pragma unroll
@@ -179,7 +197,7 @@
                 const int cur = s + d * kStride;
                 if (cur < n_full) {
                     const bool more = cur + DEPTH * kStride < n_full;
-                    make_b(xd[d]);
+                    make_b(xd[d], kRaw);
                     if (more) load_x(cur + DEPTH * kStride, xd[d]);
                     multiply(yd[d]);
                     if (more) load_rows(dy, cout, yoff, cur + DEPTH * kStride, yd[d]);
@@ -193,7 +211,7 @@
         }
         for (; s < n_full; s += kStride) {
             const bool more = s + kStride < n_full;
-            make_b(xr);
+            make_b(xr, kRaw);
             if (more) load_x(s + kStride, xr);
             multiply(yr);
             if (more) load_rows(dy, cout, yoff, s + kStride, yr);
@@ -212,11 +230,12 @@
                 xq[i] = ok ? vx : make_uint2(0u, 0u);
             } else {
                 const f32x4 vx = *reinterpret_cast<const f32x4*>(x + r * cin + (b_ok ? ci0 + 4 * cq : 0));
-                xr[i] = ok ? vx : z;
+                if constexpr (BN) xr[i] = ok ? bn_relu(vx) : z;
+                else xr[i] = ok ? vx : z;
             }
             yr[i] = ok ? vy : z;
         }
-        make_b(xr);
+        make_b(xr, std::bool_constant<BN>{});
         multiply(yr);
     }
 
@@ -373,10 +392,10 @@
         const unsigned blocks = (unsigned)((p.chunks + 7) / 8 * 8) * (unsigned)groups;
         if (x_bf16)
             hipLaunchKernelGGL((wgrad_dense_kernel<true, true>), dim3(blocks), dim3(kThreads), 0, st, x, dy, m, cin, cout, (int)p.rows,
-                               nbi_g, groups, part, want_bias, p.group);
+                               nbi_g, groups, part, want_bias, p.group, nullptr, nullptr);
         else
             hipLaunchKernelGGL((wgrad_dense_kernel<false, true>), dim3(blocks), dim3(kThreads), 0, st, x, dy, m, cin, cout, (int)p.rows,
-                               nbi_g, groups, part, want_bias, p.group);
+                               nbi_g, groups, part, want_bias, p.group, nullptr, nullptr);
         return;
     }
     const int tiles = p.nbo * p.nbi;
@@ -387,15 +406,15 @@
     }();
     if (!x_bf16 && depth == 3) {
         hipLaunchKernelGGL((wgrad_dense_kernel<false, false, 3>), dim3(blocks), dim3(kThreads), 0, st, x, dy, m, cin, cout, (int)p.rows,
-                           p.nbi, tiles, part, want_bias, 0);
+                           p.nbi, tiles, part, want_bias, 0, nullptr, nullptr);
         return;
     }
     if (x_bf16)
         hipLaunchKernelGGL((wgrad_dense_kernel<true, false>), dim3(blocks), dim3(kThreads), 0, st, x, dy, m, cin, cout, (int)p.rows,
-                           p.nbi, tiles, part, want_bias, 0);
+                           p.nbi, tiles, part, want_bias, 0, nullptr, nullptr);
     else
         hipLaunchKernelGGL((wgrad_dense_kernel<false, false>), dim3(blocks), dim3(kThreads), 0, st, x, dy, m, cin, cout, (int)p.rows,
-                           p.nbi, tiles, part, want_bias, 0);
+                           p.nbi, tiles, part, want_bias, 0, nullptr, nullptr);
 }
 
 static int linear_wgrad_partials(const void* x, bool x_bf16, const float* dy, int64_t m, int32_t cin, int32_t cout,
@@ -418,6 +437,32 @@
     return linear_wgrad_partials(x, false, dy, m, cin, cout, with_bias, workspace, workspace_bytes, chunks, stream);
 }
 
+extern "C" int seg3d_linear_wgrad_bnrelu_fits(int64_t m, int32_t cin, int32_t cout) {
+    if (m <= 0 || cin <= 0 || cout <= 0 || (cin & 3) || (cout & 3)) return 0;
+    const Plan p = plan(m, cin, cout, true);
+    return !p.lds && !p.group;
+}
+
+extern "C" int seg3d_linear_wgrad_partials_bnrelu(const float* x_pre, const float* scale_in, const float* shift_in,
+                                                  const float* dy, int64_t m, int32_t cin, int32_t cout, int32_t with_bias,
+                                                  void* workspace, size_t workspace_bytes, int32_t* chunks, void* stream) {
+    if (m < 0 || cin <= 0 || cout <= 0 || (cin & 3) || (cout & 3) || !chunks) return SEG3D_EINVAL;
+    if (m > 0 && (!x_pre || !scale_in || !shift_in || !dy)) return SEG3D_EINVAL;
+    if (workspace_bytes < seg3d_linear_wgrad_workspace_bytes(m, cin, cout) || (m > 0 && !workspace)) return SEG3D_EINVAL;
+    *chunks = 0;
+    if (m == 0) return SEG3D_OK;
+    const Plan p = plan(m, cin, cout, true);
+    if (p.lds || p.group) return SEG3D_EINVAL;
+    const int tiles = p.nbo * p.nbi;
+    const unsigned blocks = (unsigned)((p.chunks + 7) / 8 * 8) * (unsigned)tiles;
+    hipLaunchKernelGGL((wgrad_dense_kernel<false, false, 1, true>), dim3(blocks), dim3(kThreads), 0, as_stream(stream), x_pre, dy,
+                       m, cin, cout, (int)p.rows, p.nbi, tiles, static_cast<float*>(workspace), with_bias ? 1 : 0, 0, scale_in,
+                       shift_in);
+    SEG3D_CHECK_LAUNCH();
+    *chunks = p.chunks;
+    return SEG3D_OK;
+}
+
 extern "C" int seg3d_linear_wgrad_partials_xbf16(const uint16_t* x_bf16, const float* dy, int64_t m, int32_t cin, int32_t cout,
                                                  int32_t with_bias, void* workspace, size_t workspace_bytes, int32_t* chunks,
                                                  void* stream) {
diff --git a/openseg3d_amd/ops.py b/openseg3d_amd/ops.py
--- a/openseg3d_amd/ops.py
+++ b/openseg3d_amd/ops.py
@@ -1033,14 +1033,22 @@
         y = torch.empty_like(x)
         r = None if res is None else _f32c(res)
         _lib.call("seg3d_affine_act", _ptr(x), _ptr(r), _ptr(scale), _ptr(shift), int(relu), m, c, _ptr(y), _stream())
-        ctx.save_for_backward(x, y, mean, rstd, gamma)
+        ctx.pre = bool(relu) and res is None
+        if ctx.pre:
+            ctx.save_for_backward(x, scale, shift, mean, rstd, gamma)
+        else:
+            ctx.save_for_backward(x, y, mean, rstd, gamma)
         ctx.relu, ctx.has_res = relu, res is not None
         return y
 
     @staticmethod
     def backward(ctx, dy):
+        dy = _f32c(dy)
+        if ctx.pre:
+            x, scale, shift, mean, rstd, gamma = ctx.saved_tensors
+            dx, sums = _batchnorm_bwd_pre(dy, x, scale, shift, mean, rstd, gamma)
+            return dx, None, sums[1], sums[0], None, None, None, None, None
         x, y, mean, rstd, gamma = ctx.saved_tensors
-        dy = _f32c(dy)
         m, c = x.shape
         dx = torch.empty_like(x)
         dres = torch.empty_like(x) if ctx.has_res else None
@@ -1050,6 +1058,17 @@
         _lib.call("seg3d_batchnorm_bwd", _ptr(dy), _ptr(y), _ptr(x), _ptr(mean), _ptr(rstd), _ptr(gamma), int(ctx.relu),
                   m, c, _ptr(dx), _ptr(dres), _ptr(sums), _ptr(ws), ws_bytes, _stream())
         return dx, dres, sums[1], sums[0], None, None, None, None, None
+
+
+def _batchnorm_bwd_pre(dy, x, scale, shift, mean, rstd, gamma):
+    m, c = x.shape
+    dx = torch.empty_like(x)
+    sums = torch.empty((2, c), dtype=torch.float32, device=x.device)
+    ws_bytes = _lib.query("seg3d_batchnorm_workspace_bytes", m, c)
+    ws = _workspace(ws_bytes, x.device)
+    _lib.call("seg3d_batchnorm_bwd_pre", _ptr(dy), _ptr(x), _ptr(scale), _ptr(shift), _ptr(mean), _ptr(rstd), _ptr(gamma),
+              m, c, _ptr(dx), _ptr(sums), _ptr(ws), ws_bytes, _stream())
+    return dx, sums
 
 
 def _sync_bn_group(bn):
@@ -1254,6 +1273,88 @@
     return cached[1], cached[2], key
 
 
+def _bn_batch_stats(xc, bn):
+    m, c = xc.shape
+    with torch.no_grad():
+        stats = torch.empty((6, c), dtype=torch.float32, device=xc.device)
+        track = bn.training and bn.track_running_stats
+        mom = 0.0
+        if track:
+            bn._seg3d_stats_epoch = getattr(bn, "_seg3d_stats_epoch", 0) + 1
+            _bump_batches_tracked(bn)
+            mom = bn.momentum if bn.momentum is not None else 1.0 / float(bn.num_batches_tracked)
+        ws_bytes = _lib.query("seg3d_batchnorm_workspace_bytes", m, c)
+        ws = _workspace(ws_bytes, xc.device)
+        _lib.call("seg3d_batchnorm_stats", _ptr(xc), m, c, float(bn.eps), _ptr(bn.weight), _ptr(bn.bias), float(mom),
+                  _ptr(bn.running_mean) if track else None, _ptr(bn.running_var) if track else None, _ptr(stats),
+                  _ptr(ws), ws_bytes, _stream())
+    return stats
+
+
+POINT_BN_ONLOAD = os.environ.get("SEG3D_POINT_BN_ONLOAD", "1") != "0"
+
+
+class _BnReluLinearFn(torch.autograd.Function):
+
+    @staticmethod
+    def forward(ctx, x_pre, gamma, beta, weight, bias, mean, rstd, scale, shift):
+        cout, cin = weight.shape
+        y = torch.empty((x_pre.shape[0], cout), dtype=torch.float32, device=x_pre.device)
+        _lib.call("seg3d_linear_fwd_x6_bnrelu", _ptr(x_pre), _ptr(scale), _ptr(shift), x_pre.shape[0],
+                  _ptr(_linear_pack_x6(weight)), _ptr(None if bias is None else _f32c(bias)), cin, cout, _ptr(y), _stream())
+        ctx.save_for_backward(x_pre, mean, rstd, scale, shift, gamma, weight)
+        ctx.has_bias = bias is not None
+        ctx.bias_param = bias
+        return y
+
+    @staticmethod
+    def backward(ctx, dy):
+        x_pre, mean, rstd, scale, shift, gamma, weight = ctx.saved_tensors
+        dy = _f32c(dy)
+        cout, cin = weight.shape
+        m = x_pre.shape[0]
+        dx = dgamma = dbeta = dw = db = None
+        fk = _WgradFork(dy.device)
+        want_db = ctx.has_bias and ctx.needs_input_grad[4]
+        if ctx.needs_input_grad[3]:
+            dw = torch.empty_like(weight, memory_format=torch.contiguous_format)
+            if want_db:
+                db = torch.empty((cout,), dtype=torch.float32, device=dy.device)
+            ws_bytes = _lib.query("seg3d_linear_wgrad_workspace_bytes", m, cin, cout)
+            ws = _workspace(ws_bytes, dy.device)
+            chunks = ctypes.c_int32(0)
+            _lib.call("seg3d_linear_wgrad_partials_bnrelu", _ptr(x_pre), _ptr(scale), _ptr(shift), _ptr(dy), m, cin, cout,
+                      1 if want_db else 0, _ptr(ws), ws_bytes, ctypes.byref(chunks), fk.fork(ws, x_pre, scale, dy))
+            fk.add_reduce(ws, chunks.value, cin * cout + cout, cin * cout, dw.data_ptr(), db.data_ptr() if want_db else 0)
+        elif want_db:
+            db = dy.sum(0)
+        if any(ctx.needs_input_grad[:3]):
+            dz = _linear_apply(dy, _linear_pack(weight, 1), None, cout, cin)
+            dx, sums = _batchnorm_bwd_pre(dz, x_pre, scale, shift, mean, rstd, gamma)
+            dgamma, dbeta = sums[1], sums[0]
+        fk.join((weight, dw), (ctx.bias_param, db))
+        return dx, dgamma, dbeta, dw, db, None, None, None, None
+
+
+def bn_relu_linear_fits(x, bn, lin):
+    if not (POINT_BN_ONLOAD and torch.is_grad_enabled() and bn.training and bn.track_running_stats and bn.affine):
+        return False
+    if not (x.is_cuda and x.dim() == 2 and x.dtype == torch.float32 and x.shape[0] >= 2):
+        return False
+    cout, cin = lin.weight.shape
+    if bn.num_features != cin or cin != x.shape[1] or cin > 1024 or not _x6_fits(cin, cout):
+        return False
+    if not (CONV_PRECISION == "bf16x3" and TRAIN_STORAGE == "fp32") or _sync_bn_group(bn) is not None:
+        return False
+    return bool(_lib.query("seg3d_linear_wgrad_bnrelu_fits", x.shape[0], cin, cout))
+
+
+def bn_relu_linear(x_pre, bn, lin):
+    xc = _f32c(x_pre)
+    stats = _bn_batch_stats(xc, bn)
+    return _BnReluLinearFn.apply(xc, bn.weight, bn.bias, lin.weight, lin.bias, stats[2], stats[3], stats[4], stats[5])
+
+
 def batch_norm_act(x, bn, relu=True, res=None):
     c = x.shape[1]
     fits = x.is_cuda and x.dim() == 2 and x.dtype == torch.float32 and c % 4 == 0 and c <= 1024 and bn.affine
@@ -1269,20 +1370,7 @@
         return torch.relu(y) if relu else y
     if use_batch:
         xc = _f32c(x)
-        m = xc.shape[0]
-        with torch.no_grad():
-            stats = torch.empty((6, c), dtype=torch.float32, device=x.device)
-            track = bn.training and bn.track_running_stats
-            mom = 0.0
-            if track:
-                bn._seg3d_stats_epoch = getattr(bn, "_seg3d_stats_epoch", 0) + 1
-                _bump_batches_tracked(bn)
-                mom = bn.momentum if bn.momentum is not None else 1.0 / float(bn.num_batches_tracked)
-            ws_bytes = _lib.query("seg3d_batchnorm_workspace_bytes", m, c)
-            ws = _workspace(ws_bytes, x.device)
-            _lib.call("seg3d_batchnorm_stats", _ptr(xc), m, c, float(bn.eps), _ptr(bn.weight), _ptr(bn.bias), float(mom),
-                      _ptr(bn.running_mean) if track else None, _ptr(bn.running_var) if track else None, _ptr(stats),
-                      _ptr(ws), ws_bytes, _stream())
+        stats = _bn_batch_stats(xc, bn)
         return _BatchNormActFn.apply(xc, res, bn.weight, bn.bias, stats[2], stats[3], stats[4], stats[5], bool(relu))
     with torch.no_grad():
         scale, shift, _ = bn_eval_affine(bn)
diff --git a/openseg3d_amd/segformer.py b/openseg3d_amd/segformer.py
--- a/openseg3d_amd/segformer.py
+++ b/openseg3d_amd/segformer.py
@@ -57,6 +57,11 @@
             if isinstance(m, (nn.BatchNorm1d, nn.SyncBatchNorm)) and not isinstance(m, NarrowBatchNorm1d) \
                     and m.num_features % 4 == 0:
                 relu = i + 1 < len(mods) and isinstance(mods[i + 1], nn.ReLU)
+                if relu and self.training and i + 2 < len(mods) and isinstance(mods[i + 2], RowLinear) \
+                        and ops.bn_relu_linear_fits(x, m, mods[i + 2]):
+                    x = ops.bn_relu_linear(x, m, mods[i + 2])
+                    i += 3
+                    continue
                 x = ops.batch_norm_act(x, m, relu=relu)
                 i += 2 if relu else 1
             else:
```

New measurement: 4.266 million points/s, median of 6. 1.5% higher.
